# ZhentaoHuang/SealD-NeRF

Hardware: AMD Instinct MI355X
Metric: rendered rays/sec + sampled-points/sec, 800×800 D-NeRF jumpingjacks (higher is better)
Workload: dtype f16; 1 GPU; dnerf jumpingjacks-like 800x800 full-frame inference render, -O (fp16 field network, fp16 grid table), test sequence of 20 frames (camera orbit, one time stamp per frame, t = 0 .. 1: every frame selects its own occupancy slice, time encoding and the t == 0 canonical rule), T_thresh 1e-2, max_steps 1024, dt_gamma 0; rays=640000, field=fused, loop=device, frames_per_loop=4, rays_per_loop_on_this_gpu=2560000, frames_in_flight=4 loops of 4 frame(s) (the next starts when the newest is down to rays/2 alive), parallelism=single GPU

## Files before the change

### include/sdn_hip.h

```cpp
#ifndef SDN_HIP_H
#define SDN_HIP_H

#include <stdint.h>

#ifdef __cplusplus
extern "C" {
#endif

#define SDN_F32 0
#define SDN_F16 1

#define SDN_E_BADARG (-1)
#define SDN_E_UNSUPPORTED (-2)
#define SDN_E_TIMEOUT (-3)

const char *sdn_version(void);
int sdn_debug_shader_clock(unsigned long long *out4, uint32_t wall_ticks, void *stream);


int sdn_near_far_from_aabb(const float *rays_o, const float *rays_d, const float *aabb, uint32_t N,
                           float min_near, float *nears, float *fars, void *stream);

int sdn_sph_from_ray(const float *rays_o, const float *rays_d, float radius, uint32_t N, float *coords,
                     void *stream);

int sdn_get_rays(const float *pose, float fx, float fy, float cx, float cy, uint32_t H, uint32_t W, float *rays_o,
                 float *rays_d, void *stream);

int sdn_morton3D(const int32_t *coords, uint32_t N, int32_t *indices, void *stream);
int sdn_morton3D_invert(const int32_t *indices, uint32_t N, int32_t *coords, void *stream);

int sdn_packbits(const float *grid, uint32_t N, float density_thresh, uint8_t *bitfield, void *stream);

uint64_t sdn_march_rays_train_scratch_bytes(uint32_t N, uint32_t max_steps);
int sdn_march_rays_train(const float *rays_o, const float *rays_d, const uint8_t *grid, float bound,
                         float dt_gamma, uint32_t max_steps, uint32_t N, uint32_t C, uint32_t H, uint32_t M,
                         const float *nears, const float *fars, float *xyzs, float *dirs, float *deltas,
                         int32_t *rays, int32_t *counter, const float *noises, void *scratch, void *stream);

int sdn_composite_rays_train_forward(const float *sigmas, const float *rgbs, const float *deltas,
                                     const int32_t *rays, uint32_t M, uint32_t N, float T_thresh,
                                     float *weights_sum, float *depth, float *image, void *stream);

int sdn_composite_rays_train_backward(const float *grad_weights_sum, const float *grad_image,
                                      const float *sigmas, const float *rgbs, const float *deltas,
                                      const int32_t *rays, const float *weights_sum, const float *image,
                                      uint32_t M, uint32_t N, float T_thresh, float *grad_sigmas,
                                      float *grad_rgbs, void *stream);

int sdn_composite_whole_rays(const float *sigmas, const float *rgbs, const float *deltas, const int32_t *rays,
                             const float *nears, uint32_t M, uint32_t N, float T_thresh, float *weights_sum,
                             float *depth, float *image, void *stream);

int sdn_march_rays(uint32_t n_alive, uint32_t n_step, const int32_t *rays_alive, const float *rays_t,
                   const float *rays_o, const float *rays_d, float bound, float dt_gamma, uint32_t max_steps,
                   uint32_t C, uint32_t H, const uint8_t *grid, const float *nears, const float *fars,
                   float *xyzs, float *dirs, float *deltas, const float *noises, void *stream);

int sdn_march_rays_ex(uint32_t n_alive, uint32_t n_step, const int32_t *rays_alive, const float *rays_t,
                      const float *rays_o, const float *rays_d, float bound, float dt_gamma, uint32_t max_steps,
                      uint32_t C, uint32_t H, const uint8_t *grid, const float *fars, float *xyzs, float *dirs,
                      float *deltas, const float *noises, uint32_t M_pad, const uint8_t *cull_grid,
                      uint32_t *live_idx, uint32_t *live_count, void *stream);
uint32_t sdn_cull_grid_bytes(void);
int sdn_build_cull_grid(const uint8_t *bitfield, uint32_t H, uint8_t *cull_grid, void *stream);

int sdn_composite_rays(uint32_t n_alive, uint32_t n_step, float T_thresh, int32_t *rays_alive, float *rays_t,
                       const float *sigmas, const float *rgbs, const float *deltas, float *weights_sum,
                       float *depth, float *image, void *stream);

uint64_t sdn_compact_alive_scratch_bytes(uint32_t n);
int sdn_compact_alive(const int32_t *in, uint32_t n, int32_t *out, int32_t *n_out, void *scratch, void *stream);


int sdn_grid_encode_forward_quad_f16(const float *inputs, const void *quad_table, const int32_t *ref_offsets_host, void *outputs,
                                     uint32_t B, float S, uint32_t H, void *stream);
int sdn_grid_encode_forward(const float *inputs, const void *embeddings, const int32_t *offsets_host,
                            void *outputs, uint32_t B, uint32_t D, uint32_t C, uint32_t L, float S, uint32_t H,
                            void *dy_dx, uint32_t gridtype, int align_corners, uint32_t interp, int dtype,
                            void *stream);

int sdn_grid_encode_backward(const void *grad, const float *inputs, const int32_t *offsets_host,
                             void *grad_embeddings, uint32_t B, uint32_t D, uint32_t C, uint32_t L, float S,
                             uint32_t H, const void *dy_dx, void *grad_inputs, uint32_t gridtype,
                             int align_corners, uint32_t interp, int dtype, void *stream);
int sdn_grid_encode_backward_det(const void *grad, const float *inputs, const int32_t *offsets_host, void *grad_embeddings, uint32_t B,
                                 uint32_t D, uint32_t C, uint32_t L, float S, uint32_t H, const void *dy_dx, void *grad_inputs,
                                 uint32_t gridtype, int align_corners, uint32_t interp, int dtype, void *det_scratch, void *stream);

int sdn_sh_encode_forward(const float *inputs, float *outputs, uint32_t B, uint32_t D, uint32_t C,
                          float *dy_dx, void *stream);
int sdn_sh_encode_backward(const float *grad, const float *inputs, uint32_t B, uint32_t D, uint32_t C,
                           const float *dy_dx, float *grad_inputs, void *stream);

int sdn_freq_encode_forward(const float *inputs, uint32_t B, uint32_t D, uint32_t deg, uint32_t C,
                            float *outputs, void *stream);
int sdn_freq_encode_backward(const float *grad, const float *outputs, uint32_t B, uint32_t D, uint32_t deg,
                             uint32_t C, float *grad_inputs, void *stream);

uint32_t sdn_field_weight_blocks(void);

int sdn_field_forward_f16(const float *xyzs, const float *dirs, const uint32_t *live_idx, const uint32_t *live_count,
                          uint32_t M, const void *weights, const float *bias0, const void *table,
                          const int32_t *offsets_host, float S, uint32_t H, float bound, float density_scale,
                          int zero_deform, float *sigmas, float *rgbs, void *stream);

uint32_t sdn_field_weight_floats_f32(void);
int sdn_field_forward_f32(const float *xyzs, const float *dirs, const uint32_t *live_idx, const uint32_t *live_count,
                          uint32_t M, const float *weights, const float *bias0, const float *table,
                          const int32_t *offsets_host, float S, uint32_t H, float bound, float density_scale,
                          int zero_deform, float *sigmas, float *rgbs, float *deform, void *stream);

int sdn_field_forward_f32x3(const float *xyzs, const float *dirs, const uint32_t *live_idx, const uint32_t *live_count,
                            uint32_t M, const float *weights, const float *bias0, const float *table,
                            const int32_t *offsets_host, float S, uint32_t H, float bound, float density_scale,
                            int zero_deform, float *sigmas, float *rgbs, float *deform, void *stream);

void sdn_field_select_kernel(int persistent);
void sdn_field_persistent_workgroups(int n);

int sdn_field_build_quad_table(const void *embeddings, int dtype, const int32_t *ref_offsets_host, float S, uint32_t H, void *out,
                               void *stream);

int sdn_density_query_cells_f16(const int32_t *cells, const uint32_t *cell_count, uint32_t n, const float *noise, uint32_t seed,
                                uint32_t grid_size, float cas_bound, const void *weights, const float *bias0, const void *table,
                                const int32_t *offsets_host, float S, uint32_t H, float bound, float density_scale, int zero_deform,
                                float *tmp_slice, void *stream);
int sdn_density_query_cells_f32(const int32_t *cells, const uint32_t *cell_count, uint32_t n, const float *noise, uint32_t seed,
                                uint32_t grid_size, float cas_bound, const float *weights, const float *bias0, const float *table,
                                const int32_t *offsets_host, float S, uint32_t H, float bound, float density_scale, int zero_deform,
                                float *tmp_slice, void *stream);
int sdn_density_grid_ema(float *density_grid, const float *tmp_grid, uint64_t n, float decay, double *sum, void *stream);
int sdn_density_grid_pack(const float *density_grid, uint64_t n, const double *sum, float density_thresh, float *mean_out,
                          uint8_t *bitfield, void *stream);

uint64_t sdn_ffmlp_scratch_bytes(uint32_t B, uint32_t input_dim, uint32_t output_dim, uint32_t hidden_dim, uint32_t num_layers);

int sdn_ffmlp_forward(const void *inputs, const void *weights, uint32_t B, uint32_t input_dim, uint32_t output_dim,
                      uint32_t hidden_dim, uint32_t num_layers, uint32_t activation, uint32_t output_activation,
                      void *forward_buffer, void *outputs, void *scratch, void *stream);

int sdn_ffmlp_inference(const void *inputs, const void *weights, uint32_t B, uint32_t input_dim, uint32_t output_dim,
                        uint32_t hidden_dim, uint32_t num_layers, uint32_t activation, uint32_t output_activation,
                        void *outputs, void *scratch, void *stream);

int sdn_ffmlp_backward(const void *grad, const void *inputs, const void *weights, const void *forward_buffer, uint32_t B,
                       uint32_t input_dim, uint32_t output_dim, uint32_t hidden_dim, uint32_t num_layers,
                       uint32_t activation, uint32_t output_activation, int calc_grad_inputs, void *backward_buffer,
                       void *grad_inputs, void *grad_weights, void *scratch, void *stream);

typedef struct SdnSealBox {
    float bounds[24];
    uint32_t n_bounds, n_tris;
    const float *tris;
    float test_dir[3], tinv[12], rinv[9], scale[3], center[3];
    float hsv[3];
    int32_t modify_hsv;
    float rgb[3], rgb_light_offset;
    int32_t modify_rgb;
    int32_t has_map_source;
    float source_bound[6], map_source[3];
    uint32_t reserved_;
    void *scratch;
} SdnSealBox;

#define SDN_MAX_GROUP_FRAMES 16

typedef struct SdnFrameTime {
    const uint8_t *bitfield[SDN_MAX_GROUP_FRAMES];
    const float *field_bias0;
    uint32_t zero_deform;
    uint32_t reserved_;
    const void *cull_grid[SDN_MAX_GROUP_FRAMES];
} SdnFrameTime;

typedef struct SdnRenderCtx {
    const float *rays_o, *rays_d, *nears, *fars;
    const uint8_t *bitfield;
    void *cull_bits;
    int32_t *alive_a, *alive_b;
    float *rays_t, *weights_sum, *depth, *image;
    float *xyzs, *dirs, *deltas, *sigmas, *rgbs;
    uint32_t *live_idx;
    int32_t *live_counts, *state, *trace, *n_out;
    void *block_totals;
    const void *field_weights;
    const float *field_bias0;
    const void *grid_table;
    int32_t grid_offsets[17];
    float grid_S;
    uint32_t grid_H;
    uint32_t N, M_cap, n_counters, max_steps, C, H;
    float bound, dt_gamma, T_thresh, density_scale;
    int32_t zero_deform;
    const float *aabb;
    float min_near;
    int32_t reserved_;
    float *rays_tend;
    const struct SdnSealBox *seal;
    uint8_t *seal_mask;
    uint32_t n_group_frames, rays_per_frame;
    const uint8_t *frame_bitfield[SDN_MAX_GROUP_FRAMES];
    uint8_t *slot_frame;
    const void *frame_cull[SDN_MAX_GROUP_FRAMES];
    int32_t field_f32;
    int32_t reserved2_;
} SdnRenderCtx;

int sdn_render_begin(const SdnRenderCtx *ctx, void *stream);
int sdn_render_step_f16(const SdnRenderCtx *ctx, uint32_t bound_alive, void *stream);
int sdn_render_step_f16_ev(const SdnRenderCtx *ctx, uint32_t bound_alive, void *ev_field_begin, void *ev_field_end,
                           void *stream);
int sdn_render_time_kernel(int which);
int sdn_render_frame_f16(const SdnRenderCtx *ctx, float bg_color, float *image_out, float *depth_out, void *stream,
                         void *side_stream, void **ev_main, void **ev_copy, int32_t *host_snap, void **ev_field,
                         uint32_t max_field_events, uint32_t *iterations_out);
int sdn_render_frames_pipelined_f16(const SdnRenderCtx *const *ctxs, uint32_t n_ctx, uint32_t n_frames, const float *const *rays_o,
                                    const float *const *rays_d, float *const *image_outs, float *const *depth_outs, float bg_color,
                                    uint32_t overlap_div, void *const *streams, void *const *side_streams, void **ev_main,
                                    void **ev_copy, int32_t *host_snap, void *const *ev_field_frames, uint32_t max_field_events,
                                    const uint8_t *exclusive_frames, const SdnFrameTime *frame_times, void *const *done_events,
                                    uint32_t *iterations_out);
int sdn_seal_bbox_map(float *xyzs, float *dirs, uint32_t M, const float *bounds, uint32_t n_bounds, const float *tris,
                      uint32_t n_tris, const float *test_dir, const float *tinv, const float *rinv, const float *scale,
                      const float *center, uint8_t *mask, void *stream);
int sdn_seal_bbox_map_source(float *xyzs, float *dirs, uint32_t M, const float *bounds, uint32_t n_bounds, const float *tris,
                             uint32_t n_tris, const float *test_dir, const float *tinv, const float *rinv, const float *scale,
                             const float *center, const float *source_bound, const float *map_source, uint32_t *flag, uint8_t *mask,
                             const uint32_t *live_idx, const uint32_t *live_count, const int32_t *state, void *stream);
int sdn_seal_modify_hsv(float *rgbs, const uint8_t *mask, uint32_t M, float dh, float ds, float dv, void *stream);
int sdn_seal_modify_rgb(float *rgbs, const uint8_t *mask, uint32_t M, float r, float g, float b, float light_offset, void *scratch16,
                        const uint32_t *live_idx, const uint32_t *live_count, const int32_t *state, void *stream);

void *sdn_host_mailbox_alloc(uint32_t groups);
int sdn_host_mailbox_free(void *mailbox);
int sdn_render_finish(const SdnRenderCtx *ctx, float bg_color, float *image_out, float *depth_out, void *stream);

#define SDN_TRAIN_N_PARAMS 14

typedef struct SdnTrainParam {
    float *param;
    float *exp_avg, *exp_avg_sq;
    float *ema;
    uint64_t n;
} SdnTrainParam;

typedef struct SdnTrainStep {
    const float *rays_o, *rays_d;
    const float *target;
    const float *bg_color;
    float bg_value;
    uint32_t N, M;
    const uint8_t *bitfield;
    const void *cull_grid;
    const float *aabb;
    float bound, min_near, dt_gamma, density_scale, T_thresh;
    float time;
    uint32_t cascade, grid_size, max_steps;
    int32_t perturb;
    uint64_t noise_seed;
    const float *noises;
    int32_t *counter;
    int32_t grid_offsets[17];
    float grid_S;
    uint32_t grid_H;
    SdnTrainParam params[SDN_TRAIN_N_PARAMS];
    double lr_table, lr_net;
    double beta1, beta2, eps;
    float *adam_steps;
    float *loss_scale;
    int32_t *growth_tracker;
    float growth_factor, backoff_factor;
    uint32_t growth_interval;
    float ema_decay;
    float *loss_out;
    float *image_out;
    void *workspace;
    int32_t mode;
    int32_t keep_deform;
    float grad_divisor;
    int32_t deform_frozen;
    int32_t phase;
    int32_t sample_set;
    void *table_stream, *table_ready, *table_done;
    void *det_scratch;
} SdnTrainStep;

typedef struct SdnTrainLayout {
    uint64_t total_bytes;
    uint64_t w_table, w_deform, w_sigma0, w_sigma1, w_color;
    uint64_t g_table, g_deform, g_sigma0, g_sigma1, g_color;
    uint64_t xyzs, dirs, deltas, rays;
    uint64_t sample_set_stride;
    uint64_t sigmas;
    uint64_t weights_sum, depth, image;
    uint64_t found_inf;
} SdnTrainLayout;

int sdn_train_layout(uint32_t N, uint32_t M, uint32_t max_steps, const int32_t *grid_offsets, SdnTrainLayout *out);
int sdn_train_refresh(const SdnTrainStep *s, void *stream);
int sdn_train_step_f16(const SdnTrainStep *s, void *stream);
int sdn_train_flush(const SdnTrainStep *s, void *stream);

int sdn_train_layout_f32(uint32_t N, uint32_t M, uint32_t max_steps, const int32_t *grid_offsets, SdnTrainLayout *out);
int sdn_train_refresh_f32(const SdnTrainStep *s, void *stream);
int sdn_train_step_f32(const SdnTrainStep *s, void *stream);

#ifdef __cplusplus
}
#endif
#endif
```

### seald-nerf_amd/csrc/raymarching.hip

```cpp
#include <stdlib.h>

#include "sdn_common.h"
#include "sdn_internal.h"

namespace {
using sdn_int::FrameSel;

constexpr float kSqrt3 = 1.7320508075688772f;
constexpr float kRPi = 0.3183098861837907f;

__device__ __forceinline__ float signf_(float x) { return copysignf(1.0f, x); }
__device__ __forceinline__ float clampf_(float x, float lo, float hi) { return fminf(hi, fmaxf(lo, x)); }

__device__ __forceinline__ int mip_from_pos(float x, float y, float z, float max_cascade) {
    const float mx = fmaxf(fabsf(x), fmaxf(fabsf(y), fabsf(z)));
    int exponent;
    frexpf(mx, &exponent);
    return (int)fminf(max_cascade - 1, fmaxf(0.0f, (float)exponent));
}
__device__ __forceinline__ int mip_from_dt(float dt, float H, float max_cascade) {
    const float mx = (float)((double)(dt * H) * 0.5);
    int exponent;
    frexpf(mx, &exponent);
    return (int)fminf(max_cascade - 1, fmaxf(0.0f, (float)exponent));
// ... 702 lines not shown
    for (uint32_t k = lane; k < num_steps; k += 64u) {
        const float t = ts[k];
        const float dt = m.step_size(t);
        const float after = t + dt;
        float last = t0;
        if (k > 0) { const float tp = ts[k - 1]; last = tp + m.step_size(tp); }
        const size_t p = (size_t)point_index + k;
        xyzs[p * 3] = clampf_(m.ox + t * m.dx, -bound, bound);
        xyzs[p * 3 + 1] = clampf_(m.oy + t * m.dy, -bound, bound);
        xyzs[p * 3 + 2] = clampf_(m.oz + t * m.dz, -bound, bound);
        dirs[p * 3] = m.dx; dirs[p * 3 + 1] = m.dy; dirs[p * 3 + 2] = m.dz;
        deltas[p * 2] = dt;
        deltas[p * 2 + 1] = after - last;
    }
}

__global__ void __launch_bounds__(256) k_composite_train_fwd(const float *__restrict__ sigmas, const float *__restrict__ rgbs,
                                                             const float *__restrict__ deltas, const int32_t *__restrict__ rays,
                                                             uint32_t M, uint32_t N, float T_thresh, float *__restrict__ weights_sum,
                                                             float *__restrict__ depth, float *__restrict__ image) {
    const uint32_t n = threadIdx.x + blockIdx.x * blockDim.x;
    if (n >= N) return;
    const uint32_t index = (uint32_t)rays[n * 3], offset = (uint32_t)rays[n * 3 + 1], num_steps = (uint32_t)rays[n * 3 + 2];
    if (num_steps == 0 || offset + num_steps > M) {
        weights_sum[index] = 0; depth[index] = 0;
        image[(size_t)index * 3] = 0; image[(size_t)index * 3 + 1] = 0; image[(size_t)index * 3 + 2] = 0;
        return;
    }
    const float *s = sigmas + offset, *c = rgbs + (size_t)offset * 3, *dl = deltas + (size_t)offset * 2;
    uint32_t step = 0;
    float T = 1.0f, r = 0, g = 0, b = 0, ws = 0, t = 0, d = 0;
    while (step < num_steps) {
        const float alpha = 1.0f - sdn_exp_cr(-s[0] * dl[0]);
        const float weight = alpha * T;
        r += weight * c[0]; g += weight * c[1]; b += weight * c[2];
        t += dl[1];
        d += weight * t;
        ws += weight;
        T *= 1.0f - alpha;
        if (T < T_thresh) break;
        s++; c += 3; dl += 2; step++;
    }
    weights_sum[index] = ws; depth[index] = d;
    image[(size_t)index * 3] = r; image[(size_t)index * 3 + 1] = g; image[(size_t)index * 3 + 2] = b;
}

__global__ void __launch_bounds__(256) k_composite_whole_rays(const float *__restrict__ sigmas, const float *__restrict__ rgbs,
                                                              const float *__restrict__ deltas, const int32_t *__restrict__ rays,
                                                              const float *__restrict__ nears, uint32_t M, uint32_t N, float T_thresh,
                                                              float *__restrict__ weights_sum, float *__restrict__ depth, float *__restrict__ image) {
    const uint32_t n = threadIdx.x + blockIdx.x * blockDim.x;
    if (n >= N) return;
    const uint32_t index = (uint32_t)rays[n * 3], offset = (uint32_t)rays[n * 3 + 1], num_steps = (uint32_t)rays[n * 3 + 2];
    float weight_sum = 0, d = 0, r = 0, g = 0, b = 0;
    if (num_steps != 0 && offset + num_steps <= M) {
        const float *s = sigmas + offset, *c = rgbs + (size_t)offset * 3, *dl = deltas + (size_t)offset * 2;
        float t = nears[index];
        for (uint32_t step = 0; step < num_steps; step++) {
            if (dl[0] == 0) break;
            const float alpha = 1.0f - sdn_exp_cr(-s[0] * dl[0]);
            const float T = 1 - weight_sum;
            const float weight = alpha * T;
            weight_sum += weight;
            t += dl[1];
            d += weight * t;
            r += weight * c[0]; g += weight * c[1]; b += weight * c[2];
            if (T < T_thresh) break;
            s++; c += 3; dl += 2;
        }
    }
    weights_sum[index] = weight_sum; depth[index] = d;
    image[(size_t)index * 3] = r; image[(size_t)index * 3 + 1] = g; image[(size_t)index * 3 + 2] = b;
}

__global__ void __launch_bounds__(256) k_composite_train_bwd(const float *__restrict__ grad_weights_sum, const float *__restrict__ grad_image,
                                                             const float *__restrict__ sigmas, const float *__restrict__ rgbs,
                                                             const float *__restrict__ deltas, const int32_t *__restrict__ rays,
                                                             const float *__restrict__ weights_sum, const float *__restrict__ image,
                                                             uint32_t M, uint32_t N, float T_thresh, float *__restrict__ grad_sigmas,
                                                             float *__restrict__ grad_rgbs) {
    const uint32_t n = threadIdx.x + blockIdx.x * blockDim.x;
    if (n >= N) return;
    const uint32_t index = (uint32_t)rays[n * 3], offset = (uint32_t)rays[n * 3 + 1], num_steps = (uint32_t)rays[n * 3 + 2];
    if (num_steps == 0 || offset + num_steps > M) return;
    const float gws = grad_weights_sum[index];
    const float gi0 = grad_image[(size_t)index * 3], gi1 = grad_image[(size_t)index * 3 + 1], gi2 = grad_image[(size_t)index * 3 + 2];
    const float r_final = image[(size_t)index * 3], g_final = image[(size_t)index * 3 + 1], b_final = image[(size_t)index * 3 + 2];
    const float ws_final = weights_sum[index];
    const float *s = sigmas + offset, *c = rgbs + (size_t)offset * 3, *dl = deltas + (size_t)offset * 2;
    float *gs = grad_sigmas + offset, *gc = grad_rgbs + (size_t)offset * 3;
    uint32_t step = 0;
    float T = 1.0f, r = 0, g = 0, b = 0;
    while (step < num_steps) {
        const float alpha = 1.0f - sdn_exp_cr(-s[0] * dl[0]);
        const float weight = alpha * T;
        r += weight * c[0]; g += weight * c[1]; b += weight * c[2];
        T *= 1.0f - alpha;
        gc[0] = gi0 * weight; gc[1] = gi1 * weight; gc[2] = gi2 * weight;
        gs[0] = dl[0] * (gi0 * (T * c[0] - (r_final - r)) + gi1 * (T * c[1] - (g_final - g)) +
                         gi2 * (T * c[2] - (b_final - b)) + gws * (1 - ws_final));
        if (T < T_thresh) break;
        s++; c += 3; dl += 2; gs++; gc += 3; step++;
    }
}

constexpr float kTendUnset = -2.0f, kTendDead = -1.0f;
__device__ __forceinline__ float *state_tend(const int32_t *__restrict__ state) {
    return reinterpret_cast<float *>(((unsigned long long)(uint32_t)state[14] << 32) | (uint32_t)state[13]);
}
template <bool FAST>
__device__ __forceinline__ uint32_t march_ray(MarcherT<FAST> &m, const OccCache &oc, float t, float far, uint32_t n_step, float *px, float *pd,
                                              float *pl, float *tend = nullptr, uint8_t *psf = nullptr, uint32_t frame = 0,
                                              const float *t_begin = nullptr) {
    m.fine = oc.fine; m.fx0 = oc.fx0; m.fy0 = oc.fy0; m.fz0 = oc.fz0; m.fnx = oc.fnx; m.fny = oc.fny; m.fnz = oc.fnz;
    uint32_t step = 0;
    float last_t = t_begin ? *t_begin : t, x, y, z, dt;
    bool go = t < far;
    float t_end = far;
    if (FAST && oc.s_cull && go) {
        const float cached = tend ? *tend : kTendUnset;
        if (cached != kTendUnset) {
            t_end = cached;
            go = t < t_end;
        } else {
            go = ray_may_hit(oc.s_cull, m.ox, m.oy, m.oz, m.dx, m.dy, m.dz, t, far, t_end, oc.fx0, oc.fy0, oc.fz0, oc.fnx, oc.fny, oc.fnz);
            if (tend) *tend = go ? t_end : kTendDead;
        }
    }
    if (go) {
        while (t < far && t < t_end && step < n_step) {
            if (m.probe(t, x, y, z, dt, oc.s_cull)) {
                px[0] = x; px[1] = y; px[2] = z;
                pd[0] = m.dx; pd[1] = m.dy; pd[2] = m.dz;
                t += dt;
                pl[0] = dt;
                pl[1] = t - last_t;
                last_t = t;
                px += 3; pd += 3; pl += 2;
                if (psf) psf[step] = (uint8_t)frame;
                step++;
            }
        }
    }
    for (uint32_t k = step; k < n_step; k++) {
        px[0] = 0; px[1] = 0; px[2] = 0;
        pd[0] = 0; pd[1] = 0; pd[2] = 0;
        pl[0] = 0; pl[1] = 0;
        px += 3; pd += 3; pl += 2;
    }
    return step;
}

__device__ __forceinline__ uint32_t block_min_256(uint32_t v, uint32_t *lds4) {
    #pragma unroll
    for (int off = 32; off > 0; off >>= 1) v = min(v, (uint32_t)__shfl_xor((int)v, off, 64));
    __syncthreads();
    if ((threadIdx.x & 63u) == 0) lds4[threadIdx.x >> 6] = v;
    __syncthreads();
    return min(min(lds4[0], lds4[1]), min(lds4[2], lds4[3]));
}
constexpr uint32_t kNoFrame = 0xFFFFFFFFu;
__device__ __forceinline__ const uint8_t *frame_grid_uniform(const FrameSel &fs, uint32_t frame_uniform) {
    return fs.grid[__builtin_amdgcn_readfirstlane(frame_uniform)];
}

__device__ __forceinline__ void live_append(uint32_t step, uint32_t n, uint32_t n_step, uint32_t *__restrict__ live_idx,
                                            uint32_t *__restrict__ live_count) {
    const uint32_t lane = threadIdx.x & 63u;
    uint32_t incl = step;
    #pragma unroll
    for (int off = 1; off < 64; off <<= 1) {
        const uint32_t u = __shfl_up(incl, off, 64);
        if (lane >= (uint32_t)off) incl += u;
    }
    const uint32_t total = __shfl(incl, 63, 64);
    uint32_t base = 0;
    if (lane == 63 && total) base = atomicAdd(live_count, total);
    base = __shfl(base, 63, 64);
    const uint32_t dst = base + incl - step;
    for (uint32_t k = 0; k < step; k++) live_idx[dst + k] = n * n_step + k;
}

__device__ __forceinline__ bool composite_ray(int index, uint32_t n_step, float T_thresh, const float *s, const float *c, const float *dl,
                                              float *__restrict__ rays_t, float *__restrict__ weights_sum, float *__restrict__ depth,
                                              float *__restrict__ image, float *t_out = nullptr) {
    float t = rays_t[index];
    float weight_sum = weights_sum[index], d = depth[index];
    float r = image[(size_t)index * 3], g = image[(size_t)index * 3 + 1], b = image[(size_t)index * 3 + 2];
    uint32_t step = 0;
    if (n_step == 8) {
        float sv[8], cv[24], dv[16];
        #pragma unroll
        for (int q = 0; q < 2; q++) *reinterpret_cast<float4 *>(sv + 4 * q) = *reinterpret_cast<const float4 *>(s + 4 * q);
        #pragma unroll
        for (int q = 0; q < 6; q++) *reinterpret_cast<float4 *>(cv + 4 * q) = *reinterpret_cast<const float4 *>(c + 4 * q);
        #pragma unroll
        for (int q = 0; q < 4; q++) *reinterpret_cast<float4 *>(dv + 4 * q) = *reinterpret_cast<const float4 *>(dl + 4 * q);
        bool open = true;
        #pragma unroll
        for (int k = 0; k < 8; k++) {
            if (open && dv[2 * k] == 0) open = false;
            if (open) {
                const float alpha = 1.0f - sdn_exp_cr(-sv[k] * dv[2 * k]);
                const float T = 1 - weight_sum;
                const float weight = alpha * T;
                weight_sum += weight;
                t += dv[2 * k + 1];
                d += weight * t;
                r += weight * cv[3 * k]; g += weight * cv[3 * k + 1]; b += weight * cv[3 * k + 2];
                if (T < T_thresh) open = false; else step++;
            }
        }
    } else {
        while (step < n_step) {
            if (dl[0] == 0) break;
            const float alpha = 1.0f - sdn_exp_cr(-s[0] * dl[0]);
            const float T = 1 - weight_sum;
            const float weight = alpha * T;
            weight_sum += weight;
            t += dl[1];
            d += weight * t;
            r += weight * c[0]; g += weight * c[1]; b += weight * c[2];
            if (T < T_thresh) break;
            s++; c += 3; dl += 2; step++;
        }
    }
    const bool survives = !(step < n_step);
    if (survives) rays_t[index] = t;
    if (t_out) *t_out = t;
    weights_sum[index] = weight_sum; depth[index] = d;
    image[(size_t)index * 3] = r; image[(size_t)index * 3 + 1] = g; image[(size_t)index * 3 + 2] = b;
    return survives;
}

template <bool FAST>
__global__ void __launch_bounds__(256) k_march_rays(uint32_t n_alive, uint32_t n_step, const int32_t *__restrict__ rays_alive,
                                                    const float *__restrict__ rays_t, const float *__restrict__ rays_o,
                                                    const float *__restrict__ rays_d, float bound, float dt_gamma, uint32_t max_steps,
                                                    uint32_t C, uint32_t H, const uint8_t *__restrict__ grid,
                                                    const float *__restrict__ fars, float *__restrict__ xyzs, float *__restrict__ dirs,
                                                    float *__restrict__ deltas, const float *__restrict__ noises, uint32_t M_pad,
                                                    const uint32_t *__restrict__ cull, uint32_t *__restrict__ live_idx,
                                                    uint32_t *__restrict__ live_count, const int32_t *__restrict__ state,
                                                    const int32_t *__restrict__ rays_alive_b, FrameSel fs, const float *__restrict__ jump) {
    if (state) {
        n_alive = (uint32_t)state[0];
        n_step = (uint32_t)state[1];
        if (n_alive == 0) return;
        if (state[4]) rays_alive = rays_alive_b;
        live_count += state[3];
        const uint32_t m0 = n_alive * n_step;
        M_pad = m0 + (128u - m0 % 128u);
        if (!(state[15] && state[3] == 0)) jump = nullptr;
        if (blockIdx.x * 256u >= n_alive + 128u) return;
    }
    __shared__ uint4 s_cull4[FAST ? 256 : 1];
    __shared__ unsigned long long s_fine[FAST ? kFineCacheCells : 1];
    __shared__ uint32_t s_min4[4];
    const uint32_t n = threadIdx.x + blockIdx.x * blockDim.x;
    const int index = n < n_alive ? rays_alive[n] : -1;
    const bool grouped = fs.n_frames > 1;
    const uint32_t frame = (grouped && index >= 0) ? (uint32_t)index / fs.rays_per_frame : (grouped ? kNoFrame : 0u);
    uint32_t step = 0;
    float ro[3] = {0, 0, 0}, rdv[3] = {0, 0, 1}, t_ray = 0, far_ray = 0, t_jump = 0, noise = 0;
    if (index >= 0) {
        ro[0] = rays_o[(size_t)index * 3]; ro[1] = rays_o[(size_t)index * 3 + 1]; ro[2] = rays_o[(size_t)index * 3 + 2];
        rdv[0] = rays_d[(size_t)index * 3]; rdv[1] = rays_d[(size_t)index * 3 + 1]; rdv[2] = rays_d[(size_t)index * 3 + 2];
        t_ray = rays_t[index]; far_ray = fars[index];
        if (jump) t_jump = jump[index];
        if (noises) noise = noises[n];
    }
    uint32_t fcur = grouped ? block_min_256(frame, s_min4) : 0u;
    while (fcur != kNoFrame) {
        const uint8_t *grid_f = grouped ? frame_grid_uniform(fs, fcur) : grid;
        const uint32_t *cull_f = (grouped && cull) ? cull + (size_t)fcur * fs.cull_stride : cull;
        OccCache oc;
        occ_cache_load<FAST>(cull_f, grid_f, s_cull4, s_fine, oc);
        if (index >= 0 && frame == fcur) {
            MarcherT<FAST> m;
            m.init(ro, rdv, bound, dt_gamma, max_steps, C, H, grid_f);
            float t = t_ray;
            t += m.step_size(t) * noise;
            float *tend = state ? state_tend(state) : nullptr;
            if (tend) tend += index;
            const float t_walk = jump ? t_jump : t;
            step = march_ray<FAST>(m, oc, t_walk, far_ray, n_step, xyzs + (size_t)n * n_step * 3, dirs + (size_t)n * n_step * 3,
                                   deltas + (size_t)n * n_step * 2, tend, grouped ? fs.slot_frame + (size_t)n * n_step : nullptr, frame,
                                   jump ? &t : nullptr);
        }
        if (!grouped) break;
        fcur = block_min_256((frame != kNoFrame && frame > fcur) ? frame : kNoFrame, s_min4);
    }
    if (n >= n_alive) {
        const uint32_t slot = n_alive * n_step + (n - n_alive);
        if (slot < M_pad) {
            xyzs[(size_t)slot * 3] = 0; xyzs[(size_t)slot * 3 + 1] = 0; xyzs[(size_t)slot * 3 + 2] = 0;
            dirs[(size_t)slot * 3] = 0; dirs[(size_t)slot * 3 + 1] = 0; dirs[(size_t)slot * 3 + 2] = 0;
            deltas[(size_t)slot * 2] = 0; deltas[(size_t)slot * 2 + 1] = 0;
        }
    }
    if (live_idx) live_append(step, n, n_step, live_idx, live_count);
}

__device__ __forceinline__ uint32_t loop_list_len(const int32_t *__restrict__ state) {
    return state[8] ? (uint32_t)state[8] : (uint32_t)state[0];
}

__global__ void __launch_bounds__(256) k_composite_rays(uint32_t n_alive, uint32_t n_step, float T_thresh, int32_t *__restrict__ rays_alive,
                                                        float *__restrict__ rays_t, const float *__restrict__ sigmas,
                                                        const float *__restrict__ rgbs, const float *__restrict__ deltas,
                                                        float *__restrict__ weights_sum, float *__restrict__ depth, float *__restrict__ image,
                                                        const int32_t *__restrict__ state, int32_t *__restrict__ rays_alive_b,
                                                        uint32_t *__restrict__ block_totals) {
    if (state) {
        n_alive = loop_list_len(state);
        n_step = (uint32_t)state[1];
        if (state[4]) rays_alive = rays_alive_b;
    }
    const uint32_t n = threadIdx.x + blockIdx.x * blockDim.x;
    bool survives = false;
    if (n < n_alive) {
        const int index = rays_alive[n];
        if (index >= 0) {
            survives = composite_ray(index, n_step, T_thresh, sigmas + (size_t)n * n_step, rgbs + (size_t)n * n_step * 3,
                                     deltas + (size_t)n * n_step * 2, rays_t, weights_sum, depth, image);
            if (!survives) rays_alive[n] = -1;
        }
    }
    if (block_totals) {
        __shared__ uint32_t s_cnt[4];
        const unsigned long long m = __ballot(survives);
        if ((threadIdx.x & 63u) == 0) s_cnt[threadIdx.x >> 6] = (uint32_t)__popcll(m);
        __syncthreads();
        if (threadIdx.x == 0) block_totals[blockIdx.x] = s_cnt[0] + s_cnt[1] + s_cnt[2] + s_cnt[3];
    }
}

__global__ void __launch_bounds__(kScanBlock) k_compact_count(const int32_t *__restrict__ in, uint32_t n, uint32_t *__restrict__ block_totals,
                                                              const int32_t *__restrict__ state, const int32_t *__restrict__ in_b) {
    if (state) {
        n = loop_list_len(state);
        if (state[4]) in = in_b;
        if (blockIdx.x * kScanBlock >= n) return;
    }
    __shared__ uint32_t lds[16];
    const uint32_t i = blockIdx.x * kScanBlock + threadIdx.x;
    const bool keep = i < n && in[i] >= 0;
    const unsigned long long mask = __ballot(keep);
    if ((threadIdx.x & 63u) == 0) lds[threadIdx.x >> 6] = (uint32_t)__popcll(mask);
    __syncthreads();
    if (threadIdx.x == 0) {
        uint32_t t = 0;
        for (uint32_t w = 0; w < (kScanBlock >> 6); w++) t += lds[w];
        block_totals[blockIdx.x] = t;
    }
}

__global__ void __launch_bounds__(kScanBlock) k_compact_scatter(const int32_t *__restrict__ in, uint32_t n, const uint32_t *__restrict__ block_totals,
                                                                int32_t *__restrict__ out, int32_t *__restrict__ n_out,
                                                                const int32_t *__restrict__ state, const int32_t *__restrict__ in_b,
                                                                int32_t *__restrict__ out_b, uint32_t totals_per_block) {
    uint32_t last_block = gridDim.x - 1;
    if (state) {
        n = loop_list_len(state);
        if (state[4]) { in = in_b; out = out_b; }
        if (n == 0) {
            if (blockIdx.x == 0 && threadIdx.x == 0) n_out[0] = 0;
            return;
        }
        last_block = (n - 1) / kScanBlock;
        if (blockIdx.x > last_block) return;
    }
    __shared__ uint32_t lds[16];
    __shared__ uint32_t s_prev;
    uint32_t part = 0;
    for (uint32_t b = threadIdx.x; b < blockIdx.x * totals_per_block; b += kScanBlock) part += block_totals[b];
    uint32_t prev_total;
    block_inclusive_scan(part, lds, prev_total);
    if (threadIdx.x == 0) s_prev = prev_total;
    __syncthreads();
    const uint32_t i = blockIdx.x * kScanBlock + threadIdx.x;
    const int32_t v = i < n ? in[i] : -1;
    const bool keep = v >= 0;
    const unsigned long long mask = __ballot(keep);
    const uint32_t lane = threadIdx.x & 63u, wid = threadIdx.x >> 6;
    const uint32_t below = (uint32_t)__popcll(mask & ((1ull << lane) - 1ull));
    if (lane == 0) lds[wid] = (uint32_t)__popcll(mask);
    __syncthreads();
    uint32_t carry = 0, total = 0;
    for (uint32_t w = 0; w < (kScanBlock >> 6); w++) {
        const uint32_t c = lds[w];
        if (w < wid) carry += c;
        total += c;
    }
    if (keep) out[s_prev + carry + below] = v;
    if (blockIdx.x == last_block && threadIdx.x == 0) n_out[0] = (int32_t)(s_prev + total);
}


__global__ void __launch_bounds__(256) k_loop_init(uint32_t N, uint32_t max_steps, const float *__restrict__ nears, int32_t *__restrict__ alive_a,
                                                   float *__restrict__ rays_t, float *__restrict__ weights_sum, float *__restrict__ depth,
                                                   float *__restrict__ image, int32_t *__restrict__ state, int32_t *__restrict__ live_counts,
                                                   uint32_t n_counters, unsigned long long mailbox, uint32_t frame_tag,
                                                   float *__restrict__ rays_tend) {
    const uint32_t n = threadIdx.x + blockIdx.x * blockDim.x;
    if (n < N) {
        if (rays_tend) rays_tend[n] = kTendUnset;
        alive_a[n] = (int32_t)n;
        rays_t[n] = nears[n];
        weights_sum[n] = 0; depth[n] = 0;
        image[(size_t)n * 3] = 0; image[(size_t)n * 3 + 1] = 0; image[(size_t)n * 3 + 2] = 0;
    }
    if (n < n_counters) live_counts[n] = 0;
    if (n == 0) {
        state[0] = (int32_t)N; state[1] = 1; state[2] = 0; state[3] = 0; state[4] = 0;
        state[5] = (int32_t)N; state[6] = (int32_t)max_steps; state[7] = 0;
        for (int k = 8; k < 16; k++) state[k] = 0;
        state[10] = (int32_t)(uint32_t)mailbox;
        state[11] = (int32_t)(uint32_t)(mailbox >> 32);
        state[12] = (int32_t)frame_tag;
        const unsigned long long tp = (unsigned long long)(uintptr_t)rays_tend;
        state[13] = (int32_t)(uint32_t)tp;
        state[14] = (int32_t)(uint32_t)(tp >> 32);
    }
}


__device__ __forceinline__ void publish_snapshot(int32_t *__restrict__ state, int32_t *__restrict__ snap, int32_t call) {
    snap[(call & 3) * 2] = state[0];
    snap[(call & 3) * 2 + 1] = call + 1;
    const unsigned long long mb = ((unsigned long long)(uint32_t)state[11] << 32) | (uint32_t)state[10];
    if (mb) {
        const unsigned long long tag = ((uint32_t)state[12] << 16) | (uint32_t)(call + 1);
        __hip_atomic_store(reinterpret_cast<unsigned long long *>(mb) + (call & 3), (tag << 32) | (uint32_t)state[0], __ATOMIC_RELEASE,
                           __HIP_MEMORY_SCOPE_SYSTEM);
    }
}

__device__ __forceinline__ float lattice_floor(float t, float dt, float target) {
    for (int hop = 0; hop < 4; hop++) {
        const float first = t + dt;
        if (!(first <= target)) break;
        const float c = first - t;
        const float err = dt - c;
        const uint32_t eb = __float_as_uint(t) >> 23;
        const bool normal = t >= dt && dt > 0.0f && eb > 30u && eb < 254u;
        const float half_ulp = __uint_as_float((eb - 24u) << 23), c_cap = __uint_as_float((eb - 5u) << 23);
        if (!(normal && fabsf(err) != half_ulp && c < c_cap)) break;
        const float top = __uint_as_float(((eb + 1u) << 23) - 1u);
        const float lim = fminf(target, top);
        float k = floorf((lim - t) / c);
        while (t + (k + 1.0f) * c <= lim) k += 1.0f;
        while (k > 0.0f && t + k * c > lim) k -= 1.0f;
        t = t + k * c;
        if (lim == target) break;
        if (!(t + dt <= target)) break;
        t = t + dt;
    }
    return t;
}

__device__ __forceinline__ float certified_jump(const MarcherT<true> &m, float t, float t_safe) {
    const float dt = m.dt_const;
    if (!(t_safe > t + 64.0f * dt)) return t;
    const float L = lattice_floor(t, dt, t_safe - 18.0f * dt);
    if (!(L > t)) return t;
    const float c = (L + dt) - L, err = dt - c;
    const uint32_t eb = __float_as_uint(L) >> 23;
    if (!(L >= dt && dt > 0.0f && eb > 30u && eb < 254u)) return t;
    const float half_ulp = __uint_as_float((eb - 24u) << 23), c_cap = __uint_as_float((eb - 5u) << 23);
    if (!(fabsf(err) != half_ulp && c < c_cap && c > 0.0f)) return t;
    if ((__float_as_uint(L - 14.0f * c) >> 23) != eb || (__float_as_uint(L + 14.0f * c) >> 23) != eb) return t;
    float x, y, z;
    int vx, vy, vz, nx, ny, nz;
    m.locate(L, x, y, z, vx, vy, vz);
    float q = L;
    int k = 0;
    for (; k < 12; k++) {
        const float qm = q - c;
        if (!(qm > t) || (qm + dt) != q) return t;
        m.locate(qm, x, y, z, nx, ny, nz);
        if (nx != vx || ny != vy || nz != vz) break;
        q = qm;
    }
    if (k == 12) return t;
    float max_tt = -__FLT_MAX__;
    for (k = 0; k < 26; k++) {
        m.locate(q, x, y, z, nx, ny, nz);
        if (nx != vx || ny != vy || nz != vz) break;
        max_tt = fmaxf(max_tt, m.exit_t(q, x, y, z, nx, ny, nz));
        q = q + dt;
    }
    if (k == 26 || !(max_tt <= q) || !(q < t_safe - 4.0f * dt)) return t;
    return q;
}

__device__ __forceinline__ bool cull_start_ray(uint32_t n, const float *__restrict__ rays_o, const float *__restrict__ rays_d,
                                               const float *__restrict__ nears, const float *__restrict__ fars, const uint32_t *__restrict__ cull,
                                               const FrameSel &fs, int32_t *__restrict__ alive_a, float *__restrict__ rays_tend, float bound,
                                               float dt_gamma, uint32_t max_steps, uint32_t C, uint32_t H, float *__restrict__ jump) {
    const uint32_t frame = fs.n_frames > 1 ? n / fs.rays_per_frame : 0u;
    const uint32_t *__restrict__ cull_f = fs.n_frames > 1 ? cull + (size_t)frame * fs.cull_stride : cull;
    const int *meta = reinterpret_cast<const int *>(cull_f + kCullWords);
    const int fx0 = meta[0], fy0 = meta[1], fz0 = meta[2];
    const int fnx = meta[3] - fx0 + 1, fny = meta[4] - fy0 + 1, fnz = meta[5] - fz0 + 1;
    const float t = nears[n], far = fars[n];
    bool go = t < far;
    float t_end = far, start = t;
    if (go) {
        MarcherT<true> m;
        m.init(rays_o + (size_t)n * 3, rays_d + (size_t)n * 3, bound, dt_gamma, max_steps, C, H, nullptr);
        float t_safe;
        go = ray_may_hit(cull_f, m.ox, m.oy, m.oz, m.dx, m.dy, m.dz, t, far, t_end, fx0, fy0, fz0, fnx, fny, fnz, &t_safe);
        rays_tend[n] = go ? t_end : kTendDead;
        if (go && jump && m.dt_is_const) start = certified_jump(m, t, fminf(t_safe, fminf(far, t_end)));
    }
    alive_a[n] = go ? (int32_t)n : -1;
    if (jump) jump[n] = start;
    return go;
}

__global__ void __launch_bounds__(256) k_cull_start(uint32_t N, const float *__restrict__ rays_o, const float *__restrict__ rays_d,
                                                    const float *__restrict__ nears, const float *__restrict__ fars,
                                                    const uint32_t *__restrict__ cull, FrameSel fs, int32_t *__restrict__ alive_a,
                                                    float *__restrict__ rays_tend, float bound, float dt_gamma, uint32_t max_steps, uint32_t C,
                                                    uint32_t H, float *__restrict__ jump, uint32_t *__restrict__ block_totals) {
    const uint32_t n = threadIdx.x + blockIdx.x * blockDim.x;
    bool go = false;
    if (n < N) go = cull_start_ray(n, rays_o, rays_d, nears, fars, cull, fs, alive_a, rays_tend, bound, dt_gamma, max_steps, C, H, jump);
    __shared__ uint32_t s_cnt[4];
    const unsigned long long m = __ballot(go);
    if ((threadIdx.x & 63u) == 0) s_cnt[threadIdx.x >> 6] = (uint32_t)__popcll(m);
    __syncthreads();
    if (threadIdx.x == 0) block_totals[blockIdx.x] = s_cnt[0] + s_cnt[1] + s_cnt[2] + s_cnt[3];
}

__global__ void k_cull_advance(int32_t *__restrict__ state, const int32_t *__restrict__ n_out, int32_t *__restrict__ trace) {
    if (threadIdx.x != 0 || blockIdx.x != 0) return;
    const int32_t n0 = n_out[0];
    state[4] = 1;
    state[15] = 1;
    if (n0 > 0) {
        state[0] = n0;
    } else {
        trace[0] = state[5];
        trace[1] = state[1];
        state[2] += state[1];
        state[3] = 1;
        state[0] = 0;
    }
}

__global__ void k_loop_advance(int32_t *__restrict__ state, const int32_t *__restrict__ n_out, int32_t *__restrict__ trace,
                               int32_t *__restrict__ snap, int freeze) {
    if (threadIdx.x != 0 || blockIdx.x != 0) return;
    const int32_t it = state[3];
    const int32_t call = state[7];
    state[7] = call + 1;
    if (state[0] > 0) {
        trace[2 * it] = (it == 0 && state[15]) ? state[5] : state[0];
        trace[2 * it + 1] = state[1];
        state[2] += state[1];
        state[3] = it + 1;
        state[4] ^= 1;
        int32_t n_new = n_out[0];
        if (state[2] >= state[6]) n_new = 0;
        state[0] = n_new;
        if (n_new > 0) {
            int32_t ns = state[5] / n_new;
            state[1] = ns > 8 ? 8 : (ns < 1 ? 1 : ns);
        }
    }
    if (freeze) { state[8] = state[0]; state[9] = 0; }
    publish_snapshot(state, snap, call);
}

__device__ __forceinline__ uint32_t block_sum_256(uint32_t v, uint32_t *lds4) {
    #pragma unroll
    for (int off = 32; off > 0; off >>= 1) v += __shfl_down(v, off, 64);
    __syncthreads();
    if ((threadIdx.x & 63u) == 0) lds4[threadIdx.x >> 6] = v;
    __syncthreads();
    return lds4[0] + lds4[1] + lds4[2] + lds4[3];
}

__global__ void __launch_bounds__(256) k_scatter_advance(int32_t *__restrict__ alive_a, int32_t *__restrict__ alive_b,
                                                         const uint32_t *__restrict__ block_totals, int32_t *__restrict__ state,
                                                         int32_t *__restrict__ ticket, int32_t *__restrict__ trace, int32_t *__restrict__ snap,
                                                         int freeze) {
    __shared__ uint32_t lds4[4];
    __shared__ int s_last;
    const uint32_t n = loop_list_len(state);
    const int32_t *in = state[4] ? alive_b : alive_a;
    int32_t *out = state[4] ? alive_a : alive_b;
    const uint32_t nb = (n + 255u) / 256u;
    if (blockIdx.x < nb) {
        uint32_t part = 0;
        for (uint32_t b = threadIdx.x; b < blockIdx.x; b += 256) part += block_totals[b];
        const uint32_t prev = block_sum_256(part, lds4);
        const uint32_t i = blockIdx.x * 256u + threadIdx.x;
        const int32_t v = i < n ? in[i] : -1;
        const bool keep = v >= 0;
        const unsigned long long mask = __ballot(keep);
        const uint32_t lane = threadIdx.x & 63u, wid = threadIdx.x >> 6;
        const uint32_t below = (uint32_t)__popcll(mask & ((1ull << lane) - 1ull));
        __syncthreads();
        if (lane == 0) lds4[wid] = (uint32_t)__popcll(mask);
        __syncthreads();
        uint32_t carry = 0;
        for (uint32_t w = 0; w < wid; w++) carry += lds4[w];
        if (keep) out[prev + carry + below] = v;
    }
    __syncthreads();
    if (threadIdx.x == 0) {
        __threadfence();
        s_last = (atomicAdd(ticket, 1) == (int)gridDim.x - 1);
    }
    __syncthreads();
    if (!s_last) return;
    __threadfence();
    uint32_t part = 0;
    for (uint32_t b = threadIdx.x; b < nb; b += 256) part += block_totals[b];
    const uint32_t total = block_sum_256(part, lds4);
    if (threadIdx.x == 0) {
        *ticket = 0;
        const int32_t it = state[3];
        const int32_t call = state[7];
        state[7] = call + 1;
        if (state[0] > 0) {
            trace[2 * it] = (it == 0 && state[15]) ? state[5] : state[0];
            trace[2 * it + 1] = state[1];
            state[2] += state[1];
            state[3] = it + 1;
            state[4] ^= 1;
            int32_t n_new = (int32_t)total;
            if (state[2] >= state[6]) n_new = 0;
            state[0] = n_new;
            if (n_new > 0) {
                const int32_t ns = state[5] / n_new;
                state[1] = ns > 8 ? 8 : (ns < 1 ? 1 : ns);
            }
        }
        if (freeze) { state[8] = state[0]; state[9] = 0; }
        publish_snapshot(state, snap, call);
    }
}


__global__ void k_steady_begin(int32_t *__restrict__ state) {
    if (threadIdx.x == 0 && blockIdx.x == 0) { state[8] = state[0]; state[9] = 0; }
}

template <bool FAST>
__global__ void __launch_bounds__(256) k_composite_march(float T_thresh, int32_t *__restrict__ alive_a, int32_t *__restrict__ alive_b,
                                                         float *__restrict__ rays_t, const float *__restrict__ rays_o,
                                                         const float *__restrict__ rays_d, float bound, float dt_gamma, uint32_t max_steps,
                                                         uint32_t C, uint32_t H, const uint8_t *__restrict__ grid, const float *__restrict__ fars,
                                                         const float *__restrict__ sigmas, const float *__restrict__ rgbs,
                                                         float *__restrict__ xyzs, float *__restrict__ dirs, float *__restrict__ deltas,
                                                         float *__restrict__ weights_sum, float *__restrict__ depth, float *__restrict__ image,
                                                         const uint32_t *__restrict__ cull, uint32_t *__restrict__ live_idx,
                                                         uint32_t *__restrict__ live_counts, int32_t *__restrict__ state,
                                                         int32_t *__restrict__ ticket, int32_t *__restrict__ trace, int32_t *__restrict__ snap,
                                                         FrameSel fs) {
    __shared__ uint4 s_cull4[FAST ? 256 : 1];
    __shared__ unsigned long long s_fine[FAST ? kFineCacheCells : 1];
    __shared__ uint32_t s_cnt[4], s_min4[4];
    __shared__ int s_last;
    const uint32_t n_alive = (uint32_t)state[0], n_step = (uint32_t)state[1], list_len = (uint32_t)state[8];
    const int32_t it = state[3];
    int32_t *__restrict__ alive = state[4] ? alive_b : alive_a;
    const bool march_next = (uint32_t)state[2] + n_step < (uint32_t)state[6];
    const uint32_t n = threadIdx.x + blockIdx.x * blockDim.x;
    bool survives = false;
    uint32_t emitted = 0;
    if (n_alive > 0 && blockIdx.x * 256u < list_len) {
        const int index = n < list_len ? alive[n] : -1;
        float ro[3] = {0, 0, 0}, rdv[3] = {0, 0, 1}, far_ray = 0, t_new = 0;
        if (index >= 0) {
            if (march_next) {
                ro[0] = rays_o[(size_t)index * 3]; ro[1] = rays_o[(size_t)index * 3 + 1]; ro[2] = rays_o[(size_t)index * 3 + 2];
                rdv[0] = rays_d[(size_t)index * 3]; rdv[1] = rays_d[(size_t)index * 3 + 1]; rdv[2] = rays_d[(size_t)index * 3 + 2];
                far_ray = fars[index];
            }
            survives = composite_ray(index, n_step, T_thresh, sigmas + (size_t)n * n_step, rgbs + (size_t)n * n_step * 3,
                                     deltas + (size_t)n * n_step * 2, rays_t, weights_sum, depth, image, &t_new);
            if (!survives) alive[n] = -1;
        }
        const bool marches = survives && march_next;
        const bool grouped = fs.n_frames > 1;
        const uint32_t frame = (grouped && marches) ? (uint32_t)index / fs.rays_per_frame : (grouped ? kNoFrame : 0u);
        uint32_t fcur = grouped ? block_min_256(frame, s_min4) : 0u;
        while (fcur != kNoFrame) {
            const uint8_t *grid_f = grouped ? frame_grid_uniform(fs, fcur) : grid;
            const uint32_t *cull_f = (grouped && cull) ? cull + (size_t)fcur * fs.cull_stride : cull;
            OccCache oc;
            occ_cache_load<FAST>(cull_f, grid_f, s_cull4, s_fine, oc);
            if (marches && frame == fcur) {
                float *px = xyzs + (size_t)n * n_step * 3, *pd = dirs + (size_t)n * n_step * 3, *pl = deltas + (size_t)n * n_step * 2;
                MarcherT<FAST> m;
                m.init(ro, rdv, bound, dt_gamma, max_steps, C, H, grid_f);
                float *tend = state_tend(state);
                if (tend) tend += index;
                emitted = march_ray<FAST>(m, oc, t_new, far_ray, n_step, px, pd, pl, tend,
                                          grouped ? fs.slot_frame + (size_t)n * n_step : nullptr, frame);
            }
            if (!grouped) break;
            fcur = block_min_256((frame != kNoFrame && frame > fcur) ? frame : kNoFrame, s_min4);
        }
        live_append(emitted, n, n_step, live_idx, live_counts + it + 1);
    }
    const unsigned long long mask = __ballot(survives);
    if ((threadIdx.x & 63u) == 0) s_cnt[threadIdx.x >> 6] = (uint32_t)__popcll(mask);
    __syncthreads();
    if (threadIdx.x == 0) {
        const uint32_t c = s_cnt[0] + s_cnt[1] + s_cnt[2] + s_cnt[3];
        if (c) atomicAdd(state + 9, (int32_t)c);
        __threadfence();
        s_last = (atomicAdd(ticket, 1) == (int)gridDim.x - 1);
    }
    __syncthreads();
    if (!s_last || threadIdx.x != 0) return;
    __threadfence();
    *ticket = 0;
    const int32_t call = state[7];
    state[7] = call + 1;
    if (state[0] > 0) {
        trace[2 * it] = state[0];
        trace[2 * it + 1] = state[1];
        state[2] += state[1];
        state[3] = it + 1;
        int32_t n_new = atomicAdd(state + 9, 0);
        state[9] = 0;
        if (state[2] >= state[6]) n_new = 0;
        state[0] = n_new;
    }
    publish_snapshot(state, snap, call);
}

__global__ void __launch_bounds__(256) k_loop_finish(uint32_t N, const float *__restrict__ nears, const float *__restrict__ fars,
                                                     const float *__restrict__ weights_sum, const float *__restrict__ depth,
                                                     const float *__restrict__ image, float bg, float *__restrict__ image_out,
                                                     float *__restrict__ depth_out) {
    const uint32_t n = threadIdx.x + blockIdx.x * blockDim.x;
    if (n >= N) return;
    const float w = (1 - weights_sum[n]) * bg;
    image_out[(size_t)n * 3] = image[(size_t)n * 3] + w;
    image_out[(size_t)n * 3 + 1] = image[(size_t)n * 3 + 1] + w;
    image_out[(size_t)n * 3 + 2] = image[(size_t)n * 3 + 2] + w;
    depth_out[n] = fmaxf(depth[n] - nears[n], 0.0f) / (fars[n] - nears[n]);
}

}

namespace sdn_int {

int loop_begin(uint32_t N, uint32_t max_steps, const float *nears, int32_t *alive_a, float *rays_t, float *weights_sum, float *depth,
               float *image, int32_t *state, int32_t *live_counts, uint32_t n_counters, void *mailbox, uint32_t frame_tag, float *rays_tend,
               hipStream_t st) {
    const uint32_t threads = N > n_counters ? N : n_counters;
    hipLaunchKernelGGL(k_loop_init, dim3(sdn_div_up(threads, 256u)), dim3(256), 0, st, N, max_steps, nears, alive_a, rays_t, weights_sum, depth,
                       image, state, live_counts, n_counters, (unsigned long long)(uintptr_t)mailbox, frame_tag, rays_tend);
    return sdn_launch_status();
}

int loop_cull_start(uint32_t N, const float *rays_o, const float *rays_d, const float *nears, const float *fars, float bound, float dt_gamma,
                    uint32_t C, uint32_t H, const uint32_t *cull, const FrameSel &fs, int32_t *alive_a, int32_t *alive_b, float *rays_tend,
                    int32_t *state, uint32_t *block_totals, int32_t *n_out, int32_t *trace, uint32_t max_steps, float *jump, hipStream_t st) {
    if (!cull || !rays_tend || H != 128 || !fast_config(bound, C, H)) return 0;
    hipLaunchKernelGGL(k_cull_start, dim3(sdn_div_up(N, 256u)), dim3(256), 0, st, N, rays_o, rays_d, nears, fars, cull, fs, alive_a, rays_tend, bound,
                       dt_gamma, max_steps, C, H, jump, block_totals);
    const uint32_t nb = sdn_div_up(N, kScanBlock);
    hipLaunchKernelGGL(k_compact_scatter, dim3(nb), dim3(kScanBlock), 0, st, (const int32_t *)alive_a, N, (const uint32_t *)block_totals, alive_b, n_out,
                       (const int32_t *)nullptr, (const int32_t *)nullptr, (int32_t *)nullptr, 4u);
    hipLaunchKernelGGL(k_cull_advance, dim3(1), dim3(64), 0, st, state, (const int32_t *)n_out, trace);
    return sdn_launch_status();
}

int loop_march(uint32_t bound_alive, const int32_t *alive_a, const int32_t *alive_b, const float *rays_t, const float *rays_o,
               const float *rays_d, float bound, float dt_gamma, uint32_t max_steps, uint32_t C, uint32_t H, const uint8_t *grid,
               const float *fars, float *xyzs, float *dirs, float *deltas, const uint32_t *cull, uint32_t *live_idx,
               uint32_t *live_counts, const int32_t *state, const FrameSel &fs, hipStream_t st, const float *jump) {
    const dim3 g(sdn_div_up(bound_alive + 128u, 256u)), b(256);
    if (fast_config(bound, C, H)) {
        if (cull && H != 128) cull = nullptr;
        hipLaunchKernelGGL(k_march_rays<true>, g, b, 0, st, 0u, 0u, alive_a, rays_t, rays_o, rays_d, bound, dt_gamma, max_steps, C, H, grid, fars,
                           xyzs, dirs, deltas, (const float *)nullptr, 0u, cull, live_idx, live_counts, state, alive_b, fs, cull ? jump : (const float *)nullptr);
    } else {
        hipLaunchKernelGGL(k_march_rays<false>, g, b, 0, st, 0u, 0u, alive_a, rays_t, rays_o, rays_d, bound, dt_gamma, max_steps, C, H, grid, fars,
                           xyzs, dirs, deltas, (const float *)nullptr, 0u, (const uint32_t *)nullptr, live_idx, live_counts, state, alive_b, fs,
                           (const float *)nullptr);
    }
    return sdn_launch_status();
}

int loop_composite_compact(uint32_t bound_alive, float T_thresh, int32_t *alive_a, int32_t *alive_b, float *rays_t, const float *sigmas,
                           const float *rgbs, const float *deltas, float *weights_sum, float *depth, float *image, int32_t *state,
                           uint32_t *block_totals, int32_t *n_out, int32_t *trace, int32_t *snap, hipStream_t st, bool freeze) {
    const dim3 g(sdn_div_up(bound_alive, 256u)), b(256);
    if (bound_alive > 65536u) {
        static_assert(kScanBlock == 1024, "the compositing kernel's 256-ray survivor counts are summed four to a scatter block");
        hipLaunchKernelGGL(k_composite_rays, g, b, 0, st, 0u, 0u, T_thresh, alive_a, rays_t, sigmas, rgbs, deltas, weights_sum, depth, image,
                           (const int32_t *)state, alive_b, block_totals);
        const uint32_t nb = sdn_div_up(bound_alive, kScanBlock);
        hipLaunchKernelGGL(k_compact_scatter, dim3(nb), dim3(kScanBlock), 0, st, (const int32_t *)alive_a, 0u, (const uint32_t *)block_totals,
                           alive_b, snap + 8, (const int32_t *)state, (const int32_t *)alive_b, alive_a, 4u);
        hipLaunchKernelGGL(k_loop_advance, dim3(1), dim3(64), 0, st, state, (const int32_t *)(snap + 8), trace, snap, freeze ? 1 : 0);
        return sdn_launch_status();
    }
    hipLaunchKernelGGL(k_composite_rays, g, b, 0, st, 0u, 0u, T_thresh, alive_a, rays_t, sigmas, rgbs, deltas, weights_sum, depth, image,
                       (const int32_t *)state, alive_b, block_totals);
    hipLaunchKernelGGL(k_scatter_advance, g, b, 0, st, alive_a, alive_b, (const uint32_t *)block_totals, state, n_out, trace, snap, freeze ? 1 : 0);
    return sdn_launch_status();
}


int loop_steady_begin(uint32_t bound_alive, const int32_t *alive_a, const int32_t *alive_b, const float *rays_t, const float *rays_o,
                      const float *rays_d, float bound, float dt_gamma, uint32_t max_steps, uint32_t C, uint32_t H, const uint8_t *grid,
                      const float *fars, float *xyzs, float *dirs, float *deltas, const uint32_t *cull, uint32_t *live_idx,
                      uint32_t *live_counts, int32_t *state, const FrameSel &fs, hipStream_t st, bool frozen_already) {
    if (!frozen_already) hipLaunchKernelGGL(k_steady_begin, dim3(1), dim3(64), 0, st, state);
    return loop_march(bound_alive, alive_a, alive_b, rays_t, rays_o, rays_d, bound, dt_gamma, max_steps, C, H, grid, fars, xyzs, dirs, deltas,
                      cull, live_idx, live_counts, state, fs, st, nullptr);
}

int loop_composite_march(uint32_t bound_list, float T_thresh, int32_t *alive_a, int32_t *alive_b, float *rays_t, const float *rays_o,
                         const float *rays_d, float bound, float dt_gamma, uint32_t max_steps, uint32_t C, uint32_t H, const uint8_t *grid,
                         const float *fars, const float *sigmas, const float *rgbs, float *xyzs, float *dirs, float *deltas,
                         float *weights_sum, float *depth, float *image, const uint32_t *cull, uint32_t *live_idx, uint32_t *live_counts,
                         int32_t *state, int32_t *ticket, int32_t *trace, int32_t *snap, const FrameSel &fs, hipStream_t st) {
    const dim3 g(sdn_div_up(bound_list, 256u)), b(256);
    if (fast_config(bound, C, H)) {
        if (cull && H != 128) cull = nullptr;
        hipLaunchKernelGGL(k_composite_march<true>, g, b, 0, st, T_thresh, alive_a, alive_b, rays_t, rays_o, rays_d, bound, dt_gamma, max_steps, C, H,
                           grid, fars, sigmas, rgbs, xyzs, dirs, deltas, weights_sum, depth, image, cull, live_idx, live_counts, state, ticket,
                           trace, snap, fs);
    } else {
        hipLaunchKernelGGL(k_composite_march<false>, g, b, 0, st, T_thresh, alive_a, alive_b, rays_t, rays_o, rays_d, bound, dt_gamma, max_steps, C,
                           H, grid, fars, sigmas, rgbs, xyzs, dirs, deltas, weights_sum, depth, image, (const uint32_t *)nullptr, live_idx,
                           live_counts, state, ticket, trace, snap, fs);
    }
    return sdn_launch_status();
}

int loop_finish(uint32_t N, const float *nears, const float *fars, const float *weights_sum, const float *depth, const float *image, float bg,
                float *image_out, float *depth_out, hipStream_t st) {
    hipLaunchKernelGGL(k_loop_finish, dim3(sdn_div_up(N, 256u)), dim3(256), 0, st, N, nears, fars, weights_sum, depth, image, bg, image_out,
                       depth_out);
    return sdn_launch_status();
}

int build_cull(const uint8_t *bitfield, uint32_t *cull_bits, hipStream_t st, bool with_image) {
    hipLaunchKernelGGL(k_cull_meta_init, dim3(1), dim3(64), 0, st, cull_bits, 1u, 0u);
    hipLaunchKernelGGL(k_build_cull_grid, dim3(kCullRes * kCullRes * kCullRes / 256), dim3(256), 0, st, bitfield, cull_bits, FrameSel());
    if (with_image) hipLaunchKernelGGL(k_build_fine_image, dim3(kFineCacheCells / 256), dim3(256), 0, st, bitfield, cull_bits, FrameSel());
    return sdn_launch_status();
}

struct CullCopy { const uint32_t *src[SDN_MAX_GROUP_FRAMES]; };
__global__ void __launch_bounds__(256) k_copy_cull_grids(CullCopy srcs, uint32_t *__restrict__ dst, uint32_t words, uint32_t stride) {
    const uint32_t i = blockIdx.x * blockDim.x + threadIdx.x;
    if (i < words) dst[(size_t)blockIdx.y * stride + i] = srcs.src[blockIdx.y][i];
}

int copy_cull(const void *const *prebuilt, uint32_t n_frames, uint32_t *cull_bits, hipStream_t st) {
    CullCopy c{};
    for (uint32_t f = 0; f < n_frames && f < (uint32_t)SDN_MAX_GROUP_FRAMES; f++) c.src[f] = (const uint32_t *)prebuilt[f];
    const uint32_t words = sdn_cull_grid_bytes() / 4u;
    hipLaunchKernelGGL(k_copy_cull_grids, dim3(sdn_div_up(words, 256u), n_frames), dim3(256), 0, st, c, cull_bits, words, n_frames > 1 ? words : 0u);
    return sdn_launch_status();
}

int build_cull_group(const FrameSel &fs, uint32_t *cull_bits, hipStream_t st) {
    hipLaunchKernelGGL(k_cull_meta_init, dim3(1), dim3(64), 0, st, cull_bits, fs.n_frames, fs.cull_stride);
    hipLaunchKernelGGL(k_build_cull_grid, dim3(kCullRes * kCullRes * kCullRes / 256, fs.n_frames), dim3(256), 0, st, (const uint8_t *)nullptr,
                       cull_bits, fs);
    hipLaunchKernelGGL(k_build_fine_image, dim3(kFineCacheCells / 256, fs.n_frames), dim3(256), 0, st, (const uint8_t *)nullptr, cull_bits, fs);
    return sdn_launch_status();
}

FrameSel frame_sel(const SdnRenderCtx *c) {
    FrameSel fs;
    if (c->n_group_frames > 1) {
        fs.n_frames = c->n_group_frames;
        fs.rays_per_frame = c->rays_per_frame;
        fs.cull_stride = sdn_cull_grid_bytes() / 4u;
        for (uint32_t f = 0; f < c->n_group_frames && f < SDN_MAX_GROUP_FRAMES; f++) fs.grid[f] = c->frame_bitfield[f];
        fs.slot_frame = c->slot_frame;
    }
    return fs;
}

}

extern "C" {

int sdn_near_far_from_aabb(const float *rays_o, const float *rays_d, const float *aabb, uint32_t N, float min_near,
                           float *nears, float *fars, void *stream) {
    if (N == 0) return 0;
    if (!rays_o || !rays_d || !aabb || !nears || !fars) return SDN_E_BADARG;
    hipLaunchKernelGGL(k_near_far_from_aabb, dim3(sdn_div_up(N, 256u)), dim3(256), 0, (hipStream_t)stream, rays_o, rays_d, aabb, N,
                       min_near, nears, fars);
    return sdn_launch_status();
}

int sdn_sph_from_ray(const float *rays_o, const float *rays_d, float radius, uint32_t N, float *coords, void *stream) {
    if (N == 0) return 0;
    if (!rays_o || !rays_d || !coords) return SDN_E_BADARG;
    hipLaunchKernelGGL(k_sph_from_ray, dim3(sdn_div_up(N, 256u)), dim3(256), 0, (hipStream_t)stream, rays_o, rays_d, radius, N, coords);
    return sdn_launch_status();
}

int sdn_morton3D(const int32_t *coords, uint32_t N, int32_t *indices, void *stream) {
    if (N == 0) return 0;
    if (!coords || !indices) return SDN_E_BADARG;
    hipLaunchKernelGGL(k_morton3D, dim3(sdn_div_up(N, 256u)), dim3(256), 0, (hipStream_t)stream, coords, N, indices);
    return sdn_launch_status();
}

int sdn_morton3D_invert(const int32_t *indices, uint32_t N, int32_t *coords, void *stream) {
    if (N == 0) return 0;
    if (!coords || !indices) return SDN_E_BADARG;
    hipLaunchKernelGGL(k_morton3D_invert, dim3(sdn_div_up(N, 256u)), dim3(256), 0, (hipStream_t)stream, indices, N, coords);
    return sdn_launch_status();
}

int sdn_packbits(const float *grid, uint32_t N, float density_thresh, uint8_t *bitfield, void *stream) {
    if (N == 0) return 0;
    if (!grid || !bitfield) return SDN_E_BADARG;
    if (((uintptr_t)grid & 15u) != 0) return SDN_E_BADARG;
    hipLaunchKernelGGL(k_packbits, dim3(sdn_div_up(N, 256u)), dim3(256), 0, (hipStream_t)stream, (const float4 *)grid, N, density_thresh,
                       bitfield);
    return sdn_launch_status();
}

static uint64_t train_scratch_words(uint32_t N) { return (uint64_t)N + sdn_div_up(N, kScanBlock) + 4u; }

uint64_t sdn_march_rays_train_scratch_bytes(uint32_t N, uint32_t max_steps) {
    const uint64_t head = (train_scratch_words(N) * sizeof(uint32_t) + 15u) & ~(uint64_t)15u;
    const uint64_t cull = ((uint64_t)(kCullWords + 8u) * sizeof(uint32_t) + 15u) & ~(uint64_t)15u;
    return head + cull + (uint64_t)N * max_steps * sizeof(float);
}

int sdn_march_rays_train(const float *rays_o, const float *rays_d, const uint8_t *grid, float bound, float dt_gamma,
                         uint32_t max_steps, uint32_t N, uint32_t C, uint32_t H, uint32_t M, const float *nears,
                         const float *fars, float *xyzs, float *dirs, float *deltas, int32_t *rays, int32_t *counter,
                         const float *noises, void *scratch, void *stream) {
    return sdn_int::march_rays_train(rays_o, rays_d, grid, bound, dt_gamma, max_steps, N, C, H, M, nears, fars, xyzs, dirs, deltas, rays, counter, noises,
                                     scratch, nullptr, (hipStream_t)stream);
}

}

int sdn_int::march_rays_train(const float *rays_o, const float *rays_d, const uint8_t *grid, float bound, float dt_gamma, uint32_t max_steps, uint32_t N,
                              uint32_t C, uint32_t H, uint32_t M, const float *nears, const float *fars, float *xyzs, float *dirs, float *deltas,
                              int32_t *rays, int32_t *counter, const float *noises, void *scratch, const void *prebuilt_cull, hipStream_t st) {
    if (N == 0) return 0;
    if (!rays_o || !rays_d || !grid || !nears || !fars || !xyzs || !dirs || !deltas || !rays || !counter || !noises || !scratch)
        return SDN_E_BADARG;
    if (C == 0 || C > 16 || H == 0 || max_steps == 0 || ((uintptr_t)scratch & 15u) || ((uintptr_t)prebuilt_cull & 15u)) return SDN_E_BADARG;
    uint32_t *num_steps = (uint32_t *)scratch;
    const uint32_t nb = sdn_div_up(N, kScanBlock);
    uint32_t *block_totals = num_steps + N;
    uint32_t *base_out = block_totals + nb;
    const uint64_t head = (train_scratch_words(N) * sizeof(uint32_t) + 15u) & ~(uint64_t)15u;
    const uint64_t cull_bytes = ((uint64_t)(kCullWords + 8u) * sizeof(uint32_t) + 15u) & ~(uint64_t)15u;
    const uint32_t *cull = (const uint32_t *)((unsigned char *)scratch + head);
    float *sample_t = (float *)((unsigned char *)scratch + head + cull_bytes);
    const bool fast = fast_config(bound, C, H);
    const bool use_cull = fast && H == 128;
    if (use_cull && prebuilt_cull) {
        cull = (const uint32_t *)prebuilt_cull;
    } else if (use_cull) {
        int rc = sdn_int::build_cull(grid, (uint32_t *)((unsigned char *)scratch + head), st, false);
        if (rc) return rc;
    }
    if (fast && dt_gamma == 0.0f && H <= 256u)
        hipLaunchKernelGGL(k_march_train_count_wave, dim3(sdn_div_up(N, 4u)), dim3(256), 0, st, rays_o, rays_d, grid, bound, max_steps, N, H, nears,
                           fars, noises, num_steps, use_cull ? cull : nullptr, sample_t);
    else if (fast) hipLaunchKernelGGL(k_march_train_count<true>, dim3(sdn_div_up(N, 256u)), dim3(256), 0, st, rays_o, rays_d, grid, bound, dt_gamma,
                                 max_steps, N, C, H, nears, fars, noises, num_steps, use_cull ? cull : nullptr, sample_t);
    else hipLaunchKernelGGL(k_march_train_count<false>, dim3(sdn_div_up(N, 256u)), dim3(256), 0, st, rays_o, rays_d, grid, bound, dt_gamma,
                            max_steps, N, C, H, nears, fars, noises, num_steps, (const uint32_t *)nullptr, sample_t);
    const bool small = N <= 16u * kScanBlock;
    if (small) {
        hipLaunchKernelGGL(k_march_train_offsets_small, dim3(1), dim3(kScanBlock), 0, st, num_steps, N, rays, counter, base_out);
    } else {
        hipLaunchKernelGGL(k_scan_block_totals, dim3(nb), dim3(kScanBlock), 0, st, num_steps, N, block_totals);
        hipLaunchKernelGGL(k_march_train_offsets, dim3(nb), dim3(kScanBlock), 0, st, num_steps, N, block_totals, rays, counter, base_out);
    }
    if (fast) hipLaunchKernelGGL(k_march_train_emit<true>, dim3(sdn_div_up(N, 4u)), dim3(256), 0, st, rays_o, rays_d, bound, dt_gamma, max_steps, N, C, H, M,
                                 nears, noises, rays, base_out, sample_t, xyzs, dirs, deltas);
    else hipLaunchKernelGGL(k_march_train_emit<false>, dim3(sdn_div_up(N, 4u)), dim3(256), 0, st, rays_o, rays_d, bound, dt_gamma, max_steps, N, C, H, M,
                            nears, noises, rays, base_out, sample_t, xyzs, dirs, deltas);
    if (!small) hipLaunchKernelGGL(k_march_train_finish, dim3(1), dim3(64), 0, st, counter, base_out, N);
    return sdn_launch_status();
}

extern "C" {

int sdn_composite_rays_train_forward(const float *sigmas, const float *rgbs, const float *deltas, const int32_t *rays, uint32_t M,
                                     uint32_t N, float T_thresh, float *weights_sum, float *depth, float *image, void *stream) {
    if (N == 0) return 0;
    if ((M != 0 && (!sigmas || !rgbs || !deltas)) || !rays || !weights_sum || !depth || !image) return SDN_E_BADARG;
    hipLaunchKernelGGL(k_composite_train_fwd, dim3(sdn_div_up(N, 256u)), dim3(256), 0, (hipStream_t)stream, sigmas, rgbs, deltas, rays, M, N,
                       T_thresh, weights_sum, depth, image);
    return sdn_launch_status();
}

int sdn_composite_whole_rays(const float *sigmas, const float *rgbs, const float *deltas, const int32_t *rays, const float *nears, uint32_t M,
                             uint32_t N, float T_thresh, float *weights_sum, float *depth, float *image, void *stream) {
    if (N == 0) return 0;
    if (!sigmas || !rgbs || !deltas || !rays || !nears || !weights_sum || !depth || !image) return SDN_E_BADARG;
    hipLaunchKernelGGL(k_composite_whole_rays, dim3(sdn_div_up(N, 256u)), dim3(256), 0, (hipStream_t)stream, sigmas, rgbs, deltas, rays, nears, M, N,
                       T_thresh, weights_sum, depth, image);
    return sdn_launch_status();
}

int sdn_composite_rays_train_backward(const float *grad_weights_sum, const float *grad_image, const float *sigmas, const float *rgbs,
                                      const float *deltas, const int32_t *rays, const float *weights_sum, const float *image,
                                      uint32_t M, uint32_t N, float T_thresh, float *grad_sigmas, float *grad_rgbs, void *stream) {
    if (N == 0) return 0;
    if (M == 0) return 0;
    if (!grad_weights_sum || !grad_image || !sigmas || !rgbs || !deltas || !rays || !weights_sum || !image || !grad_sigmas || !grad_rgbs)
        return SDN_E_BADARG;
    hipLaunchKernelGGL(k_composite_train_bwd, dim3(sdn_div_up(N, 256u)), dim3(256), 0, (hipStream_t)stream, grad_weights_sum, grad_image,
                       sigmas, rgbs, deltas, rays, weights_sum, image, M, N, T_thresh, grad_sigmas, grad_rgbs);
    return sdn_launch_status();
}

static int launch_march_rays(uint32_t n_alive, uint32_t n_step, const int32_t *rays_alive, const float *rays_t, const float *rays_o,
                             const float *rays_d, float bound, float dt_gamma, uint32_t max_steps, uint32_t C, uint32_t H,
                             const uint8_t *grid, const float *fars, float *xyzs, float *dirs, float *deltas, const float *noises,
                             uint32_t M_pad, const uint32_t *cull, uint32_t *live_idx, uint32_t *live_count, hipStream_t st) {
    if (n_alive == 0 || n_step == 0) {
        if (M_pad && xyzs && dirs && deltas) {
            if (hipMemsetAsync(xyzs, 0, (size_t)M_pad * 12, st) != hipSuccess || hipMemsetAsync(dirs, 0, (size_t)M_pad * 12, st) != hipSuccess ||
                hipMemsetAsync(deltas, 0, (size_t)M_pad * 8, st) != hipSuccess)
                return sdn_launch_status();
        }
        return 0;
    }
    if (!rays_alive || !rays_t || !rays_o || !rays_d || !grid || !fars || !xyzs || !dirs || !deltas) return SDN_E_BADARG;
    if (C == 0 || C > 16 || H == 0 || max_steps == 0) return SDN_E_BADARG;
    if ((live_idx == nullptr) != (live_count == nullptr)) return SDN_E_BADARG;
    const uint32_t base = n_alive * n_step;
    if (M_pad < base) M_pad = base;
    const uint32_t threads = n_alive + (M_pad - base);
    const dim3 g(sdn_div_up(threads, 256u)), b(256);
    if (fast_config(bound, C, H)) {
        if (cull && H != 128) cull = nullptr;
        hipLaunchKernelGGL(k_march_rays<true>, g, b, 0, st, n_alive, n_step, rays_alive, rays_t, rays_o, rays_d, bound, dt_gamma, max_steps, C, H,
                           grid, fars, xyzs, dirs, deltas, noises, M_pad, cull, live_idx, live_count, (const int32_t *)nullptr,
                           (const int32_t *)nullptr, FrameSel(), (const float *)nullptr);
    } else {
        hipLaunchKernelGGL(k_march_rays<false>, g, b, 0, st, n_alive, n_step, rays_alive, rays_t, rays_o, rays_d, bound, dt_gamma, max_steps, C, H,
                           grid, fars, xyzs, dirs, deltas, noises, M_pad, (const uint32_t *)nullptr, live_idx, live_count,
                           (const int32_t *)nullptr, (const int32_t *)nullptr, FrameSel(), (const float *)nullptr);
    }
    return sdn_launch_status();
}

int sdn_march_rays(uint32_t n_alive, uint32_t n_step, const int32_t *rays_alive, const float *rays_t, const float *rays_o,
                   const float *rays_d, float bound, float dt_gamma, uint32_t max_steps, uint32_t C, uint32_t H,
                   const uint8_t *grid, const float *nears, const float *fars, float *xyzs, float *dirs, float *deltas,
                   const float *noises, void *stream) {
    (void)nears;
    return launch_march_rays(n_alive, n_step, rays_alive, rays_t, rays_o, rays_d, bound, dt_gamma, max_steps, C, H, grid, fars, xyzs, dirs,
                             deltas, noises, 0, nullptr, nullptr, nullptr, (hipStream_t)stream);
}

int sdn_march_rays_ex(uint32_t n_alive, uint32_t n_step, const int32_t *rays_alive, const float *rays_t, const float *rays_o,
                      const float *rays_d, float bound, float dt_gamma, uint32_t max_steps, uint32_t C, uint32_t H,
                      const uint8_t *grid, const float *fars, float *xyzs, float *dirs, float *deltas, const float *noises,
                      uint32_t M_pad, const uint8_t *cull_grid, uint32_t *live_idx, uint32_t *live_count, void *stream) {
    return launch_march_rays(n_alive, n_step, rays_alive, rays_t, rays_o, rays_d, bound, dt_gamma, max_steps, C, H, grid, fars, xyzs, dirs,
                             deltas, noises, M_pad, (const uint32_t *)cull_grid, live_idx, live_count, (hipStream_t)stream);
}

uint32_t sdn_cull_grid_bytes(void) { return kCullImageWord * 4 + kFineCacheCells * 8; }

int sdn_build_cull_grid(const uint8_t *bitfield, uint32_t H, uint8_t *cull_grid, void *stream) {
    if (!bitfield || !cull_grid) return SDN_E_BADARG;
    if (H != 128) return SDN_E_UNSUPPORTED;
    if (((uintptr_t)bitfield & 7u) != 0 || ((uintptr_t)cull_grid & 15u) != 0) return SDN_E_BADARG;
    hipLaunchKernelGGL(k_cull_meta_init, dim3(1), dim3(64), 0, (hipStream_t)stream, (uint32_t *)cull_grid, 1u, 0u);
    hipLaunchKernelGGL(k_build_cull_grid, dim3(kCullRes * kCullRes * kCullRes / 256), dim3(256), 0, (hipStream_t)stream, bitfield,
                       (uint32_t *)cull_grid, FrameSel());
    hipLaunchKernelGGL(k_build_fine_image, dim3(kFineCacheCells / 256), dim3(256), 0, (hipStream_t)stream, bitfield, (uint32_t *)cull_grid, FrameSel());
    return sdn_launch_status();
}

int sdn_composite_rays(uint32_t n_alive, uint32_t n_step, float T_thresh, int32_t *rays_alive, float *rays_t, const float *sigmas,
                       const float *rgbs, const float *deltas, float *weights_sum, float *depth, float *image, void *stream) {
    if (n_alive == 0 || n_step == 0) return 0;
    if (!rays_alive || !rays_t || !sigmas || !rgbs || !deltas || !weights_sum || !depth || !image) return SDN_E_BADARG;
    hipLaunchKernelGGL(k_composite_rays, dim3(sdn_div_up(n_alive, 256u)), dim3(256), 0, (hipStream_t)stream, n_alive, n_step, T_thresh,
                       rays_alive, rays_t, sigmas, rgbs, deltas, weights_sum, depth, image, (const int32_t *)nullptr, (int32_t *)nullptr,
                       (uint32_t *)nullptr);
    return sdn_launch_status();
}

uint64_t sdn_compact_alive_scratch_bytes(uint32_t n) { return (uint64_t)sdn_div_up(n, kScanBlock) * sizeof(uint32_t); }

int sdn_compact_alive(const int32_t *in, uint32_t n, int32_t *out, int32_t *n_out, void *scratch, void *stream) {
    if (!n_out) return SDN_E_BADARG;
    hipStream_t st = (hipStream_t)stream;
    if (n == 0) return (int)hipMemsetAsync(n_out, 0, sizeof(int32_t), st);
    if (!in || !out || !scratch) return SDN_E_BADARG;
    const uint32_t nb = sdn_div_up(n, kScanBlock);
    hipLaunchKernelGGL(k_compact_count, dim3(nb), dim3(kScanBlock), 0, st, in, n, (uint32_t *)scratch, (const int32_t *)nullptr,
                       (const int32_t *)nullptr);
    hipLaunchKernelGGL(k_compact_scatter, dim3(nb), dim3(kScanBlock), 0, st, in, n, (const uint32_t *)scratch, out, n_out,
                       (const int32_t *)nullptr, (const int32_t *)nullptr, (int32_t *)nullptr, 1u);
    return sdn_launch_status();
}

}
```

### seald-nerf_amd/csrc/render.hip

```cpp
#include <atomic>
#include <chrono>
#include <stdio.h>
#include <stdlib.h>
#include <string.h>

#include "sdn_common.h"
#include "sdn_internal.h"

namespace sdn_int {
int render_begin(const SdnRenderCtx *c, void *mailbox, uint32_t frame_tag, hipStream_t st) {
    if (c->aabb) {
        int rc0 = sdn_near_far_from_aabb(c->rays_o, c->rays_d, c->aabb, c->N, c->min_near, (float *)c->nears, (float *)c->fars, st);
        if (rc0) return rc0;
    }
    int rc = loop_begin(c->N, c->max_steps, c->nears, c->alive_a, c->rays_t, c->weights_sum, c->depth, c->image, c->state, c->live_counts,
                        c->n_counters, mailbox, frame_tag, c->rays_tend, st);
    if (rc) return rc;
    if (c->H == 128 && c->C == 1) {
        const uint32_t nf = c->n_group_frames > 1 ? c->n_group_frames : 1u;
        bool kept = true;
        for (uint32_t f = 0; f < nf; f++) kept = kept && c->frame_cull[f] != nullptr;
        if (kept) rc = copy_cull(c->frame_cull, nf, (uint32_t *)c->cull_bits, st);
        else rc = c->n_group_frames > 1 ? build_cull_group(frame_sel(c), (uint32_t *)c->cull_bits, st) : build_cull(c->bitfield, (uint32_t *)c->cull_bits, st);
        if (!rc && c->rays_tend)
            rc = loop_cull_start(c->N, c->rays_o, c->rays_d, c->nears, c->fars, c->bound, c->dt_gamma, c->C, c->H, (const uint32_t *)c->cull_bits, frame_sel(c),
                                 c->alive_a, c->alive_b, (float *)c->rays_tend, c->state, (uint32_t *)c->block_totals, c->trace + 2 * (size_t)c->n_counters + 8,
                                 c->trace, c->max_steps, c->sigmas, st);
    }
    return rc;
}
}

namespace {
std::atomic<int> g_timed_kernel{0};
}

extern "C" {

int sdn_render_time_kernel(int which) {
    if (which < 0 || which > 1) return SDN_E_BADARG;
    g_timed_kernel.store(which);
    return 0;
}

int sdn_render_finish(const SdnRenderCtx *c, float bg_color, float *image_out, float *depth_out, void *stream);
int sdn_render_step_f16_ev(const SdnRenderCtx *c, uint32_t bound_alive, void *ev_field_begin, void *ev_field_end, void *stream);

static int seal_map(const SdnRenderCtx *c, uint32_t m_slots, hipStream_t st) {
    const SdnSealBox *s = c->seal;
    if (!s) return 0;
    if (!c->seal_mask) return SDN_E_BADARG;
    if (s->has_map_source) {
        if (!s->scratch) return SDN_E_BADARG;
        return sdn_seal_bbox_map_source(c->xyzs, c->dirs, m_slots, s->bounds, s->n_bounds, s->tris, s->n_tris, s->test_dir, s->tinv, s->rinv,
                                        s->scale, s->center, s->source_bound, s->map_source, (uint32_t *)((char *)s->scratch + 16), c->seal_mask,
                                        c->live_idx, (const uint32_t *)c->live_counts, c->state, st);
    }
    return sdn_seal_bbox_map(c->xyzs, c->dirs, m_slots, s->bounds, s->n_bounds, s->tris, s->n_tris, s->test_dir, s->tinv, s->rinv, s->scale,
                             s->center, c->seal_mask, st);
}
static int seal_color(const SdnRenderCtx *c, uint32_t m_slots, hipStream_t st) {
    const SdnSealBox *s = c->seal;
    if (!s) return 0;
    int rc = 0;
    if (s->modify_hsv) rc = sdn_seal_modify_hsv(c->rgbs, c->seal_mask, m_slots, s->hsv[0], s->hsv[1], s->hsv[2], st);
    if (!rc && s->modify_rgb) {
        if (!s->scratch) return SDN_E_BADARG;
        rc = sdn_seal_modify_rgb(c->rgbs, c->seal_mask, m_slots, s->rgb[0], s->rgb[1], s->rgb[2], s->rgb_light_offset, s->scratch, c->live_idx,
                                 (const uint32_t *)c->live_counts, c->state, st);
    }
    return rc;
}

static int launch_field(const SdnRenderCtx *c, uint32_t m_bound, uint32_t expect_points, hipStream_t st) {
    if (c->field_f32 == 2)
        return sdn_int::field_forward_f32x3(c->xyzs, c->dirs, c->live_idx, (const uint32_t *)c->live_counts, c->state, m_bound,
                                            (const float *)c->field_weights, c->field_bias0, (const float *)c->grid_table, c->grid_offsets, c->grid_S,
                                            c->grid_H, c->bound, c->density_scale, c->zero_deform, c->sigmas, c->rgbs, nullptr,
                                            c->n_group_frames > 1 ? c->slot_frame : nullptr, c->n_group_frames > 1 ? c->n_group_frames : 1u, st);
    if (c->field_f32)
        return sdn_int::field_forward_f32(c->xyzs, c->dirs, c->live_idx, (const uint32_t *)c->live_counts, c->state, m_bound,
                                          (const float *)c->field_weights, c->field_bias0, (const float *)c->grid_table, c->grid_offsets, c->grid_S,
                                          c->grid_H, c->bound, c->density_scale, c->zero_deform, c->sigmas, c->rgbs, nullptr,
                                          c->n_group_frames > 1 ? c->slot_frame : nullptr, c->n_group_frames > 1 ? c->n_group_frames : 1u, st);
    return sdn_int::field_forward_f16(c->xyzs, c->dirs, c->live_idx, (const uint32_t *)c->live_counts, c->state, m_bound, c->field_weights,
                                      c->field_bias0, c->grid_table, c->grid_offsets, c->grid_S, c->grid_H, c->bound, c->density_scale,
                                      c->zero_deform, c->sigmas, c->rgbs, expect_points, c->n_group_frames > 1 ? c->slot_frame : nullptr,
                                      c->n_group_frames > 1 ? c->n_group_frames : 1u, st);
}

static bool ctx_ok(const SdnRenderCtx *c) {
    if (!(c && c->rays_o && c->rays_d && c->nears && c->fars && c->alive_a && c->alive_b && c->rays_t && c->weights_sum &&
          c->depth && c->image && c->state && c->live_counts && c->cull_bits))
        return false;
    if (c->n_group_frames > 1) {
        if (c->n_group_frames > SDN_MAX_GROUP_FRAMES || !c->slot_frame || c->rays_per_frame == 0 ||
            (uint64_t)c->n_group_frames * c->rays_per_frame != c->N)
            return false;
        for (uint32_t f = 0; f < c->n_group_frames; f++)
            if (!c->frame_bitfield[f]) return false;
        return true;
    }
    return c->bitfield != nullptr;
}

int sdn_render_begin(const SdnRenderCtx *c, void *stream) {
    if (!ctx_ok(c)) return SDN_E_BADARG;
    return sdn_int::render_begin(c, nullptr, 0, (hipStream_t)stream);
}

int sdn_render_step_f16(const SdnRenderCtx *c, uint32_t bound_alive, void *stream) {
    return sdn_render_step_f16_ev(c, bound_alive, nullptr, nullptr, stream);
}

int sdn_render_step_f16_ev(const SdnRenderCtx *c, uint32_t bound_alive, void *ev_field_begin, void *ev_field_end, void *stream) {
    if (!c || bound_alive == 0) return SDN_E_BADARG;
    if (bound_alive > c->N) bound_alive = c->N;
    hipStream_t st = (hipStream_t)stream;
    const uint32_t *cull = (c->H == 128 && c->C == 1) ? (const uint32_t *)c->cull_bits : nullptr;
    const bool time_march = g_timed_kernel.load() == 1;
    if (time_march && ev_field_begin) (void)hipEventRecord((hipEvent_t)ev_field_begin, st);
    int rc = sdn_int::loop_march(bound_alive, c->alive_a, c->alive_b, c->rays_t, c->rays_o, c->rays_d, c->bound, c->dt_gamma, c->max_steps,
                                 c->C, c->H, c->bitfield, c->fars, c->xyzs, c->dirs, c->deltas, cull, c->live_idx,
                                 (uint32_t *)c->live_counts, c->state, sdn_int::frame_sel(c), st, c->rays_tend ? c->sigmas : nullptr);
    if (time_march && ev_field_end) (void)hipEventRecord((hipEvent_t)ev_field_end, st);
    if (time_march) ev_field_begin = ev_field_end = nullptr;
    if (rc) return rc;
    uint64_t m_bound = (uint64_t)bound_alive * 8u;
    if (m_bound > c->N) m_bound = c->N;
    rc = seal_map(c, (uint32_t)m_bound, st);
    if (rc) return rc;
    if (ev_field_begin) (void)hipEventRecord((hipEvent_t)ev_field_begin, st);
    rc = launch_field(c, (uint32_t)m_bound, 0u, st);
    if (ev_field_end) (void)hipEventRecord((hipEvent_t)ev_field_end, st);
    if (rc) return rc;
    rc = seal_color(c, (uint32_t)m_bound, st);
    if (rc) return rc;
    return sdn_int::loop_composite_compact(bound_alive, c->T_thresh, c->alive_a, c->alive_b, c->rays_t, c->sigmas, c->rgbs, c->deltas,
                                           c->weights_sum, c->depth, c->image, c->state, (uint32_t *)c->block_totals, c->n_out, c->trace,
                                           c->trace + 2 * (size_t)c->n_counters, st);
}

}

namespace {

constexpr uint32_t kRecompactMin = 8192;
uint32_t recompact_pct(uint32_t list_len) { return list_len > 81920u ? 95u : 50u; }
constexpr int kDriverTimeoutSeconds = 20;

struct FrameRun {
    const SdnRenderCtx *c;
    hipStream_t st, side;
    void **ev_main, **ev_copy, **ev_field;
    int32_t *host_snap;
    uint32_t max_field_events;
    uint32_t bound, it;
    bool steady, done;
    bool recompact = false;
    uint32_t list_bound = 0;
    void *mail_dev = nullptr;
    uint32_t tag = 0;
    uint32_t last_alive = 0;

    int begin() {
        if (!ctx_ok(c)) return SDN_E_BADARG;
        bound = c->N; it = 0; steady = false; done = false; last_alive = c->N; recompact = false; list_bound = 0;
        mail_dev = nullptr;
        unsigned int flags = 0;
        void *dptr = nullptr;
        if (hipHostGetFlags(&flags, host_snap) == hipSuccess && (flags & hipHostMallocCoherent) &&
            hipHostGetDevicePointer(&dptr, host_snap, 0) == hipSuccess && dptr) {
            static std::atomic<uint32_t> frame_seq{0};
            tag = (frame_seq.fetch_add(1) % 0x7FFFu) + 1u;
            mail_dev = dptr;
        } else {
            (void)hipGetLastError();
        }
        return sdn_int::render_begin(c, mail_dev, tag, st);
    }
    const uint32_t *cull() const { return (c->H == 128 && c->C == 1) ? (const uint32_t *)c->cull_bits : nullptr; }

    int enqueue() {
        int32_t *snap_dev = c->trace + 2 * (size_t)c->n_counters;
        void *e0 = (ev_field && it < max_field_events) ? ev_field[2 * it] : nullptr;
        void *e1 = (ev_field && it < max_field_events) ? ev_field[2 * it + 1] : nullptr;
        int rc;
        if (!steady) {
            rc = sdn_render_step_f16_ev(c, bound, e0, e1, st);
        } else {
            uint64_t m_bound = (uint64_t)bound * 8u;
            if (m_bound > c->N) m_bound = c->N;
            rc = seal_map(c, (uint32_t)m_bound, st);
            if (rc) return rc;
            const bool time_march = g_timed_kernel.load() == 1;
            void *m0 = time_march ? e0 : nullptr, *m1 = time_march ? e1 : nullptr;
            if (time_march) e0 = e1 = nullptr;
            if (e0) (void)hipEventRecord((hipEvent_t)e0, st);
            rc = launch_field(c, (uint32_t)m_bound, last_alive * 8u, st);
            if (e1) (void)hipEventRecord((hipEvent_t)e1, st);
            if (!rc) rc = seal_color(c, (uint32_t)m_bound, st);
            if (!rc && m0) (void)hipEventRecord((hipEvent_t)m0, st);
            if (!rc && recompact) {
                rc = sdn_int::loop_composite_compact(bound, c->T_thresh, c->alive_a, c->alive_b, c->rays_t, c->sigmas, c->rgbs, c->deltas, c->weights_sum,
                                                     c->depth, c->image, c->state, (uint32_t *)c->block_totals, c->n_out, c->trace, snap_dev, st, true);
                const uint32_t nb = last_alive < bound ? last_alive : bound;
                if (!rc)
                    rc = sdn_int::loop_steady_begin(nb, c->alive_a, c->alive_b, c->rays_t, c->rays_o, c->rays_d, c->bound, c->dt_gamma, c->max_steps, c->C,
                                                    c->H, c->bitfield, c->fars, c->xyzs, c->dirs, c->deltas, cull(), c->live_idx, (uint32_t *)c->live_counts,
                                                    c->state, sdn_int::frame_sel(c), st, true);
                bound = list_bound = nb;
                recompact = false;
            } else if (!rc)
                rc = sdn_int::loop_composite_march(bound, c->T_thresh, c->alive_a, c->alive_b, c->rays_t, c->rays_o, c->rays_d, c->bound,
                                                   c->dt_gamma, c->max_steps, c->C, c->H, c->bitfield, c->fars, c->sigmas, c->rgbs, c->xyzs,
                                                   c->dirs, c->deltas, c->weights_sum, c->depth, c->image, cull(), c->live_idx,
                                                   (uint32_t *)c->live_counts, c->state, c->n_out, c->trace, snap_dev, sdn_int::frame_sel(c), st);
            if (!rc && m1) (void)hipEventRecord((hipEvent_t)m1, st);
        }
        if (rc) return rc;
        if (mail_dev) return 0;
        const uint32_t slot = it & 3u;
        hipError_t e = hipEventRecord((hipEvent_t)ev_main[slot], st);
        if (e == hipSuccess) e = hipStreamWaitEvent(side, (hipEvent_t)ev_main[slot], 0);
        if (e == hipSuccess) e = hipMemcpyAsync(host_snap + 2 * slot, snap_dev + 2 * slot, 2 * sizeof(int32_t), hipMemcpyDeviceToHost, side);
        if (e == hipSuccess) e = hipEventRecord((hipEvent_t)ev_copy[slot], side);
        return (int)e;
    }

    bool ready() const {
        if (it == 0) return true;
        const uint32_t prev = (it - 1) & 3u;
        if (mail_dev) {
            const uint64_t want = ((uint64_t)tag << 16) | it;
            return (__atomic_load_n(reinterpret_cast<const uint64_t *>(host_snap) + prev, __ATOMIC_ACQUIRE) >> 32) == want;
        }
        return hipEventQuery((hipEvent_t)ev_copy[prev]) == hipSuccess;
    }

    int settle() {
        if (it >= 1) {
            const uint32_t prev = (it - 1) & 3u;
            int32_t n_prev;
            if (mail_dev) {
                const uint64_t want = ((uint64_t)tag << 16) | it;
                const uint64_t *word = reinterpret_cast<const uint64_t *>(host_snap) + prev;
                uint64_t v;
                uint32_t spins = 0;
                auto t0 = std::chrono::steady_clock::now();
                auto t_query = t0;
                while (((v = __atomic_load_n(word, __ATOMIC_ACQUIRE)) >> 32) != want) {
                    if ((++spins & 0x3FFFu) == 0) {
                        const auto now = std::chrono::steady_clock::now();
                        if (now - t0 > std::chrono::seconds(kDriverTimeoutSeconds)) return SDN_E_TIMEOUT;
                        if (now - t_query > std::chrono::milliseconds(5)) {
                            t_query = now;
                            hipError_t q = hipStreamQuery(st);
                            if (q != hipSuccess && q != hipErrorNotReady) return (int)q;
                        }
                    }
                }
                n_prev = (int32_t)(uint32_t)v;
            } else {
                hipError_t e = hipEventSynchronize((hipEvent_t)ev_copy[prev]);
                if (e != hipSuccess) return (int)e;
                n_prev = host_snap[2 * prev];
            }
            if (n_prev <= 0) { done = true; return 0; }
            last_alive = (uint32_t)n_prev;
            if (!steady) {
                bound = (uint32_t)n_prev;
                if ((uint64_t)n_prev * 8u <= c->N) {
                    int rc = sdn_int::loop_steady_begin(bound, c->alive_a, c->alive_b, c->rays_t, c->rays_o, c->rays_d, c->bound, c->dt_gamma,
                                                        c->max_steps, c->C, c->H, c->bitfield, c->fars, c->xyzs, c->dirs, c->deltas, cull(),
                                                        c->live_idx, (uint32_t *)c->live_counts, c->state, sdn_int::frame_sel(c), st);
                    if (rc) return rc;
                    steady = true;
                    list_bound = bound;
                }
            } else if ((uint64_t)n_prev * 100u <= (uint64_t)list_bound * recompact_pct(list_bound) && (uint32_t)n_prev >= kRecompactMin) {
                recompact = true;
            }
        }
        it++;
        if (it > c->max_steps + 1) done = true;
        return 0;
    }
};

}

extern "C" {

int sdn_render_frame_f16(const SdnRenderCtx *c, float bg_color, float *image_out, float *depth_out, void *stream, void *side_stream,
                         void **ev_main, void **ev_copy, int32_t *host_snap, void **ev_field, uint32_t max_field_events,
                         uint32_t *iterations_out) {
    if (!c || !image_out || !depth_out || !side_stream || !ev_main || !ev_copy || !host_snap) return SDN_E_BADARG;
    FrameRun r{c, (hipStream_t)stream, (hipStream_t)side_stream, ev_main, ev_copy, ev_field, host_snap, max_field_events, 0, 0, false, false};
    int rc = r.begin();
    while (!rc && !r.done) {
        rc = r.enqueue();
        if (!rc) rc = r.settle();
    }
    if (rc) return rc;
    if (iterations_out) *iterations_out = r.it + 1;
    return sdn_render_finish(c, bg_color, image_out, depth_out, stream);
}

int sdn_render_frames_pipelined_f16(const SdnRenderCtx *const *ctxs, uint32_t n_ctx, uint32_t n_frames, const float *const *rays_o,
                                    const float *const *rays_d, float *const *image_outs, float *const *depth_outs, float bg_color,
                                    uint32_t overlap_div, void *const *streams, void *const *side_streams, void **ev_main, void **ev_copy,
                                    int32_t *host_snap, void *const *ev_field_frames, uint32_t max_field_events, const uint8_t *exclusive_frames,
                                    const SdnFrameTime *frame_times, void *const *done_events, uint32_t *iterations_out) {
    constexpr uint32_t kMaxCtx = 8;
    if (!ctxs || n_ctx == 0 || n_ctx > kMaxCtx || !rays_o || !rays_d || !image_outs || !depth_outs || !streams || !side_streams ||
        !ev_main || !ev_copy || !host_snap)
        return SDN_E_BADARG;
    for (uint32_t s = 0; s < n_ctx; s++)
        if (!ctxs[s] || !ctxs[s]->aabb || !side_streams[s]) return SDN_E_BADARG;
    if (n_frames == 0) return 0;
    if (overlap_div == 0) overlap_div = 1;
    SdnRenderCtx local[kMaxCtx];
    FrameRun runs[kMaxCtx];
    int frame_of[kMaxCtx];
    for (uint32_t s = 0; s < n_ctx; s++) { local[s] = *ctxs[s]; frame_of[s] = -1; }
    uint32_t next = 0, finished = 0;
    auto start = [&](uint32_t slot) -> int {
        if (!rays_o[next] || !rays_d[next] || !image_outs[next] || !depth_outs[next]) return SDN_E_BADARG;
        local[slot].rays_o = rays_o[next];
        local[slot].rays_d = rays_d[next];
        if (frame_times) {
            const SdnFrameTime &ft = frame_times[next];
            if (!ft.field_bias0 || !ft.bitfield[0]) return SDN_E_BADARG;
            local[slot].bitfield = ft.bitfield[0];
            for (uint32_t f = 0; f < SDN_MAX_GROUP_FRAMES; f++) local[slot].frame_bitfield[f] = ft.bitfield[f];
            for (uint32_t f = 0; f < SDN_MAX_GROUP_FRAMES; f++) local[slot].frame_cull[f] = ft.cull_grid[f];
            local[slot].field_bias0 = ft.field_bias0;
            local[slot].zero_deform = (int32_t)ft.zero_deform;
        }
        void **evf = ev_field_frames ? (void **)ev_field_frames[next] : nullptr;
        runs[slot] = FrameRun{&local[slot], (hipStream_t)streams[slot], (hipStream_t)side_streams[slot], ev_main + 4 * slot, ev_copy + 4 * slot,
                              evf, host_snap + 8 * slot, evf ? max_field_events : 0u, 0, 0, false, false};
        frame_of[slot] = (int)next++;
        return runs[slot].begin();
    };
    const bool stats = getenv("SDN_DRIVER_STATS") != nullptr;
    double t_work = 0, t_idle = 0;
    uint32_t n_loops = 0;
    auto now = [] { return std::chrono::duration<double, std::micro>(std::chrono::steady_clock::now().time_since_epoch()).count(); };
    auto launch_next = [&]() -> int {
        if (next >= n_frames) return 0;
        const uint32_t slot = next % n_ctx;
        if (frame_of[slot] >= 0) return 0;
        int newest = -1;
        bool any_active = false, excl_in_flight = false;
        for (uint32_t c = 0; c < n_ctx; c++) {
            if (frame_of[c] < 0) continue;
            any_active = true;
            if (newest < 0 || frame_of[c] > frame_of[newest]) newest = (int)c;
            if (exclusive_frames && exclusive_frames[frame_of[c]]) excl_in_flight = true;
        }
        bool ok = !any_active || (uint64_t)runs[newest].last_alive * overlap_div <= local[slot].N;
        if (exclusive_frames && any_active && (exclusive_frames[next] || excl_in_flight)) ok = false;
        if (!ok) return 0;
        int r = start(slot);
        if (!r) r = runs[slot].enqueue();
        return r;
    };
    auto fail = [&](int code) -> int {
        for (uint32_t c = 0; c < n_ctx; c++) { (void)hipStreamSynchronize((hipStream_t)streams[c]); (void)hipStreamSynchronize((hipStream_t)side_streams[c]); }
        (void)hipGetLastError();
        return code;
    };
    int rc = launch_next();
    if (rc) return fail(rc);
    auto t_last = stats ? now() : 0.0;
    uint32_t idle_spins = 0;
    auto t_progress = std::chrono::steady_clock::now();
    auto t_query = t_progress;
    while (finished < n_frames) {
        n_loops++;
        bool progress = false;
        uint32_t order[kMaxCtx], n_act = 0;
        for (uint32_t s2 = 0; s2 < n_ctx; s2++)
            if (frame_of[s2] >= 0) order[n_act++] = s2;
        for (uint32_t a = 1; a < n_act; a++)
            for (uint32_t b = a; b > 0 && frame_of[order[b]] < frame_of[order[b - 1]]; b--) { const uint32_t t = order[b]; order[b] = order[b - 1]; order[b - 1] = t; }
        for (uint32_t a = 0; a < n_act; a++) {
            const uint32_t s2 = order[a];
            if (!runs[s2].ready()) continue;
            progress = true;
            rc = runs[s2].settle();
            if (rc) return fail(rc);
            if (runs[s2].done) {
                const int f = frame_of[s2];
                rc = sdn_render_finish(&local[s2], bg_color, image_outs[f], depth_outs[f], streams[s2]);
                if (rc) return fail(rc);
                if (done_events && done_events[f]) {
                    hipError_t e = hipEventRecord((hipEvent_t)done_events[f], (hipStream_t)streams[s2]);
                    if (e != hipSuccess) return fail((int)e);
                }
                if (iterations_out) __atomic_store_n(&iterations_out[f], runs[s2].it + 1, __ATOMIC_RELEASE);
                frame_of[s2] = -1;
                finished++;
            } else {
                rc = runs[s2].enqueue();
                if (rc) return fail(rc);
            }
            rc = launch_next();
            if (rc) return fail(rc);
        }
        if (!progress) {
            rc = launch_next();
            if (rc) return fail(rc);
            if ((++idle_spins & 0x3FFFu) == 0) {
                const auto now_c = std::chrono::steady_clock::now();
                if (now_c - t_progress > std::chrono::milliseconds(5) && now_c - t_query > std::chrono::milliseconds(5)) {
                    t_query = now_c;
                    for (uint32_t c = 0; c < n_ctx; c++)
                        if (frame_of[c] >= 0) { hipError_t q = hipStreamQuery((hipStream_t)streams[c]); if (q != hipSuccess && q != hipErrorNotReady) return fail((int)q); }
                }
                if (now_c - t_progress > std::chrono::seconds(kDriverTimeoutSeconds)) return SDN_E_TIMEOUT;
            }
        } else {
            idle_spins = 0;
            t_progress = std::chrono::steady_clock::now();
        }
        if (stats) { const double t = now(); (progress ? t_work : t_idle) += t - t_last; t_last = t; }
    }
    if (stats)
        fprintf(stderr, "[sdn driver] frames %u contexts %u loops %u  host busy %.0f us  idle-polling %.0f us  mailbox %d\n", n_frames, n_ctx, n_loops, t_work,
                t_idle, runs[0].mail_dev != nullptr);
    return 0;
}

void *sdn_host_mailbox_alloc(uint32_t groups) {
    void *p = nullptr;
    if (groups == 0 || hipHostMalloc(&p, 32u * groups, hipHostMallocCoherent | hipHostMallocMapped) != hipSuccess) {
        (void)hipGetLastError();
        return nullptr;
    }
    memset(p, 0, 32u * groups);
    return p;
}

int sdn_host_mailbox_free(void *p) { return p ? (int)hipHostFree(p) : 0; }

int sdn_render_finish(const SdnRenderCtx *c, float bg_color, float *image_out, float *depth_out, void *stream) {
    if (!c || !image_out || !depth_out) return SDN_E_BADARG;
    return sdn_int::loop_finish(c->N, c->nears, c->fars, c->weights_sum, c->depth, c->image, bg_color, image_out, depth_out,
                                (hipStream_t)stream);
}

}
```

### seald-nerf_amd/csrc/sdn_internal.h

```cpp
#pragma once
#include "sdn_common.h"

namespace sdn_int {

struct FrameSel {
    uint32_t n_frames = 0;
    uint32_t rays_per_frame = 0;
    uint32_t cull_stride = 0;
    uint32_t pad_ = 0;
    const uint8_t *grid[SDN_MAX_GROUP_FRAMES] = {};
    uint8_t *slot_frame = nullptr;
};
FrameSel frame_sel(const SdnRenderCtx *c);

int loop_begin(uint32_t N, uint32_t max_steps, const float *nears, int32_t *alive_a, float *rays_t, float *weights_sum, float *depth,
               float *image, int32_t *state, int32_t *live_counts, uint32_t n_counters, void *mailbox, uint32_t frame_tag, float *rays_tend,
               hipStream_t st);
int loop_cull_start(uint32_t N, const float *rays_o, const float *rays_d, const float *nears, const float *fars, float bound, float dt_gamma,
                    uint32_t C, uint32_t H, const uint32_t *cull, const FrameSel &fs, int32_t *alive_a, int32_t *alive_b, float *rays_tend,
                    int32_t *state, uint32_t *block_totals, int32_t *n_out, int32_t *trace, uint32_t max_steps, float *jump, hipStream_t st);
int loop_march(uint32_t bound_alive, const int32_t *alive_a, const int32_t *alive_b, const float *rays_t, const float *rays_o,
               const float *rays_d, float bound, float dt_gamma, uint32_t max_steps, uint32_t C, uint32_t H, const uint8_t *grid,
               const float *fars, float *xyzs, float *dirs, float *deltas, const uint32_t *cull, uint32_t *live_idx,
               uint32_t *live_counts, const int32_t *state, const FrameSel &fs, hipStream_t st, const float *jump = nullptr);
int loop_composite_compact(uint32_t bound_alive, float T_thresh, int32_t *alive_a, int32_t *alive_b, float *rays_t, const float *sigmas,
                           const float *rgbs, const float *deltas, float *weights_sum, float *depth, float *image, int32_t *state,
                           uint32_t *block_totals, int32_t *n_out, int32_t *trace, int32_t *snap, hipStream_t st, bool freeze = false);
int loop_steady_begin(uint32_t bound_alive, const int32_t *alive_a, const int32_t *alive_b, const float *rays_t, const float *rays_o,
                      const float *rays_d, float bound, float dt_gamma, uint32_t max_steps, uint32_t C, uint32_t H, const uint8_t *grid,
                      const float *fars, float *xyzs, float *dirs, float *deltas, const uint32_t *cull, uint32_t *live_idx,
                      uint32_t *live_counts, int32_t *state, const FrameSel &fs, hipStream_t st, bool frozen_already = false);
int loop_composite_march(uint32_t bound_list, float T_thresh, int32_t *alive_a, int32_t *alive_b, float *rays_t, const float *rays_o,
                         const float *rays_d, float bound, float dt_gamma, uint32_t max_steps, uint32_t C, uint32_t H, const uint8_t *grid,
                         const float *fars, const float *sigmas, const float *rgbs, float *xyzs, float *dirs, float *deltas,
                         float *weights_sum, float *depth, float *image, const uint32_t *cull, uint32_t *live_idx, uint32_t *live_counts,
                         int32_t *state, int32_t *ticket, int32_t *trace, int32_t *snap, const FrameSel &fs, hipStream_t st);
int loop_finish(uint32_t N, const float *nears, const float *fars, const float *weights_sum, const float *depth, const float *image, float bg,
                float *image_out, float *depth_out, hipStream_t st);
int render_begin(const SdnRenderCtx *c, void *mailbox, uint32_t frame_tag, hipStream_t st);
int build_cull(const uint8_t *bitfield, uint32_t *cull_bits, hipStream_t st, bool with_image = true);
int march_rays_train(const float *rays_o, const float *rays_d, const uint8_t *grid, float bound, float dt_gamma, uint32_t max_steps, uint32_t N, uint32_t C,
                     uint32_t H, uint32_t M, const float *nears, const float *fars, float *xyzs, float *dirs, float *deltas, int32_t *rays, int32_t *counter,
                     const float *noises, void *scratch, const void *prebuilt_cull, hipStream_t st);
int build_cull_group(const FrameSel &fs, uint32_t *cull_bits, hipStream_t st);
int copy_cull(const void *const *prebuilt, uint32_t n_frames, uint32_t *cull_bits, hipStream_t st);
int field_forward_f16(const float *xyzs, const float *dirs, const uint32_t *live_idx, const uint32_t *live_count, const int32_t *state,
                      uint32_t M, const void *weights, const float *bias0, const void *table, const int32_t *offsets_host, float S,
                      uint32_t H, float bound, float density_scale, int zero_deform, float *sigmas, float *rgbs, uint32_t expect_points,
                      const uint8_t *slot_frame, uint32_t n_frames, hipStream_t st);

int field_forward_f32(const float *xyzs, const float *dirs, const uint32_t *live_idx, const uint32_t *live_count, const int32_t *state,
                      uint32_t M, const float *weights, const float *bias0, const float *table, const int32_t *offsets_host, float S,
                      uint32_t H, float bound, float density_scale, int zero_deform, float *sigmas, float *rgbs, float *deform,
                      const uint8_t *slot_frame, uint32_t n_frames, hipStream_t st);

int field_forward_f32x3(const float *xyzs, const float *dirs, const uint32_t *live_idx, const uint32_t *live_count, const int32_t *state,
                        uint32_t M, const float *weights, const float *bias0, const float *table, const int32_t *offsets_host, float S,
                        uint32_t H, float bound, float density_scale, int zero_deform, float *sigmas, float *rgbs, float *deform,
                        const uint8_t *slot_frame, uint32_t n_frames, hipStream_t st);

int field_cells_f16(const int32_t *cells, const uint32_t *cell_count, uint32_t n, const float *noise, uint32_t seed, uint32_t grid_size,
                    float cas_bound, const void *weights, const float *bias0, const void *table, const int32_t *offsets_host, float S,
                    uint32_t H, float bound, float density_scale, int zero_deform, float *tmp_slice, hipStream_t st);

}

namespace sdn_ffh {
struct PackJob { const void *weights; void *packed; uint32_t in_dim, W, L; int backward, with_last; };
struct DwJob { const void *G; uint32_t ldg, M; const void *X; uint32_t ldx, N; void *out; };
uint32_t total_frags(uint32_t in_dim, uint32_t W, uint32_t L, int backward, int with_last);
int pack_many(const PackJob *jobs, uint32_t n, hipStream_t st);
int forward_packed(const void *inputs, const void *packed, uint32_t B, uint32_t in_dim, uint32_t W, uint32_t L, uint32_t act,
                   void *forward_buffer, void *outputs, hipStream_t st);
int backward_packed(const void *grad, const void *packed, const void *forward_buffer, uint32_t B, uint32_t in_dim, uint32_t W, uint32_t L,
                    uint32_t act, int want_dx, void *backward_buffer, void *grad_inputs, hipStream_t st);
uint64_t dw_jobs_bytes(const DwJob *jobs, uint32_t n, uint32_t B);
int dw_jobs(const DwJob *jobs, uint32_t n, uint32_t B, void *partial, hipStream_t st);
}
```

### seald-nerf_amd/dnerf_amd/renderer.py

```python
import math

import numpy as np
import torch
import torch.nn as nn

import raymarching


def _meshgrid(*args):
    return torch.meshgrid(*args, indexing="ij")


def sample_pdf(bins, weights, n_samples, det=False):
    weights = weights + 1e-5
    pdf = weights / torch.sum(weights, -1, keepdim=True)
    cdf = torch.cumsum(pdf, -1)
    cdf = torch.cat([torch.zeros_like(cdf[..., :1]), cdf], -1)
    if det:
        u = torch.linspace(0.0 + 0.5 / n_samples, 1.0 - 0.5 / n_samples, steps=n_samples, device=weights.device)
        u = u.expand(list(cdf.shape[:-1]) + [n_samples])
    else:
        u = torch.rand(list(cdf.shape[:-1]) + [n_samples], device=weights.device)
    u = u.contiguous()
    inds = torch.searchsorted(cdf, u, right=True)
# ... 94 lines not shown
            counter = self.step_counter[self.local_step % 16]
            counter.zero_()
            self.local_step += 1
            bitfield = self.density_bitfield.index_select(0, t.reshape(1))[0]
            xyzs, dirs, deltas, rays = raymarching.march_rays_train(rays_o, rays_d, self.bound, bitfield, self.cascade,
                                                                    self.grid_size, nears, fars, counter, self.mean_count, perturb, 128,
                                                                    force_all_rays, dt_gamma, max_steps)
            sigmas, rgbs, deform = self(xyzs, dirs, time)
            sigmas = self.density_scale * sigmas
            args = (sigmas, rgbs, deltas, rays) if T_thresh is None else (sigmas, rgbs, deltas, rays, T_thresh)
            weights_sum, depth, image = raymarching.composite_rays_train(*args)
            image = image + (1 - weights_sum).unsqueeze(-1) * bg_color
            depth = torch.clamp(depth - nears, min=0) / (fars - nears)
            results["deform"] = deform
        else:
            weights_sum = torch.zeros(N, dtype=torch.float32, device=device)
            depth = torch.zeros(N, dtype=torch.float32, device=device)
            image = torch.zeros(N, 3, dtype=torch.float32, device=device)
            rays_alive = torch.arange(N, dtype=torch.int32, device=device)
            rays_t = nears.clone()
            bitfield = self.density_bitfield[t]
            step = 0
            while step < max_steps:
                n_alive = rays_alive.shape[0]
                if n_alive <= 0:
                    break
                n_step = max(min(N // n_alive, 8), 1)
                xyzs, dirs, deltas = raymarching.march_rays(n_alive, n_step, rays_alive, rays_t, rays_o, rays_d, self.bound, bitfield,
                                                            self.cascade, self.grid_size, nears, fars, 128, perturb if step == 0 else False,
                                                            dt_gamma, max_steps)
                sigmas, rgbs, _ = self(xyzs, dirs, time)
                sigmas = self.density_scale * sigmas
                cargs = (n_alive, n_step, rays_alive, rays_t, sigmas, rgbs, deltas, weights_sum, depth, image)
                raymarching.composite_rays(*(cargs if T_thresh is None else cargs + (T_thresh,)))
                rays_alive = rays_alive[rays_alive >= 0]
                step += n_step
            image = image + (1 - weights_sum).unsqueeze(-1) * bg_color
            depth = torch.clamp(depth - nears, min=0) / (fars - nears)
        results["depth"] = depth.view(*prefix)
        results["image"] = image.view(*prefix, 3)
        return results

    def run(self, rays_o, rays_d, time, num_steps=128, upsample_steps=128, bg_color=None, perturb=False, **kwargs):
        prefix = rays_o.shape[:-1]
        rays_o = rays_o.contiguous().view(-1, 3)
        rays_d = rays_d.contiguous().view(-1, 3)
        N = rays_o.shape[0]
        device = rays_o.device
        aabb = self.aabb_train if self.training else self.aabb_infer
        nears, fars = raymarching.near_far_from_aabb(rays_o, rays_d, aabb, self.min_near)
        nears, fars = nears.unsqueeze(-1), fars.unsqueeze(-1)
        z_vals = torch.linspace(0.0, 1.0, num_steps, device=device).unsqueeze(0).expand((N, num_steps))
        z_vals = nears + (fars - nears) * z_vals
        sample_dist = (fars - nears) / num_steps
        if perturb:
            z_vals = z_vals + (torch.rand(z_vals.shape, device=device) - 0.5) * sample_dist

        def points(z):
            p = rays_o.unsqueeze(-2) + rays_d.unsqueeze(-2) * z.unsqueeze(-1)
            return torch.min(torch.max(p, aabb[:3]), aabb[3:])

        def weights_of(z, sigma):
            deltas = torch.cat([z[..., 1:] - z[..., :-1], sample_dist * torch.ones_like(z[..., :1])], dim=-1)
            alphas = 1 - torch.exp(-deltas * self.density_scale * sigma)
            shifted = torch.cat([torch.ones_like(alphas[..., :1]), 1 - alphas + 1e-15], dim=-1)
            return deltas, alphas * torch.cumprod(shifted, dim=-1)[..., :-1]

        xyzs = points(z_vals)
        dens = {k: v.view(N, num_steps, -1) for k, v in self.density(xyzs.reshape(-1, 3), time).items()}
        if upsample_steps > 0:
            with torch.no_grad():
                deltas, weights = weights_of(z_vals, dens["sigma"].squeeze(-1))
                z_mid = z_vals[..., :-1] + 0.5 * deltas[..., :-1]
                new_z = sample_pdf(z_mid, weights[:, 1:-1], upsample_steps, det=not self.training).detach()
                new_xyzs = points(new_z)
            new_dens = {k: v.view(N, upsample_steps, -1) for k, v in self.density(new_xyzs.reshape(-1, 3), time).items()}
            z_vals, z_index = torch.sort(torch.cat([z_vals, new_z], dim=1), dim=1)
            xyzs = torch.cat([xyzs, new_xyzs], dim=1)
            xyzs = torch.gather(xyzs, dim=1, index=z_index.unsqueeze(-1).expand_as(xyzs))
            for k in dens:
                tmp = torch.cat([dens[k], new_dens[k]], dim=1)
                dens[k] = torch.gather(tmp, dim=1, index=z_index.unsqueeze(-1).expand_as(tmp))
        _, weights = weights_of(z_vals, dens["sigma"].squeeze(-1))
        dirs = rays_d.view(-1, 1, 3).expand_as(xyzs)
        dens = {k: v.view(-1, v.shape[-1]) for k, v in dens.items()}
        mask = weights > 1e-4
        rgbs = self.color(xyzs.reshape(-1, 3), dirs.reshape(-1, 3), mask=mask.reshape(-1), **dens).view(N, -1, 3)
        weights_sum = weights.sum(dim=-1)
        ori_z = ((z_vals - nears) / (fars - nears)).clamp(0, 1)
        depth = torch.sum(weights * ori_z, dim=-1)
        image = torch.sum(weights.unsqueeze(-1) * rgbs, dim=-2)
        bg_color = self._bg(rays_o, rays_d, bg_color)
        image = image + (1 - weights_sum).unsqueeze(-1) * bg_color
        return {"depth": depth.view(*prefix), "image": image.view(*prefix, 3), "deform": dens["deform"]}

    @torch.no_grad()
    def update_extra_state(self, decay=0.95, S=128):
        if not self.cuda_ray:
            return
        if getattr(self, "_density_updater", None) is not None:
            self._density_updater.refresh()
            self._mean_density_dev = self._density_updater.update(decay)
            self._update_step_counter()
            return
        dev = self.density_bitfield.device
        tmp_grid = -torch.ones_like(self.density_grid)
        half_time = 0.5 / self.time_size

        def query(coords, indices, t_idx, time, cas):
            xyzs = 2 * coords.float() / (self.grid_size - 1) - 1
            bound = min(2 ** cas, self.bound)
            half_grid = bound / self.grid_size
            cas_xyzs = xyzs * (bound - half_grid)
            cas_xyzs += (torch.rand_like(cas_xyzs) * 2 - 1) * half_grid
            time_perturb = time + (torch.rand_like(time) * 2 - 1) * half_time
            sigmas = self.density(cas_xyzs, time_perturb)["sigma"].reshape(-1).detach().float()
            tmp_grid[t_idx, cas, indices] = sigmas * self.density_scale

        if self.iter_density < 16:
            axes = [torch.arange(self.grid_size, dtype=torch.int32, device=dev).split(S) for _ in range(3)]
            for t_idx, time in enumerate(self.times):
                for xs in axes[0]:
                    for ys in axes[1]:
                        for zs in axes[2]:
                            xx, yy, zz = _meshgrid(xs, ys, zs)
                            coords = torch.cat([xx.reshape(-1, 1), yy.reshape(-1, 1), zz.reshape(-1, 1)], dim=-1)
                            indices = raymarching.morton3D(coords).long()
                            for cas in range(self.cascade):
                                query(coords, indices, t_idx, time, cas)
        elif self.iter_density < 100:
            N = self.grid_size ** 3 // 4
            for t_idx, time in enumerate(self.times):
                for cas in range(self.cascade):
                    coords = torch.randint(0, self.grid_size, (N, 3), device=dev)
                    indices = raymarching.morton3D(coords).long()
                    occ = torch.nonzero(self.density_grid[t_idx, cas] > 0).squeeze(-1)
                    if occ.shape[0] > 0:
                        occ = occ[torch.randint(0, occ.shape[0], [N], dtype=torch.long, device=dev)]
                        indices = torch.cat([indices, occ], dim=0)
                        coords = torch.cat([coords, raymarching.morton3D_invert(occ)], dim=0)
                    query(coords, indices, t_idx, time, cas)
        valid = (self.density_grid >= 0) & (tmp_grid >= 0)
        self.density_grid[valid] = torch.maximum(self.density_grid[valid] * decay, tmp_grid[valid])
        self.mean_density = torch.mean(self.density_grid.clamp(min=0)).item()
        self.iter_density += 1
        density_thresh = min(self.mean_density, self.density_thresh)
        for t_idx in range(self.time_size):
            raymarching.packbits(self.density_grid[t_idx], density_thresh, self.density_bitfield[t_idx])
        self._update_step_counter()

    def _update_step_counter(self):
        total_step = min(16, self.local_step)
        if total_step > 0:
            self.mean_count = int(self.step_counter[:total_step, 0].sum().item() / total_step)
        self.local_step = 0

    def render(self, rays_o, rays_d, time, staged=False, max_ray_batch=4096, **kwargs):
        _run = self.run_cuda if self.cuda_ray else self.run
        B, N = rays_o.shape[:2]
        device = rays_o.device
        if staged and not self.cuda_ray:
            depth = torch.empty((B, N), device=device)
            image = torch.empty((B, N, 3), device=device)
            for b in range(B):
                for head in range(0, N, max_ray_batch):
                    tail = min(head + max_ray_batch, N)
                    r = _run(rays_o[b:b + 1, head:tail], rays_d[b:b + 1, head:tail], time[b:b + 1], **kwargs)
                    depth[b:b + 1, head:tail] = r["depth"]
                    image[b:b + 1, head:tail] = r["image"]
            return {"depth": depth, "image": image}
        return _run(rays_o, rays_d, time, **kwargs)


class FrameWorkspace:

    def __init__(self, N, device):
        self.N = N
        f32, i32 = torch.float32, torch.int32
        M = N + 128 + 8 * 128
        self.xyzs = torch.empty(M, 3, dtype=f32, device=device)
        self.dirs = torch.empty(M, 3, dtype=f32, device=device)
        self.deltas = torch.empty(M, 2, dtype=f32, device=device)
        self.alive = [torch.empty(N, dtype=i32, device=device), torch.empty(N, dtype=i32, device=device)]
        self.rays_t = torch.empty(N, dtype=f32, device=device)
        self.weights_sum = torch.empty(N, dtype=f32, device=device)
        self.depth = torch.empty(N, dtype=f32, device=device)
        self.image = torch.empty(N, 3, dtype=f32, device=device)
        self.count = torch.zeros(1, dtype=i32, device=device)
        self.count_host = torch.zeros(1, dtype=i32).pin_memory()
        from sdn_backend import lib
        self.scratch = torch.empty(max(int(lib.sdn_compact_alive_scratch_bytes(N)), 4), dtype=torch.uint8, device=device)
        self.cull = torch.empty(int(lib.sdn_cull_grid_bytes()), dtype=torch.uint8, device=device)
        self.live_idx = torch.empty(M, dtype=i32, device=device)
        self.live_counts = torch.zeros(1024 + 8, dtype=i32, device=device)


@torch.no_grad()
def render_frame(model, rays_o, rays_d, time, fp16=False, dt_gamma=0.0, max_steps=1024, T_thresh=1e-2, bg_color=1.0,
                 workspace=None, field=None, count_samples=True, use_cull=True, mapper=None):
    from sdn_backend import lib, check, ptr, stream
    device = rays_o.device
    rays_o = rays_o.contiguous().view(-1, 3)
    rays_d = rays_d.contiguous().view(-1, 3)
    N = rays_o.shape[0]
    ws = workspace if workspace is not None and workspace.N == N else FrameWorkspace(N, device)
    nears, fars = raymarching.near_far_from_aabb(rays_o, rays_d, model.aabb_infer, model.min_near)
    bitfield = model.density_bitfield[model.time_slice(time)]
    ws.weights_sum.zero_(); ws.depth.zero_(); ws.image.zero_()
    ws.rays_t.copy_(nears)
    torch.arange(N, dtype=torch.int32, device=device, out=ws.alive[0])
    cur = 0
    n_alive = N
    step = 0
    trace = []
    use_list = field is not None
    n_samples = torch.zeros((), dtype=torch.int64, device=device) if (count_samples and not use_list) else None
    st = stream()
    evaluate = field if field is not None else _field_eval(model, time, fp16)
    cull = None
    if use_cull and model.grid_size == 128 and model.cascade == 1:
        check(lib.sdn_build_cull_grid(ptr(bitfield), 128, ptr(ws.cull), st), "build_cull_grid")
        cull = ptr(ws.cull)
    if use_list:
        ws.live_counts.zero_()
    it = 0
    while step < max_steps and n_alive > 0:
        n_step = max(min(N // n_alive, 8), 1)
        M0 = n_alive * n_step
        M = M0 + (128 - M0 % 128)
        xyzs, dirs, deltas = ws.xyzs[:M], ws.dirs[:M], ws.deltas[:M]
        alive = ws.alive[cur]
        live_count = ws.live_counts[it:it + 1] if use_list else None
        check(lib.sdn_march_rays_ex(n_alive, n_step, ptr(alive), ptr(ws.rays_t), ptr(rays_o), ptr(rays_d), float(model.bound),
                                    float(dt_gamma), int(max_steps), int(model.cascade), int(model.grid_size), ptr(bitfield), ptr(fars),
                                    ptr(xyzs), ptr(dirs), ptr(deltas), None, M, cull, ptr(ws.live_idx) if use_list else None,
                                    ptr(live_count), st), "march_rays_ex")
        if n_samples is not None:
            n_samples += (deltas[:M0, 0] > 0).sum()
        q_xyzs, q_dirs, mapped = xyzs, dirs, None
        native_map = mapper is not None and hasattr(mapper, "map_to_origin_") and mapper._native_ok(xyzs, dirs)
        if native_map:
            mapper.map_data_conversion(xyzs)
            mapped = mapper.map_to_origin_(xyzs, dirs)
        elif mapper is not None:
            q_xyzs, q_dirs, mapped = mapper.map_to_origin(xyzs, dirs)
            q_xyzs, q_dirs = q_xyzs.contiguous(), q_dirs.contiguous()
        if use_list:
            sigmas, rgbs = evaluate(q_xyzs, q_dirs, ws.live_idx, live_count)
        else:
            sigmas, rgbs = evaluate(q_xyzs, q_dirs)
        if native_map:
            mapper.map_color_(rgbs, mapped)
        elif mapped is not None and bool(mapped.any()):
            rgbs[mapped] = mapper.map_color(q_xyzs[mapped], q_dirs[mapped], rgbs[mapped]).to(rgbs.dtype)
        check(lib.sdn_composite_rays(n_alive, n_step, float(T_thresh), ptr(alive), ptr(ws.rays_t), ptr(sigmas), ptr(rgbs), ptr(deltas),
                                     ptr(ws.weights_sum), ptr(ws.depth), ptr(ws.image), st), "composite_rays")
        check(lib.sdn_compact_alive(ptr(alive), n_alive, ptr(ws.alive[1 - cur]), ptr(ws.count), ptr(ws.scratch), st), "compact_alive")
        ws.count_host.copy_(ws.count, non_blocking=True)
        torch.cuda.current_stream().synchronize()
        trace.append((n_alive, n_step, M))
        n_alive = int(ws.count_host[0])
        cur = 1 - cur
        step += n_step
        it += 1
    if getattr(model, "bg_radius", -1) > 0:
        bg_color = model._bg(rays_o, rays_d, None).float()
    image = ws.image + (1 - ws.weights_sum).unsqueeze(-1) * bg_color
    depth = torch.clamp(ws.depth - nears, min=0) / (fars - nears)
    if count_samples:
        total = int(ws.live_counts[:it].sum().item()) if use_list else int(n_samples.item())
    else:
        total = None
    return {"image": image, "depth": depth, "weights_sum": ws.weights_sum.clone(), "trace": trace, "nears": nears, "fars": fars,
            "n_samples": total}


def _field_eval(model, time, fp16):
    def run(xyzs, dirs):
        keep = model.__dict__.get("fused_inference")
        model.fused_inference = False
        try:
            if fp16:
                with torch.autocast("cuda", dtype=torch.float16):
                    sigmas, rgbs, _ = model(xyzs, dirs, time)
            else:
                sigmas, rgbs, _ = model(xyzs, dirs, time)
        finally:
            if keep is None:
                del model.fused_inference
            else:
                model.fused_inference = keep
        return (model.density_scale * sigmas).float().contiguous(), rgbs.float().contiguous()
    return run


class DeviceLoop:

    RING = 4
    MAX_TIMED = 24

    def __init__(self, model, field, N, device, max_steps=1024, T_thresh=1e-2, dt_gamma=0.0, mailbox=True, mapper=None, frames=1,
                 keep_cull_grids=False):
        import ctypes
        from sdn_backend import lib, SdnRenderCtx, MAX_GROUP_FRAMES
        f32, i32 = torch.float32, torch.int32
        self.model, self.field, self.N = model, field, N
        self.frames = int(frames)
        self.keep_cull_grids = bool(keep_cull_grids)
        if not 1 <= self.frames <= MAX_GROUP_FRAMES or N % self.frames:
            raise ValueError(f"a frame group holds 1..{MAX_GROUP_FRAMES} frames of equal ray count (N = {N}, frames = {frames})")
        M = N + 128 + 8 * 128
        n_counters = max_steps + 8
        z = lambda *shape, dt=f32: torch.empty(*shape, dtype=dt, device=device)
        self.buf = dict(alive_a=z(N, dt=i32), alive_b=z(N, dt=i32), rays_t=z(N), weights_sum=z(N), depth=z(N), image=z(N, 3),
                        xyzs=z(M, 3), dirs=z(M, 3), deltas=z(M, 2), sigmas=z(M), rgbs=z(M, 3), live_idx=z(M, dt=i32),
                        live_counts=torch.zeros(n_counters, dtype=i32, device=device), state=torch.zeros(16, dtype=i32, device=device),
                        trace=torch.zeros(2 * n_counters + 16, dtype=i32, device=device), n_out=torch.zeros(1, dtype=i32, device=device),
                        block_totals=z((N + 255) // 256 + 1, dt=i32), nears=z(N), fars=z(N), rays_tend=z(N),
                        cull_bits=torch.empty(self.frames * int(lib.sdn_cull_grid_bytes()), dtype=torch.uint8, device=device))
        if self.frames > 1:
            self.buf["slot_frame"] = torch.zeros(M, dtype=torch.uint8, device=device)
        self.image_out, self.depth_out = z(N, 3), z(N)
        self.snap = self.buf["trace"][2 * n_counters: 2 * n_counters + 8].view(4, 2)
        from sdn_backend import HostMailbox
        self.host_state = HostMailbox(1) if mailbox else torch.zeros(self.RING, 2, dtype=i32).pin_memory()
        self.events = [torch.cuda.Event() for _ in range(self.RING)]
        self.copy_events = [torch.cuda.Event() for _ in range(self.RING)]
        self.side = torch.cuda.Stream(device=device)
        self._handles = None
        self._timing_queue = []
        c = SdnRenderCtx()
        for k, v in self.buf.items():
            setattr(c, k, v.data_ptr())
        c.field_weights, c.field_bias0, c.grid_table = field.weights.data_ptr(), field.bias0.data_ptr(), field.table.data_ptr()
        c.grid_offsets = (ctypes.c_int32 * 17)(*[int(v) for v in field.offsets_host])
        c.grid_S, c.grid_H = field.S, field.H
        c.N, c.M_cap, c.n_counters, c.max_steps, c.C, c.H = N, M, n_counters, int(max_steps), int(model.cascade), int(model.grid_size)
        c.bound, c.dt_gamma, c.T_thresh, c.density_scale = float(model.bound), float(dt_gamma), float(T_thresh), float(model.density_scale)
        c.n_group_frames, c.rays_per_frame = (self.frames, N // self.frames) if self.frames > 1 else (0, 0)
        c.field_f32 = field.ctx_kind
        self.ctx = c
        self.max_steps = int(max_steps)
        self.set_mapper(mapper)

    def set_mapper(self, mapper):
        import ctypes
        from sdn_backend import SdnSealBox
        c = self.ctx
        self.mapper = mapper
        if mapper is None:
            c.seal, c.seal_mask, self._seal = None, None, None
            return
        dev = self.buf["xyzs"].device
        mapper.map_data_conversion(self.buf["xyzs"])
        a = mapper._native_args(dev)
        if self.frames > 1 and ("map_source" in mapper.map_data or "rgb" in mapper.map_data):
            raise NotImplementedError("mapSource / rgb tint depend on the set of samples of an iteration: render such edits one frame per loop")
        box = SdnSealBox()
        for k in range(6 * a["n_bounds"]):
            box.bounds[k] = a["bounds"][k]
        box.n_bounds, box.n_tris, box.tris = a["n_bounds"], a["n_tris"], a["tris"].data_ptr()
        for name, n in (("test_dir", 3), ("tinv", 12), ("rinv", 9), ("scale", 3), ("center", 3)):
            for k in range(n):
                getattr(box, name)[k] = a[name][k]
        if "hsv" in mapper.map_data:
            h = [float(v) for v in mapper.map_data["hsv"].reshape(-1).tolist()]
            box.hsv[0], box.hsv[1], box.hsv[2], box.modify_hsv = h[0], h[1], h[2], 1
        if "rgb" in a:
            box.rgb[0], box.rgb[1], box.rgb[2], box.rgb_light_offset, box.modify_rgb = a["rgb"][0], a["rgb"][1], a["rgb"][2], a["rgb_light_offset"], 1
        if "map_source" in a:
            for k in range(6):
                box.source_bound[k] = a["source_bound"][k]
            for k in range(3):
                box.map_source[k] = a["map_source"][k]
            box.has_map_source = 1
        scratch = torch.zeros(32, dtype=torch.uint8, device=dev)
        box.scratch = scratch.data_ptr()
        mask = torch.empty(self.buf["sigmas"].shape[0], dtype=torch.uint8, device=dev)
        self._seal = (box, mask, a, scratch)
        c.seal, c.seal_mask = ctypes.addressof(box), mask.data_ptr()

    def prepare_timing(self, frames):
        import ctypes
        cur = torch.cuda.current_stream()
        self._timing_queue = []
        for _ in range(frames):
            recs = []
            for _ in range(self.MAX_TIMED):
                s_, e_ = torch.cuda.Event(enable_timing=True), torch.cuda.Event(enable_timing=True)
                s_.record(cur); e_.record(cur)
                recs.append((s_, e_, 0))
            arr = (ctypes.c_void_p * (2 * self.MAX_TIMED))(*[h for r in recs for h in (r[0].cuda_event, r[1].cuda_event)])
            self._timing_queue.append((arr, recs))
        torch.cuda.synchronize()

    def frame_time(self, time):
        from sdn_backend import SdnFrameTime
        model = self.model
        times = list(time) if isinstance(time, (list, tuple)) else [time]
        if len(times) == 1 and self.frames > 1:
            times = times * self.frames
        if len(times) != self.frames:
            raise ValueError(f"{self.frames} frame(s) in this loop, {len(times)} time stamp(s) given")
        bias, mask, slices = self.field.group_constants(times)
        ft = SdnFrameTime()
        bits = [model.density_bitfield[s_] for s_ in slices]
        for f, b_ in enumerate(bits):
            ft.bitfield[f] = b_.data_ptr()
        ft.field_bias0, ft.zero_deform = bias.data_ptr(), mask
        culls = None
        if self.keep_cull_grids and int(model.grid_size) == 128 and int(model.cascade) == 1:
            culls = [self._cull_grid(s_) for s_ in slices]
            for f, g_ in enumerate(culls):
                ft.cull_grid[f] = g_.data_ptr()
        return ft, (bias, bits, culls)

    def _cull_grid(self, t_idx):
        import sdn_backend as B
        cache = self.model.__dict__.get("_sdn_cull_cache")
        if cache is None:
            cache = {"epoch": None, "grids": {}}
            self.model.__dict__["_sdn_cull_cache"] = cache
        bf = self.model.density_bitfield
        epoch = (self.model.iter_density, bf.data_ptr(), bf._version)
        if cache["epoch"] != epoch:
            cache["epoch"], cache["grids"] = epoch, {}
        hit = cache["grids"].get(t_idx)
        if hit is None:
            hit = torch.empty(int(B.lib.sdn_cull_grid_bytes()), dtype=torch.uint8, device=self.model.density_bitfield.device)
            B.check(B.lib.sdn_build_cull_grid(self.model.density_bitfield[t_idx].data_ptr(), 128, hit.data_ptr(), B.stream()), "build_cull_grid")
            cache["grids"][t_idx] = hit
        return hit

    @staticmethod
    def invalidate_cull_grids(model=None):
        if model is not None:
            model.__dict__.pop("_sdn_cull_cache", None)

    def bind(self, rays_o, rays_d, time):
        import ctypes
        from sdn_backend import ptr
        c, model = self.ctx, self.model
        rays_o = rays_o.contiguous().view(-1, 3)
        rays_d = rays_d.contiguous().view(-1, 3)
        assert rays_o.shape[0] == self.N
        nears, fars = self.buf["nears"], self.buf["fars"]
        c.aabb, c.min_near = ptr(model.aabb_infer, torch.float32, "aabb_infer"), float(model.min_near)
        ft, refs = self.frame_time(time)
        c.rays_o, c.rays_d = ptr(rays_o, torch.float32, "rays_o"), ptr(rays_d, torch.float32, "rays_d")
        c.bitfield, c.field_bias0, c.zero_deform = ft.bitfield[0], ft.field_bias0, int(ft.zero_deform)
        for f in range(self.frames):
            c.frame_bitfield[f] = ft.bitfield[f]
            c.frame_cull[f] = ft.cull_grid[f]
        self._frame_refs = (rays_o, rays_d, nears, fars, refs)
        cur = torch.cuda.current_stream()
        if self._handles is None:
            for e in self.events + self.copy_events:
                e.record(cur)
            self._ev_main = (ctypes.c_void_p * self.RING)(*[e.cuda_event for e in self.events])
            self._ev_copy = (ctypes.c_void_p * self.RING)(*[e.cuda_event for e in self.copy_events])
            self._iters = ctypes.c_uint32(0)
            self._handles = True
        return nears, fars

    def collect(self, nears, fars, want_stats):
        out = {"image": self.image_out, "depth": self.depth_out, "weights_sum": self.buf["weights_sum"], "nears": nears, "fars": fars}
        if want_stats:
            iters = int(self.buf["state"][3].item())
            tr = self.buf["trace"][: 2 * iters].cpu().view(-1, 2).tolist()
            out["trace"] = [(a, s, a * s + (128 - (a * s) % 128)) for a, s in tr]
            out["n_samples"] = int(self.buf["live_counts"][:iters].sum().item())
        return out

    @torch.no_grad()
    def render(self, rays_o, rays_d, time, bg_color=1.0, want_stats=True):
        import ctypes
        from sdn_backend import lib, check, ptr, stream
        import sdn_backend
        nears, fars = self.bind(rays_o, rays_d, time)
        bg_model = getattr(self.model, "bg_radius", -1) > 0
        if bg_model:
            bg_color = 0.0
        cur = torch.cuda.current_stream()
        ev_field, n_ev, recs = None, 0, None
        if sdn_backend.timers is not None and self._timing_queue:
            ev_field, recs = self._timing_queue.pop()
            n_ev = self.MAX_TIMED
        self.side.wait_stream(cur)
        check(lib.sdn_render_frame_f16(ctypes.byref(self.ctx), float(bg_color), ptr(self.image_out), ptr(self.depth_out), stream(),
                                       self.side.cuda_stream, self._ev_main, self._ev_copy, self.host_state.data_ptr(), ev_field, n_ev,
                                       ctypes.byref(self._iters)), "render_frame_f16")
        if recs is not None:
            sdn_backend.timers.records.setdefault("field_forward_f16", []).extend(recs[: min(n_ev, int(self._iters.value))])
        if bg_model:
            ro, rd = self._frame_refs[0], self._frame_refs[1]
            self.image_out += (1 - self.buf["weights_sum"]).unsqueeze(-1) * self.model._bg(ro, rd, None).float()
        return self.collect(nears, fars, want_stats)


def _context_streams(k, device):
    import os
    if os.environ.get("SDN_CTX_STREAMS", "") == "torch":
        return [torch.cuda.Stream(device=device) for _ in range(k)]
    import ctypes
    spec = os.environ.get("SDN_CTX_PRIORITIES", "").strip() or "0"
    try:
        prios = [int(x) for x in spec.split(",")]
    except ValueError:
        raise ValueError(f"SDN_CTX_PRIORITIES={spec!r}: expected comma-separated integers (HIP stream priorities, e.g. '-1,0,0,0')") from None
    if any(p < -1 or p > 1 for p in prios):
        raise ValueError(f"SDN_CTX_PRIORITIES={spec!r}: HIP stream priorities are -1 (high), 0, 1 (low)")
    key = (str(torch.device(device)), int(k), tuple(prios))
    if key in _CONTEXT_STREAMS:
        return _CONTEXT_STREAMS[key]
    try:
        hip = ctypes.CDLL("libamdhip64.so")
    except OSError:
        return [torch.cuda.Stream(device=device) for _ in range(k)]
    out = []
    with torch.cuda.device(device):
        for i in range(k):
            h = ctypes.c_void_p()
            rc = hip.hipStreamCreateWithPriority(ctypes.byref(h), ctypes.c_uint(1), ctypes.c_int(prios[i % len(prios)]))
            if rc != 0:
                raise RuntimeError(f"hipStreamCreateWithPriority failed ({rc})")
            out.append(torch.cuda.ExternalStream(h.value, device=device))
    _CONTEXT_STREAMS[key] = out
    return out


_CONTEXT_STREAMS = {}


class PipelinedDeviceLoop:

    def __init__(self, model, field, N, device, overlap_div=1, contexts=2, mailbox=True, **kw):
        import ctypes
        from sdn_backend import SdnRenderCtx, HostMailbox
        self.N, self.device, self.overlap_div, self.K = N, device, int(overlap_div), int(contexts)
        self.loops = [DeviceLoop(model, field, N, device, mailbox=mailbox, **kw) for _ in range(self.K)]
        self.streams = _context_streams(self.K, device)
        if self.K > 1:
            import sdn_backend as B
            B.lib.sdn_field_persistent_workgroups(int(torch.cuda.get_device_properties(device).multi_processor_count) * 7 // 8)
        self.host_state = HostMailbox(self.K) if mailbox else torch.zeros(self.K, 8, dtype=torch.int32).pin_memory()
        self._ctxs = (ctypes.POINTER(SdnRenderCtx) * self.K)(*[ctypes.pointer(lp.ctx) for lp in self.loops])
        self._fixed = None

    def _drive(self, lib, n, a_ro, a_rd, a_img, a_dep, bg_color, fx, a_ev, n_ev, exclusive, a_ft, a_done, iters):
        import ctypes
        from sdn_backend import check
        check(lib.sdn_render_frames_pipelined_f16(self._ctxs, self.K, n, a_ro, a_rd, a_img, a_dep, float(bg_color), self.overlap_div, fx["streams"],
                                                  fx["sides"], fx["ev_main"], fx["ev_copy"], self.host_state.data_ptr(), a_ev, n_ev,
                                                  (ctypes.c_uint8 * n)(*[1 if e else 0 for e in exclusive]) if exclusive is not None else None,
                                                  a_ft, a_done, iters),
              "render_frames_pipelined_f16")

    @torch.no_grad()
    def render_frames(self, rays_o, rays_d, time, bg_color=1.0, outputs=None, timing=None, exclusive=None, on_done=None):
        import ctypes
        import time as _t
        _tin = _t.perf_counter()
        from sdn_backend import lib, check, ptr
        n = len(rays_o)
        assert n == len(rays_d) and n >= 1
        cur = torch.cuda.current_stream()
        ro = [r.contiguous().view(-1, 3) for r in rays_o]
        rd = [r.contiguous().view(-1, 3) for r in rays_d]
        from sdn_backend import SdnFrameTime
        times = list(time) if isinstance(time, (list, tuple)) else [time] * n
        if len(times) != n:
            raise ValueError(f"{n} frames, {len(times)} time entries")
        a_ft = (SdnFrameTime * n)()
        ft_refs = []
        for f in range(n):
            rec, refs = self.loops[0].frame_time(times[f])
            a_ft[f] = rec
            ft_refs.append(refs)
        for s, lp in enumerate(self.loops):
            self.streams[s].wait_stream(cur)
            with torch.cuda.stream(self.streams[s]):
                lp.bind(ro[min(s, n - 1)], rd[min(s, n - 1)], times[min(s, n - 1)])
                lp.side.wait_stream(self.streams[s])
        if outputs is None:
            outputs = [(self.loops[f % self.K].image_out, self.loops[f % self.K].depth_out) for f in range(n)]
        vp = ctypes.c_void_p
        if self._fixed is None:
            K = self.K
            self._fixed = dict(streams=(vp * K)(*[s.cuda_stream for s in self.streams]),
                               sides=(vp * K)(*[lp.side.cuda_stream for lp in self.loops]),
                               ev_main=(vp * (4 * K))(*[e.cuda_event for lp in self.loops for e in lp.events]),
                               ev_copy=(vp * (4 * K))(*[e.cuda_event for lp in self.loops for e in lp.copy_events]))
        fx = self._fixed
        a_ro = (vp * n)(*[ptr(t, torch.float32, "rays_o") for t in ro])
        a_rd = (vp * n)(*[ptr(t, torch.float32, "rays_d") for t in rd])
        a_img = (vp * n)(*[ptr(o[0], torch.float32, "image_out") for o in outputs])
        a_dep = (vp * n)(*[ptr(o[1], torch.float32, "depth_out") for o in outputs])
        iters = (ctypes.c_uint32 * n)()
        a_ev, n_ev = None, 0
        if timing is not None:
            a_ev = (vp * n)(*[ctypes.cast(t, vp).value if t is not None else None for t in timing])
            n_ev = DeviceLoop.MAX_TIMED
        import os, time as _t
        _dbg = os.environ.get("SDN_DRIVER_STATS")
        a_done, worker = None, None
        if on_done is not None:
            from .dist import InOrderHandOn
            done = [torch.cuda.Event(enable_timing=True) for _ in range(n)]
            for e in done:
                e.record(cur)
            a_done = (vp * n)(*[e.cuda_event for e in done])
            dev_index = self.streams[0].device_index
            self._done_stream = getattr(self, "_done_stream", None) or torch.cuda.Stream()
            side = self._done_stream

            def in_side_stream():
                torch.cuda.set_device(dev_index)
                return torch.cuda.stream(side)
            worker = InOrderHandOn(n, lambda f: iters[f] != 0, on_done, outputs, before=lambda f: side.wait_event(done[f]),
                                   context=in_side_stream).start()
            self.last_done_events, self.last_hand_on = done, worker
# ... 84 lines not shown
```

### seald-nerf_amd/sdn_backend.py

```python
import ctypes
import os
import weakref

import torch

_HERE = os.path.dirname(os.path.abspath(__file__))
LIB_PATH = os.environ.get("SDN_LIB_PATH") or os.path.join(_HERE, "lib", "libsdn_hip.so")

SDN_F32 = 0
SDN_F16 = 1

_c = ctypes
_vp, _u32, _f32, _i32, _u64 = _c.c_void_p, _c.c_uint32, _c.c_float, _c.c_int, _c.c_uint64

PROTOTYPES = {
    "sdn_near_far_from_aabb": [_vp, _vp, _vp, _u32, _f32, _vp, _vp, _vp],
    "sdn_sph_from_ray": [_vp, _vp, _f32, _u32, _vp, _vp],
    "sdn_get_rays": [_vp, _f32, _f32, _f32, _f32, _u32, _u32, _vp, _vp, _vp],
    "sdn_morton3D": [_vp, _u32, _vp, _vp],
    "sdn_morton3D_invert": [_vp, _u32, _vp, _vp],
    "sdn_packbits": [_vp, _u32, _f32, _vp, _vp],
    "sdn_march_rays_train": [_vp, _vp, _vp, _f32, _f32, _u32, _u32, _u32, _u32, _u32, _vp, _vp, _vp, _vp, _vp, _vp, _vp, _vp, _vp, _vp],
    "sdn_composite_rays_train_forward": [_vp, _vp, _vp, _vp, _u32, _u32, _f32, _vp, _vp, _vp, _vp],
    "sdn_composite_whole_rays": [_vp, _vp, _vp, _vp, _vp, _u32, _u32, _f32, _vp, _vp, _vp, _vp],
    "sdn_composite_rays_train_backward": [_vp, _vp, _vp, _vp, _vp, _vp, _vp, _vp, _u32, _u32, _f32, _vp, _vp, _vp],
    "sdn_march_rays": [_u32, _u32, _vp, _vp, _vp, _vp, _f32, _f32, _u32, _u32, _u32, _vp, _vp, _vp, _vp, _vp, _vp, _vp, _vp],
    "sdn_march_rays_ex": [_u32, _u32, _vp, _vp, _vp, _vp, _f32, _f32, _u32, _u32, _u32, _vp, _vp, _vp, _vp, _vp, _vp, _u32, _vp, _vp, _vp, _vp],
    "sdn_build_cull_grid": [_vp, _u32, _vp, _vp],
    "sdn_composite_rays": [_u32, _u32, _f32, _vp, _vp, _vp, _vp, _vp, _vp, _vp, _vp, _vp],
    "sdn_compact_alive": [_vp, _u32, _vp, _vp, _vp, _vp],
    "sdn_grid_encode_forward": [_vp, _vp, _vp, _vp, _u32, _u32, _u32, _u32, _f32, _u32, _vp, _u32, _i32, _u32, _i32, _vp],
    "sdn_grid_encode_backward": [_vp, _vp, _vp, _vp, _u32, _u32, _u32, _u32, _f32, _u32, _vp, _vp, _u32, _i32, _u32, _i32, _vp],
    "sdn_grid_encode_backward_det": [_vp, _vp, _vp, _vp, _u32, _u32, _u32, _u32, _f32, _u32, _vp, _vp, _u32, _i32, _u32, _i32, _vp, _vp],
    "sdn_sh_encode_forward": [_vp, _vp, _u32, _u32, _u32, _vp, _vp],
    "sdn_sh_encode_backward": [_vp, _vp, _u32, _u32, _u32, _vp, _vp, _vp],
    "sdn_freq_encode_forward": [_vp, _u32, _u32, _u32, _u32, _vp, _vp],
    "sdn_freq_encode_backward": [_vp, _vp, _u32, _u32, _u32, _u32, _vp, _vp],
    "sdn_render_begin": [_vp, _vp],
    "sdn_render_step_f16": [_vp, _u32, _vp],
    "sdn_render_step_f16_ev": [_vp, _u32, _vp, _vp, _vp],
    "sdn_render_finish": [_vp, _f32, _vp, _vp, _vp],
    "sdn_render_time_kernel": [_i32],
    "sdn_render_frame_f16": [_vp, _f32, _vp, _vp, _vp, _vp, _vp, _vp, _vp, _vp, _u32, _vp],
    "sdn_render_frames_pipelined_f16": [_vp, _u32, _u32, _vp, _vp, _vp, _vp, _f32, _u32, _vp, _vp, _vp, _vp, _vp, _vp, _u32, _vp, _vp, _vp, _vp],
    "sdn_host_mailbox_free": [_vp],
    "sdn_seal_bbox_map": [_vp, _vp, _u32, _vp, _u32, _vp, _u32, _vp, _vp, _vp, _vp, _vp, _vp, _vp],
    "sdn_seal_modify_hsv": [_vp, _vp, _u32, _f32, _f32, _f32, _vp],
    "sdn_seal_bbox_map_source": [_vp, _vp, _u32, _vp, _u32, _vp, _u32, _vp, _vp, _vp, _vp, _vp, _vp, _vp, _vp, _vp, _vp, _vp, _vp, _vp],
    "sdn_seal_modify_rgb": [_vp, _vp, _u32, _f32, _f32, _f32, _f32, _vp, _vp, _vp, _vp, _vp],
    "sdn_field_forward_f16": [_vp, _vp, _vp, _vp, _u32, _vp, _vp, _vp, _vp, _f32, _u32, _f32, _f32, _i32, _vp, _vp, _vp],
    "sdn_field_forward_f32": [_vp, _vp, _vp, _vp, _u32, _vp, _vp, _vp, _vp, _f32, _u32, _f32, _f32, _i32, _vp, _vp, _vp, _vp],
    "sdn_field_forward_f32x3": [_vp, _vp, _vp, _vp, _u32, _vp, _vp, _vp, _vp, _f32, _u32, _f32, _f32, _i32, _vp, _vp, _vp, _vp],
    "sdn_field_build_quad_table": [_vp, _i32, _vp, _f32, _u32, _vp, _vp],
    "sdn_grid_encode_forward_quad_f16": [_vp, _vp, _vp, _vp, _u32, _f32, _u32, _vp],
    "sdn_density_query_cells_f16": [_vp, _vp, _u32, _vp, _u32, _u32, _f32, _vp, _vp, _vp, _vp, _f32, _u32, _f32, _f32, _i32, _vp, _vp],
    "sdn_debug_shader_clock": [_vp, _u32, _vp],
    "sdn_density_query_cells_f32": [_vp, _vp, _u32, _vp, _u32, _u32, _f32, _vp, _vp, _vp, _vp, _f32, _u32, _f32, _f32, _i32, _vp, _vp],
    "sdn_density_grid_ema": [_vp, _vp, ctypes.c_uint64, _f32, _vp, _vp],
    "sdn_density_grid_pack": [_vp, ctypes.c_uint64, _vp, _f32, _vp, _vp, _vp],
    "sdn_ffmlp_forward": [_vp, _vp, _u32, _u32, _u32, _u32, _u32, _u32, _u32, _vp, _vp, _vp, _vp],
    "sdn_ffmlp_inference": [_vp, _vp, _u32, _u32, _u32, _u32, _u32, _u32, _u32, _vp, _vp, _vp],
    "sdn_ffmlp_backward": [_vp, _vp, _vp, _vp, _u32, _u32, _u32, _u32, _u32, _u32, _u32, _i32, _vp, _vp, _vp, _vp, _vp],
}
MAX_GROUP_FRAMES = 16


class SdnFrameTime(ctypes.Structure):
    _fields_ = [("bitfield", _vp * MAX_GROUP_FRAMES), ("field_bias0", _vp), ("zero_deform", _u32), ("reserved_", _u32),
                ("cull_grid", _vp * MAX_GROUP_FRAMES)]


class SdnRenderCtx(ctypes.Structure):
    _fields_ = ([(n, _vp) for n in ("rays_o", "rays_d", "nears", "fars", "bitfield", "cull_bits", "alive_a", "alive_b", "rays_t",
                                   "weights_sum", "depth", "image", "xyzs", "dirs", "deltas", "sigmas", "rgbs", "live_idx",
                                   "live_counts", "state", "trace", "n_out", "block_totals", "field_weights", "field_bias0",
                                   "grid_table")]
                + [("grid_offsets", ctypes.c_int32 * 17), ("grid_S", _f32), ("grid_H", _u32)]
                + [(n, _u32) for n in ("N", "M_cap", "n_counters", "max_steps", "C", "H")]
                + [(n, _f32) for n in ("bound", "dt_gamma", "T_thresh", "density_scale")]
                + [("zero_deform", ctypes.c_int32), ("aabb", _vp), ("min_near", _f32), ("reserved_", ctypes.c_int32), ("rays_tend", _vp), ("seal", _vp), ("seal_mask", _vp),
                   ("n_group_frames", _u32), ("rays_per_frame", _u32), ("frame_bitfield", _vp * MAX_GROUP_FRAMES), ("slot_frame", _vp),
                   ("frame_cull", _vp * MAX_GROUP_FRAMES), ("field_f32", _i32), ("reserved2_", _i32)])


class SdnSealBox(ctypes.Structure):
    _fields_ = [("bounds", _f32 * 24), ("n_bounds", _u32), ("n_tris", _u32), ("tris", _vp), ("test_dir", _f32 * 3), ("tinv", _f32 * 12),
                ("rinv", _f32 * 9), ("scale", _f32 * 3), ("center", _f32 * 3), ("hsv", _f32 * 3), ("modify_hsv", ctypes.c_int32),
                ("rgb", _f32 * 3), ("rgb_light_offset", _f32), ("modify_rgb", ctypes.c_int32), ("has_map_source", ctypes.c_int32),
                ("source_bound", _f32 * 6), ("map_source", _f32 * 3), ("reserved_", _u32), ("scratch", _vp)]


TRAIN_N_PARAMS = 14


class SdnTrainParam(ctypes.Structure):
    _fields_ = [("param", _vp), ("exp_avg", _vp), ("exp_avg_sq", _vp), ("ema", _vp), ("n", ctypes.c_uint64)]


class SdnTrainStep(ctypes.Structure):
    _fields_ = ([(n, _vp) for n in ("rays_o", "rays_d", "target", "bg_color")]
                + [("bg_value", _f32), ("N", _u32), ("M", _u32), ("bitfield", _vp), ("cull_grid", _vp), ("aabb", _vp)]
                + [(n, _f32) for n in ("bound", "min_near", "dt_gamma", "density_scale", "T_thresh", "time")]
                + [(n, _u32) for n in ("cascade", "grid_size", "max_steps")]
                + [("perturb", ctypes.c_int32), ("noise_seed", ctypes.c_uint64), ("noises", _vp), ("counter", _vp),
                   ("grid_offsets", ctypes.c_int32 * 17), ("grid_S", _f32), ("grid_H", _u32),
                   ("params", SdnTrainParam * TRAIN_N_PARAMS)]
                + [(n, ctypes.c_double) for n in ("lr_table", "lr_net", "beta1", "beta2", "eps")]
                + [("adam_steps", _vp), ("loss_scale", _vp), ("growth_tracker", _vp), ("growth_factor", _f32), ("backoff_factor", _f32),
                   ("growth_interval", _u32), ("ema_decay", _f32), ("loss_out", _vp), ("image_out", _vp), ("workspace", _vp),
                   ("mode", ctypes.c_int32), ("keep_deform", ctypes.c_int32), ("grad_divisor", _f32), ("deform_frozen", ctypes.c_int32), ("phase", ctypes.c_int32), ("sample_set", ctypes.c_int32),
                   ("table_stream", _vp), ("table_ready", _vp), ("table_done", _vp), ("det_scratch", _vp)])


class SdnTrainLayout(ctypes.Structure):
    _fields_ = [(n, ctypes.c_uint64) for n in ("total_bytes", "w_table", "w_deform", "w_sigma0", "w_sigma1", "w_color", "g_table", "g_deform",
                                                "g_sigma0", "g_sigma1", "g_color", "xyzs", "dirs", "deltas", "rays", "sample_set_stride", "sigmas",
                                                "weights_sum", "depth", "image", "found_inf")]


PROTOTYPES.update({
    "sdn_train_layout": [_u32, _u32, _u32, ctypes.POINTER(ctypes.c_int32), ctypes.POINTER(SdnTrainLayout)],
    "sdn_train_refresh": [ctypes.POINTER(SdnTrainStep), _vp],
    "sdn_train_step_f16": [ctypes.POINTER(SdnTrainStep), _vp],
    "sdn_train_flush": [ctypes.POINTER(SdnTrainStep), _vp],
    "sdn_train_layout_f32": [_u32, _u32, _u32, ctypes.POINTER(ctypes.c_int32), ctypes.POINTER(SdnTrainLayout)],
    "sdn_train_refresh_f32": [ctypes.POINTER(SdnTrainStep), _vp],
    "sdn_train_step_f32": [ctypes.POINTER(SdnTrainStep), _vp],
})

PROTOTYPES_U32 = {
    "sdn_field_weight_blocks": [],
    "sdn_field_weight_floats_f32": [],
    "sdn_cull_grid_bytes": [],
}
PROTOTYPES_U64 = {
    "sdn_march_rays_train_scratch_bytes": [_u32, _u32],
    "sdn_compact_alive_scratch_bytes": [_u32],
    "sdn_ffmlp_scratch_bytes": [_u32, _u32, _u32, _u32, _u32],
}

if not os.path.exists(LIB_PATH):
    raise ImportError(
        f"{LIB_PATH} is missing: build it with `make -C seald-nerf_amd/csrc` (or __graft_entry__.build()). "
        "There is no CPU fallback for the SealD-NeRF operators.")

lib = ctypes.CDLL(LIB_PATH)
lib.sdn_version.restype = ctypes.c_char_p
lib.sdn_host_mailbox_alloc.restype = ctypes.c_void_p
lib.sdn_host_mailbox_alloc.argtypes = [ctypes.c_uint32]
lib.sdn_field_select_kernel.restype = None
lib.sdn_field_select_kernel.argtypes = [ctypes.c_int]
lib.sdn_field_persistent_workgroups.restype = None
lib.sdn_field_persistent_workgroups.argtypes = [ctypes.c_int]
for _name, _args in PROTOTYPES.items():
    _fn = getattr(lib, _name)
    _fn.argtypes = _args
    _fn.restype = ctypes.c_int
for _name, _args in PROTOTYPES_U32.items():
    _fn = getattr(lib, _name)
    _fn.argtypes = _args
    _fn.restype = ctypes.c_uint32
for _name, _args in PROTOTYPES_U64.items():
    _fn = getattr(lib, _name)
    _fn.argtypes = _args
    _fn.restype = ctypes.c_uint64


class SdnError(RuntimeError):
    pass


def check(rc, what):
    if rc != 0:
        kind = {-1: "bad argument", -2: "unsupported configuration", -3: "timed out waiting for the device"}.get(rc, f"hipError_t {rc}")
        raise SdnError(f"{what} failed: {kind}")


class HostMailbox:

    def __init__(self, groups=1):
        self.ptr = lib.sdn_host_mailbox_alloc(int(groups))
        if not self.ptr:
            raise SdnError("sdn_host_mailbox_alloc failed")

    def data_ptr(self):
        return self.ptr

    def __del__(self):
        try:
            if getattr(self, "ptr", None):
                lib.sdn_host_mailbox_free(self.ptr)
                self.ptr = None
        except Exception:
            pass


_device_seen = False


def require_device():
    global _device_seen
    if _device_seen:
        return
    if not torch.cuda.is_available():
        raise SdnError("SealD-NeRF HIP operators need a ROCm device (torch.cuda.is_available() is False); "
                       "there is no CPU fallback")
    _device_seen = True


def to_device(t):
    require_device()
    return t if t.is_cuda else t.cuda()


def ptr(t, dtype=None, name="tensor"):
    if t is None:
        return None
    if not t.is_cuda:
        raise SdnError(f"{name} must be a device tensor")
    if not t.is_contiguous():
        raise SdnError(f"{name} must be contiguous")
    if dtype is not None and t.dtype != dtype:
        raise SdnError(f"{name} must be {dtype}, got {t.dtype}")
    return t.data_ptr()


_raw_stream = getattr(torch._C, "_cuda_getCurrentRawStream", None)


def stream():
    if _raw_stream is not None:
        return _raw_stream(torch.cuda.current_device())
    return torch.cuda.current_stream().cuda_stream


_PENDING_WRITES = {}


def set_pending_write(t, writer):
    _PENDING_WRITES[id(t)] = (weakref.ref(t), weakref.ref(writer))


def await_pending_write(t):
    if not _PENDING_WRITES:
        return
    hit = _PENDING_WRITES.get(id(t))
    if hit is None or hit[0]() is not t:
        return
    writer = hit[1]()
    if writer is None or not writer.pending():
        del _PENDING_WRITES[id(t)]
        return
    writer.flush()


def dtype_id(dt):
    if dt == torch.float32:
        return SDN_F32
    if dt == torch.float16:
        return SDN_F16
    raise SdnError(f"unsupported table dtype {dt} (the reference dispatches float/half; double is not built)")


class KernelTimers:

    def __init__(self):
        self.records = {}

    def record(self, name, units):
        s = torch.cuda.Event(enable_timing=True)
        e = torch.cuda.Event(enable_timing=True)
        self.records.setdefault(name, []).append((s, e, units))
        return s, e

    def raw_pair(self, name, units):
        s, e = self.record(name, units)
        cur = torch.cuda.current_stream()
        s.record(cur); e.record(cur)
        return s.cuda_event, e.cuda_event

    def summary(self):
        torch.cuda.synchronize()
        out = {}
        for name, recs in self.records.items():
            ms = [s.elapsed_time(e) for s, e, _ in recs]
            units = [u for _, _, u in recs]
            out[name] = {"launches": len(recs), "total_ms": float(sum(ms)), "avg_ms": float(sum(ms) / len(ms)),
                         "units": int(sum(units)), "avg_units": float(sum(units) / len(units))}
        return out


timers = None


_launch_log = None


class launch_log:

    def __init__(self, out):
        self.out = out

    def __enter__(self):
        global _launch_log
        self.prev, _launch_log = _launch_log, self.out
        return self.out

    def __exit__(self, *exc):
        global _launch_log
        _launch_log = self.prev
        return False


class timed:

    def __init__(self, name, units):
        if _launch_log is not None:
            _launch_log.append((name, units))
        self.ev = timers.record(name, units) if timers is not None else None

    def __enter__(self):
        if self.ev:
            self.ev[0].record()

    def __exit__(self, *exc):
        if self.ev:
            self.ev[1].record()
        return False
```

Baseline: 3.288 billion sampled-points/s.

## Compact alive list inside fused composite-march kernel via per-block prefix offsets

Replaces the frozen alive list with survivors marked -1 by a ping-pong list that the fused composite+march kernel compacts as it goes. Each block writes its entries at an offset taken from a per-block prefix table, and its samples go to the compacted slot. The last block rebuilds the prefix table for the next step. Deltas are double-buffered so compositing reads the old layout while marching writes the new one. This drops the periodic recompaction path and keeps slot indices dense as rays die. In exchange it adds a block-level scan in the final block and two extra syncs per block.

```diff
diff --git a/include/sdn_hip.h b/include/sdn_hip.h
--- a/include/sdn_hip.h
+++ b/include/sdn_hip.h
@@ -205,12 +205,17 @@
     const void *frame_cull[SDN_MAX_GROUP_FRAMES];
     int32_t field_f32;
     int32_t reserved2_;
+    float *deltas_b;
+    uint32_t *steady_blocks;
 } SdnRenderCtx;
+#define SDN_STEADY_BLOCKS(N) ((N) / 2048u + 2u)
 
 int sdn_render_begin(const SdnRenderCtx *ctx, void *stream);
 int sdn_render_step_f16(const SdnRenderCtx *ctx, uint32_t bound_alive, void *stream);
 int sdn_render_step_f16_ev(const SdnRenderCtx *ctx, uint32_t bound_alive, void *ev_field_begin, void *ev_field_end,
                            void *stream);
+int sdn_render_steady_begin(const SdnRenderCtx *ctx, uint32_t bound_alive, void *stream);
+int sdn_render_steady_step_f16(const SdnRenderCtx *ctx, uint32_t bound_list, void *stream);
 int sdn_render_time_kernel(int which);
 int sdn_render_frame_f16(const SdnRenderCtx *ctx, float bg_color, float *image_out, float *depth_out, void *stream,
                          void *side_stream, void **ev_main, void **ev_copy, int32_t *host_snap, void **ev_field,
diff --git a/seald-nerf_amd/csrc/raymarching.hip b/seald-nerf_amd/csrc/raymarching.hip
--- a/seald-nerf_amd/csrc/raymarching.hip
+++ b/seald-nerf_amd/csrc/raymarching.hip
@@ -1028,10 +1028,6 @@
     if (live_idx) live_append(step, n, n_step, live_idx, live_count);
 }
 
-__device__ __forceinline__ uint32_t loop_list_len(const int32_t *__restrict__ state) {
-    return state[8] ? (uint32_t)state[8] : (uint32_t)state[0];
-}
-
 __global__ void __launch_bounds__(256) k_composite_rays(uint32_t n_alive, uint32_t n_step, float T_thresh, int32_t *__restrict__ rays_alive,
                                                         float *__restrict__ rays_t, const float *__restrict__ sigmas,
                                                         const float *__restrict__ rgbs, const float *__restrict__ deltas,
@@ -1039,7 +1035,7 @@
                                                         const int32_t *__restrict__ state, int32_t *__restrict__ rays_alive_b,
                                                         uint32_t *__restrict__ block_totals) {
     if (state) {
-        n_alive = loop_list_len(state);
+        n_alive = (uint32_t)state[0];
         n_step = (uint32_t)state[1];
         if (state[4]) rays_alive = rays_alive_b;
     }
@@ -1065,7 +1061,7 @@
 __global__ void __launch_bounds__(kScanBlock) k_compact_count(const int32_t *__restrict__ in, uint32_t n, uint32_t *__restrict__ block_totals,
                                                               const int32_t *__restrict__ state, const int32_t *__restrict__ in_b) {
     if (state) {
-        n = loop_list_len(state);
+        n = (uint32_t)state[0];
         if (state[4]) in = in_b;
         if (blockIdx.x * kScanBlock >= n) return;
     }
@@ -1088,7 +1084,7 @@
                                                                 int32_t *__restrict__ out_b, uint32_t totals_per_block) {
     uint32_t last_block = gridDim.x - 1;
     if (state) {
-        n = loop_list_len(state);
+        n = (uint32_t)state[0];
         if (state[4]) { in = in_b; out = out_b; }
         if (n == 0) {
             if (blockIdx.x == 0 && threadIdx.x == 0) n_out[0] = 0;
@@ -1278,7 +1274,7 @@
 }
 
 __global__ void k_loop_advance(int32_t *__restrict__ state, const int32_t *__restrict__ n_out, int32_t *__restrict__ trace,
-                               int32_t *__restrict__ snap, int freeze) {
+                               int32_t *__restrict__ snap) {
     if (threadIdx.x != 0 || blockIdx.x != 0) return;
     const int32_t it = state[3];
     const int32_t call = state[7];
@@ -1297,7 +1293,6 @@
             state[1] = ns > 8 ? 8 : (ns < 1 ? 1 : ns);
         }
     }
-    if (freeze) { state[8] = state[0]; state[9] = 0; }
     publish_snapshot(state, snap, call);
 }
 
@@ -1312,11 +1307,10 @@
 
 __global__ void __launch_bounds__(256) k_scatter_advance(int32_t *__restrict__ alive_a, int32_t *__restrict__ alive_b,
                                                          const uint32_t *__restrict__ block_totals, int32_t *__restrict__ state,
-                                                         int32_t *__restrict__ ticket, int32_t *__restrict__ trace, int32_t *__restrict__ snap,
-                                                         int freeze) {
+                                                         int32_t *__restrict__ ticket, int32_t *__restrict__ trace, int32_t *__restrict__ snap) {
     __shared__ uint32_t lds4[4];
     __shared__ int s_last;
-    const uint32_t n = loop_list_len(state);
+    const uint32_t n = (uint32_t)state[0];
     const int32_t *in = state[4] ? alive_b : alive_a;
     int32_t *out = state[4] ? alive_a : alive_b;
     const uint32_t nb = (n + 255u) / 256u;
@@ -1367,14 +1361,15 @@
                 state[1] = ns > 8 ? 8 : (ns < 1 ? 1 : ns);
             }
         }
-        if (freeze) { state[8] = state[0]; state[9] = 0; }
         publish_snapshot(state, snap, call);
     }
 }
 
 
-__global__ void k_steady_begin(int32_t *__restrict__ state) {
-    if (threadIdx.x == 0 && blockIdx.x == 0) { state[8] = state[0]; state[9] = 0; }
+__global__ void __launch_bounds__(256) k_steady_begin(int32_t *__restrict__ state, uint32_t *__restrict__ blocks, uint32_t S) {
+    const uint32_t i = threadIdx.x + blockIdx.x * blockDim.x;
+    if (i < S) { blocks[i] = 0; blocks[S + i] = 256u * i; }
+    if (i == 0) { state[8] = state[0]; state[9] = 0; }
 }
 
 template <bool FAST>
@@ -1383,25 +1378,33 @@
                                                          const float *__restrict__ rays_d, float bound, float dt_gamma, uint32_t max_steps,
                                                          uint32_t C, uint32_t H, const uint8_t *__restrict__ grid, const float *__restrict__ fars,
                                                          const float *__restrict__ sigmas, const float *__restrict__ rgbs,
-                                                         float *__restrict__ xyzs, float *__restrict__ dirs, float *__restrict__ deltas,
-                                                         float *__restrict__ weights_sum, float *__restrict__ depth, float *__restrict__ image,
+                                                         float *__restrict__ xyzs, float *__restrict__ dirs, float *__restrict__ deltas_a,
+                                                         float *__restrict__ deltas_b, float *__restrict__ weights_sum,
+                                                         float *__restrict__ depth, float *__restrict__ image,
                                                          const uint32_t *__restrict__ cull, uint32_t *__restrict__ live_idx,
                                                          uint32_t *__restrict__ live_counts, int32_t *__restrict__ state,
                                                          int32_t *__restrict__ ticket, int32_t *__restrict__ trace, int32_t *__restrict__ snap,
-                                                         FrameSel fs) {
+                                                         uint32_t *__restrict__ blocks, uint32_t S, FrameSel fs) {
     __shared__ uint4 s_cull4[FAST ? 256 : 1];
     __shared__ unsigned long long s_fine[FAST ? kFineCacheCells : 1];
-    __shared__ uint32_t s_cnt[4], s_min4[4];
+    __shared__ uint32_t s_cnt[4], s_hi[4], s_min4[4];
     __shared__ int s_last;
-    const uint32_t n_alive = (uint32_t)state[0], n_step = (uint32_t)state[1], list_len = (uint32_t)state[8];
+    const uint32_t n_alive = (uint32_t)state[0], n_step = (uint32_t)state[1], list_len = (uint32_t)state[8], side = (uint32_t)state[9] & 1u;
     const int32_t it = state[3];
-    int32_t *__restrict__ alive = state[4] ? alive_b : alive_a;
+    const int32_t *__restrict__ list_in = state[4] ? alive_b : alive_a;
+    int32_t *__restrict__ list_out = state[4] ? alive_a : alive_b;
+    const float *__restrict__ deltas_in = side ? deltas_b : deltas_a;
+    float *__restrict__ deltas_out = side ? deltas_a : deltas_b;
     const bool march_next = (uint32_t)state[2] + n_step < (uint32_t)state[6];
     const uint32_t n = threadIdx.x + blockIdx.x * blockDim.x;
+    const uint32_t lane = threadIdx.x & 63u, wid = threadIdx.x >> 6;
     bool survives = false;
-    uint32_t emitted = 0;
-    if (n_alive > 0 && blockIdx.x * 256u < list_len) {
-        const int index = n < list_len ? alive[n] : -1;
+    uint32_t emitted = 0, pos = 0, first = 0;
+    if (n_alive > 0 && blockIdx.x * 256u < list_len && blockIdx.x < S) {
+        const int index = n < list_len ? list_in[n] : -1;
+        first = blocks[S * (1u + side) + blockIdx.x];
+        const unsigned long long entered = __ballot(index >= 0);
+        if (lane == 0) s_cnt[wid] = (uint32_t)__popcll(entered);
         float ro[3] = {0, 0, 0}, rdv[3] = {0, 0, 1}, far_ray = 0, t_new = 0;
         if (index >= 0) {
             if (march_next) {
@@ -1410,9 +1413,14 @@
                 far_ray = fars[index];
             }
             survives = composite_ray(index, n_step, T_thresh, sigmas + (size_t)n * n_step, rgbs + (size_t)n * n_step * 3,
-                                     deltas + (size_t)n * n_step * 2, rays_t, weights_sum, depth, image, &t_new);
-            if (!survives) alive[n] = -1;
-        }
+                                     deltas_in + (size_t)n * n_step * 2, rays_t, weights_sum, depth, image, &t_new);
+        }
+        __syncthreads();
+        pos = first + (uint32_t)__popcll(entered & ((1ull << lane) - 1ull));
+        for (uint32_t w = 0; w < wid; w++) pos += s_cnt[w];
+        const bool placed = index >= 0 && pos < n_alive;
+        if (placed) list_out[pos] = survives ? index : -1;
+        survives = survives && placed;
         const bool marches = survives && march_next;
         const bool grouped = fs.n_frames > 1;
         const uint32_t frame = (grouped && marches) ? (uint32_t)index / fs.rays_per_frame : (grouped ? kNoFrame : 0u);
@@ -1423,41 +1431,69 @@
             OccCache oc;
             occ_cache_load<FAST>(cull_f, grid_f, s_cull4, s_fine, oc);
             if (marches && frame == fcur) {
-                float *px = xyzs + (size_t)n * n_step * 3, *pd = dirs + (size_t)n * n_step * 3, *pl = deltas + (size_t)n * n_step * 2;
+                float *px = xyzs + (size_t)pos * n_step * 3, *pd = dirs + (size_t)pos * n_step * 3, *pl = deltas_out + (size_t)pos * n_step * 2;
                 MarcherT<FAST> m;
                 m.init(ro, rdv, bound, dt_gamma, max_steps, C, H, grid_f);
                 float *tend = state_tend(state);
                 if (tend) tend += index;
                 emitted = march_ray<FAST>(m, oc, t_new, far_ray, n_step, px, pd, pl, tend,
-                                          grouped ? fs.slot_frame + (size_t)n * n_step : nullptr, frame);
+                                          grouped ? fs.slot_frame + (size_t)pos * n_step : nullptr, frame);
             }
             if (!grouped) break;
             fcur = block_min_256((frame != kNoFrame && frame > fcur) ? frame : kNoFrame, s_min4);
         }
-        live_append(emitted, n, n_step, live_idx, live_counts + it + 1);
-    }
-    const unsigned long long mask = __ballot(survives);
-    if ((threadIdx.x & 63u) == 0) s_cnt[threadIdx.x >> 6] = (uint32_t)__popcll(mask);
+        live_append(emitted, pos, n_step, live_idx, live_counts + it + 1);
+    }
+    const uint32_t blk = first >> 8;
+    const unsigned long long mask = __ballot(survives), mask_hi = __ballot(survives && (pos >> 8) != blk);
+    __syncthreads();
+    if (lane == 0) { s_cnt[wid] = (uint32_t)__popcll(mask & ~mask_hi); s_hi[wid] = (uint32_t)__popcll(mask_hi); }
     __syncthreads();
     if (threadIdx.x == 0) {
-        const uint32_t c = s_cnt[0] + s_cnt[1] + s_cnt[2] + s_cnt[3];
-        if (c) atomicAdd(state + 9, (int32_t)c);
+        const uint32_t lo = s_cnt[0] + s_cnt[1] + s_cnt[2] + s_cnt[3], hi = s_hi[0] + s_hi[1] + s_hi[2] + s_hi[3];
+        if (lo && blk < S) atomicAdd(blocks + blk, lo);
+        if (hi && blk + 1u < S) atomicAdd(blocks + blk + 1u, hi);
         __threadfence();
         s_last = (atomicAdd(ticket, 1) == (int)gridDim.x - 1);
     }
     __syncthreads();
-    if (!s_last || threadIdx.x != 0) return;
+    if (!s_last) return;
     __threadfence();
+    uint32_t nb = n_alive > 0 ? (n_alive + 255u) / 256u : 0u;
+    if (nb > S) nb = S;
+    const uint32_t per = (nb + 255u) / 256u, b0 = threadIdx.x * per;
+    uint32_t *__restrict__ prefix_out = blocks + S * (2u - side);
+    uint32_t mine = 0;
+    for (uint32_t b = b0; b < b0 + per && b < nb; b++) mine += __hip_atomic_load(blocks + b, __ATOMIC_RELAXED, __HIP_MEMORY_SCOPE_AGENT);
+    uint32_t incl = mine;
+    #pragma unroll
+    for (int off = 1; off < 64; off <<= 1) {
+        const uint32_t u = __shfl_up(incl, off, 64);
+        if (lane >= (uint32_t)off) incl += u;
+    }
+    if (lane == 63) s_cnt[wid] = incl;
+    __syncthreads();
+    uint32_t run = incl - mine;
+    for (uint32_t w = 0; w < wid; w++) run += s_cnt[w];
+    for (uint32_t b = b0; b < b0 + per && b < nb; b++) {
+        const uint32_t c = __hip_atomic_load(blocks + b, __ATOMIC_RELAXED, __HIP_MEMORY_SCOPE_AGENT);
+        prefix_out[b] = run;
+        blocks[b] = 0;
+        run += c;
+    }
+    if (threadIdx.x != 0) return;
     *ticket = 0;
     const int32_t call = state[7];
     state[7] = call + 1;
-    if (state[0] > 0) {
+    if (n_alive > 0) {
         trace[2 * it] = state[0];
         trace[2 * it + 1] = state[1];
         state[2] += state[1];
         state[3] = it + 1;
-        int32_t n_new = atomicAdd(state + 9, 0);
-        state[9] = 0;
+        state[4] ^= 1;
+        state[8] = (int32_t)n_alive;
+        state[9] = (int32_t)(side ^ 1u);
+        int32_t n_new = (int32_t)(s_cnt[0] + s_cnt[1] + s_cnt[2] + s_cnt[3]);
         if (state[2] >= state[6]) n_new = 0;
         state[0] = n_new;
     }
@@ -1522,7 +1558,7 @@
 
 int loop_composite_compact(uint32_t bound_alive, float T_thresh, int32_t *alive_a, int32_t *alive_b, float *rays_t, const float *sigmas,
                            const float *rgbs, const float *deltas, float *weights_sum, float *depth, float *image, int32_t *state,
-                           uint32_t *block_totals, int32_t *n_out, int32_t *trace, int32_t *snap, hipStream_t st, bool freeze) {
+                           uint32_t *block_totals, int32_t *n_out, int32_t *trace, int32_t *snap, hipStream_t st) {
     const dim3 g(sdn_div_up(bound_alive, 256u)), b(256);
     if (bound_alive > 65536u) {
         static_assert(kScanBlock == 1024, "the compositing kernel's 256-ray survivor counts are summed four to a scatter block");
@@ -1531,12 +1567,12 @@
         const uint32_t nb = sdn_div_up(bound_alive, kScanBlock);
         hipLaunchKernelGGL(k_compact_scatter, dim3(nb), dim3(kScanBlock), 0, st, (const int32_t *)alive_a, 0u, (const uint32_t *)block_totals,
                            alive_b, snap + 8, (const int32_t *)state, (const int32_t *)alive_b, alive_a, 4u);
-        hipLaunchKernelGGL(k_loop_advance, dim3(1), dim3(64), 0, st, state, (const int32_t *)(snap + 8), trace, snap, freeze ? 1 : 0);
+        hipLaunchKernelGGL(k_loop_advance, dim3(1), dim3(64), 0, st, state, (const int32_t *)(snap + 8), trace, snap);
         return sdn_launch_status();
     }
     hipLaunchKernelGGL(k_composite_rays, g, b, 0, st, 0u, 0u, T_thresh, alive_a, rays_t, sigmas, rgbs, deltas, weights_sum, depth, image,
                        (const int32_t *)state, alive_b, block_totals);
-    hipLaunchKernelGGL(k_scatter_advance, g, b, 0, st, alive_a, alive_b, (const uint32_t *)block_totals, state, n_out, trace, snap, freeze ? 1 : 0);
+    hipLaunchKernelGGL(k_scatter_advance, g, b, 0, st, alive_a, alive_b, (const uint32_t *)block_totals, state, n_out, trace, snap);
     return sdn_launch_status();
 }
 
@@ -1544,27 +1580,28 @@
 int loop_steady_begin(uint32_t bound_alive, const int32_t *alive_a, const int32_t *alive_b, const float *rays_t, const float *rays_o,
                       const float *rays_d, float bound, float dt_gamma, uint32_t max_steps, uint32_t C, uint32_t H, const uint8_t *grid,
                       const float *fars, float *xyzs, float *dirs, float *deltas, const uint32_t *cull, uint32_t *live_idx,
-                      uint32_t *live_counts, int32_t *state, const FrameSel &fs, hipStream_t st, bool frozen_already) {
-    if (!frozen_already) hipLaunchKernelGGL(k_steady_begin, dim3(1), dim3(64), 0, st, state);
+                      uint32_t *live_counts, int32_t *state, uint32_t *steady_blocks, uint32_t S, const FrameSel &fs, hipStream_t st) {
+    hipLaunchKernelGGL(k_steady_begin, dim3(sdn_div_up(S, 256u)), dim3(256), 0, st, state, steady_blocks, S);
     return loop_march(bound_alive, alive_a, alive_b, rays_t, rays_o, rays_d, bound, dt_gamma, max_steps, C, H, grid, fars, xyzs, dirs, deltas,
                       cull, live_idx, live_counts, state, fs, st, nullptr);
 }
 
 int loop_composite_march(uint32_t bound_list, float T_thresh, int32_t *alive_a, int32_t *alive_b, float *rays_t, const float *rays_o,
                          const float *rays_d, float bound, float dt_gamma, uint32_t max_steps, uint32_t C, uint32_t H, const uint8_t *grid,
-                         const float *fars, const float *sigmas, const float *rgbs, float *xyzs, float *dirs, float *deltas,
+                         const float *fars, const float *sigmas, const float *rgbs, float *xyzs, float *dirs, float *deltas, float *deltas_b,
                          float *weights_sum, float *depth, float *image, const uint32_t *cull, uint32_t *live_idx, uint32_t *live_counts,
-                         int32_t *state, int32_t *ticket, int32_t *trace, int32_t *snap, const FrameSel &fs, hipStream_t st) {
+                         int32_t *state, int32_t *ticket, int32_t *trace, int32_t *snap, uint32_t *steady_blocks, uint32_t S,
+                         const FrameSel &fs, hipStream_t st) {
     const dim3 g(sdn_div_up(bound_list, 256u)), b(256);
     if (fast_config(bound, C, H)) {
         if (cull && H != 128) cull = nullptr;
         hipLaunchKernelGGL(k_composite_march<true>, g, b, 0, st, T_thresh, alive_a, alive_b, rays_t, rays_o, rays_d, bound, dt_gamma, max_steps, C, H,
-                           grid, fars, sigmas, rgbs, xyzs, dirs, deltas, weights_sum, depth, image, cull, live_idx, live_counts, state, ticket,
-                           trace, snap, fs);
+                           grid, fars, sigmas, rgbs, xyzs, dirs, deltas, deltas_b, weights_sum, depth, image, cull, live_idx, live_counts, state,
+                           ticket, trace, snap, steady_blocks, S, fs);
     } else {
         hipLaunchKernelGGL(k_composite_march<false>, g, b, 0, st, T_thresh, alive_a, alive_b, rays_t, rays_o, rays_d, bound, dt_gamma, max_steps, C,
-                           H, grid, fars, sigmas, rgbs, xyzs, dirs, deltas, weights_sum, depth, image, (const uint32_t *)nullptr, live_idx,
-                           live_counts, state, ticket, trace, snap, fs);
+                           H, grid, fars, sigmas, rgbs, xyzs, dirs, deltas, deltas_b, weights_sum, depth, image, (const uint32_t *)nullptr, live_idx,
+                           live_counts, state, ticket, trace, snap, steady_blocks, S, fs);
     }
     return sdn_launch_status();
 }
diff --git a/seald-nerf_amd/csrc/render.hip b/seald-nerf_amd/csrc/render.hip
--- a/seald-nerf_amd/csrc/render.hip
+++ b/seald-nerf_amd/csrc/render.hip
@@ -141,12 +141,50 @@
                                            c->trace + 2 * (size_t)c->n_counters, st);
 }
 
+static const uint32_t *ctx_cull(const SdnRenderCtx *c) { return (c->H == 128 && c->C == 1) ? (const uint32_t *)c->cull_bits : nullptr; }
+
+int sdn_render_steady_begin(const SdnRenderCtx *c, uint32_t bound_alive, void *stream) {
+    if (!c || bound_alive == 0 || !c->deltas_b || !c->steady_blocks) return SDN_E_BADARG;
+    if (bound_alive > c->N / 8u) bound_alive = c->N / 8u;
+    if (bound_alive == 0) return SDN_E_BADARG;
+    return sdn_int::loop_steady_begin(bound_alive, c->alive_a, c->alive_b, c->rays_t, c->rays_o, c->rays_d, c->bound, c->dt_gamma, c->max_steps, c->C,
+                                      c->H, c->bitfield, c->fars, c->xyzs, c->dirs, c->deltas, ctx_cull(c), c->live_idx, (uint32_t *)c->live_counts,
+                                      c->state, c->steady_blocks, SDN_STEADY_BLOCKS(c->N), sdn_int::frame_sel(c), (hipStream_t)stream);
+}
+
+static int steady_step(const SdnRenderCtx *c, uint32_t bound_list, uint32_t expect_points, void *e0, void *e1, hipStream_t st) {
+    if (!c || bound_list == 0 || !c->deltas_b || !c->steady_blocks) return SDN_E_BADARG;
+    if (bound_list > c->N / 8u) bound_list = c->N / 8u;
+    if (bound_list == 0) return SDN_E_BADARG;
+    const uint32_t m_bound = bound_list * 8u;
+    int rc = seal_map(c, m_bound, st);
+    if (rc) return rc;
+    const bool time_march = g_timed_kernel.load() == 1;
+    void *m0 = time_march ? e0 : nullptr, *m1 = time_march ? e1 : nullptr;
+    if (time_march) e0 = e1 = nullptr;
+    if (e0) (void)hipEventRecord((hipEvent_t)e0, st);
+    rc = launch_field(c, m_bound, expect_points, st);
+    if (e1) (void)hipEventRecord((hipEvent_t)e1, st);
+    if (!rc) rc = seal_color(c, m_bound, st);
+    if (rc) return rc;
+    if (m0) (void)hipEventRecord((hipEvent_t)m0, st);
+    rc = sdn_int::loop_composite_march(bound_list, c->T_thresh, c->alive_a, c->alive_b, c->rays_t, c->rays_o, c->rays_d, c->bound, c->dt_gamma,
+                                       c->max_steps, c->C, c->H, c->bitfield, c->fars, c->sigmas, c->rgbs, c->xyzs, c->dirs, c->deltas, c->deltas_b,
+                                       c->weights_sum, c->depth, c->image, ctx_cull(c), c->live_idx, (uint32_t *)c->live_counts, c->state, c->n_out,
+                                       c->trace, c->trace + 2 * (size_t)c->n_counters, c->steady_blocks, SDN_STEADY_BLOCKS(c->N),
+                                       sdn_int::frame_sel(c), st);
+    if (!rc && m1) (void)hipEventRecord((hipEvent_t)m1, st);
+    return rc;
+}
+
+int sdn_render_steady_step_f16(const SdnRenderCtx *c, uint32_t bound_list, void *stream) {
+    return steady_step(c, bound_list, 0u, nullptr, nullptr, (hipStream_t)stream);
+}
+
 }
 
 namespace {
 
-constexpr uint32_t kRecompactMin = 8192;
-uint32_t recompact_pct(uint32_t list_len) { return list_len > 81920u ? 95u : 50u; }
 constexpr int kDriverTimeoutSeconds = 20;
 
 struct FrameRun {
@@ -157,15 +195,13 @@
     uint32_t max_field_events;
     uint32_t bound, it;
     bool steady, done;
-    bool recompact = false;
-    uint32_t list_bound = 0;
     void *mail_dev = nullptr;
     uint32_t tag = 0;
     uint32_t last_alive = 0;
 
     int begin() {
-        if (!ctx_ok(c)) return SDN_E_BADARG;
-        bound = c->N; it = 0; steady = false; done = false; last_alive = c->N; recompact = false; list_bound = 0;
+        if (!ctx_ok(c) || !c->deltas_b || !c->steady_blocks) return SDN_E_BADARG;
+        bound = c->N; it = 0; steady = false; done = false; last_alive = c->N;
         mail_dev = nullptr;
         unsigned int flags = 0;
         void *dptr = nullptr;
@@ -179,51 +215,21 @@
         }
         return sdn_int::render_begin(c, mail_dev, tag, st);
     }
-    const uint32_t *cull() const { return (c->H == 128 && c->C == 1) ? (const uint32_t *)c->cull_bits : nullptr; }
-
     int enqueue() {
-        int32_t *snap_dev = c->trace + 2 * (size_t)c->n_counters;
         void *e0 = (ev_field && it < max_field_events) ? ev_field[2 * it] : nullptr;
         void *e1 = (ev_field && it < max_field_events) ? ev_field[2 * it + 1] : nullptr;
         int rc;
         if (!steady) {
             rc = sdn_render_step_f16_ev(c, bound, e0, e1, st);
         } else {
-            uint64_t m_bound = (uint64_t)bound * 8u;
-            if (m_bound > c->N) m_bound = c->N;
-            rc = seal_map(c, (uint32_t)m_bound, st);
-            if (rc) return rc;
-            const bool time_march = g_timed_kernel.load() == 1;
-            void *m0 = time_march ? e0 : nullptr, *m1 = time_march ? e1 : nullptr;
-            if (time_march) e0 = e1 = nullptr;
-            if (e0) (void)hipEventRecord((hipEvent_t)e0, st);
-            rc = launch_field(c, (uint32_t)m_bound, last_alive * 8u, st);
-            if (e1) (void)hipEventRecord((hipEvent_t)e1, st);
-            if (!rc) rc = seal_color(c, (uint32_t)m_bound, st);
-            if (!rc && m0) (void)hipEventRecord((hipEvent_t)m0, st);
-            if (!rc && recompact) {
-                rc = sdn_int::loop_composite_compact(bound, c->T_thresh, c->alive_a, c->alive_b, c->rays_t, c->sigmas, c->rgbs, c->deltas, c->weights_sum,
-                                                     c->depth, c->image, c->state, (uint32_t *)c->block_totals, c->n_out, c->trace, snap_dev, st, true);
-                const uint32_t nb = last_alive < bound ? last_alive : bound;
-                if (!rc)
-                    rc = sdn_int::loop_steady_begin(nb, c->alive_a, c->alive_b, c->rays_t, c->rays_o, c->rays_d, c->bound, c->dt_gamma, c->max_steps, c->C,
-                                                    c->H, c->bitfield, c->fars, c->xyzs, c->dirs, c->deltas, cull(), c->live_idx, (uint32_t *)c->live_counts,
-                                                    c->state, sdn_int::frame_sel(c), st, true);
-                bound = list_bound = nb;
-                recompact = false;
-            } else if (!rc)
-                rc = sdn_int::loop_composite_march(bound, c->T_thresh, c->alive_a, c->alive_b, c->rays_t, c->rays_o, c->rays_d, c->bound,
-                                                   c->dt_gamma, c->max_steps, c->C, c->H, c->bitfield, c->fars, c->sigmas, c->rgbs, c->xyzs,
-                                                   c->dirs, c->deltas, c->weights_sum, c->depth, c->image, cull(), c->live_idx,
-                                                   (uint32_t *)c->live_counts, c->state, c->n_out, c->trace, snap_dev, sdn_int::frame_sel(c), st);
-            if (!rc && m1) (void)hipEventRecord((hipEvent_t)m1, st);
+            rc = steady_step(c, bound, last_alive * 8u, e0, e1, st);
         }
         if (rc) return rc;
         if (mail_dev) return 0;
         const uint32_t slot = it & 3u;
         hipError_t e = hipEventRecord((hipEvent_t)ev_main[slot], st);
         if (e == hipSuccess) e = hipStreamWaitEvent(side, (hipEvent_t)ev_main[slot], 0);
-        if (e == hipSuccess) e = hipMemcpyAsync(host_snap + 2 * slot, snap_dev + 2 * slot, 2 * sizeof(int32_t), hipMemcpyDeviceToHost, side);
+        if (e == hipSuccess) e = hipMemcpyAsync(host_snap + 2 * slot, c->trace + 2 * (size_t)c->n_counters + 2 * slot, 2 * sizeof(int32_t), hipMemcpyDeviceToHost, side);
         if (e == hipSuccess) e = hipEventRecord((hipEvent_t)ev_copy[slot], side);
         return (int)e;
     }
@@ -268,18 +274,11 @@
             }
             if (n_prev <= 0) { done = true; return 0; }
             last_alive = (uint32_t)n_prev;
-            if (!steady) {
-                bound = (uint32_t)n_prev;
-                if ((uint64_t)n_prev * 8u <= c->N) {
-                    int rc = sdn_int::loop_steady_begin(bound, c->alive_a, c->alive_b, c->rays_t, c->rays_o, c->rays_d, c->bound, c->dt_gamma,
-                                                        c->max_steps, c->C, c->H, c->bitfield, c->fars, c->xyzs, c->dirs, c->deltas, cull(),
-                                                        c->live_idx, (uint32_t *)c->live_counts, c->state, sdn_int::frame_sel(c), st);
-                    if (rc) return rc;
-                    steady = true;
-                    list_bound = bound;
-                }
-            } else if ((uint64_t)n_prev * 100u <= (uint64_t)list_bound * recompact_pct(list_bound) && (uint32_t)n_prev >= kRecompactMin) {
-                recompact = true;
+            bound = (uint32_t)n_prev;
+            if (!steady && (uint64_t)n_prev * 8u <= c->N) {
+                int rc = sdn_render_steady_begin(c, bound, st);
+                if (rc) return rc;
+                steady = true;
             }
         }
         it++;
diff --git a/seald-nerf_amd/csrc/sdn_internal.h b/seald-nerf_amd/csrc/sdn_internal.h
--- a/seald-nerf_amd/csrc/sdn_internal.h
+++ b/seald-nerf_amd/csrc/sdn_internal.h
@@ -25,16 +25,17 @@
                uint32_t *live_counts, const int32_t *state, const FrameSel &fs, hipStream_t st, const float *jump = nullptr);
 int loop_composite_compact(uint32_t bound_alive, float T_thresh, int32_t *alive_a, int32_t *alive_b, float *rays_t, const float *sigmas,
                            const float *rgbs, const float *deltas, float *weights_sum, float *depth, float *image, int32_t *state,
-                           uint32_t *block_totals, int32_t *n_out, int32_t *trace, int32_t *snap, hipStream_t st, bool freeze = false);
+                           uint32_t *block_totals, int32_t *n_out, int32_t *trace, int32_t *snap, hipStream_t st);
 int loop_steady_begin(uint32_t bound_alive, const int32_t *alive_a, const int32_t *alive_b, const float *rays_t, const float *rays_o,
                       const float *rays_d, float bound, float dt_gamma, uint32_t max_steps, uint32_t C, uint32_t H, const uint8_t *grid,
                       const float *fars, float *xyzs, float *dirs, float *deltas, const uint32_t *cull, uint32_t *live_idx,
-                      uint32_t *live_counts, int32_t *state, const FrameSel &fs, hipStream_t st, bool frozen_already = false);
+                      uint32_t *live_counts, int32_t *state, uint32_t *steady_blocks, uint32_t S, const FrameSel &fs, hipStream_t st);
 int loop_composite_march(uint32_t bound_list, float T_thresh, int32_t *alive_a, int32_t *alive_b, float *rays_t, const float *rays_o,
                          const float *rays_d, float bound, float dt_gamma, uint32_t max_steps, uint32_t C, uint32_t H, const uint8_t *grid,
-                         const float *fars, const float *sigmas, const float *rgbs, float *xyzs, float *dirs, float *deltas,
+                         const float *fars, const float *sigmas, const float *rgbs, float *xyzs, float *dirs, float *deltas, float *deltas_b,
                          float *weights_sum, float *depth, float *image, const uint32_t *cull, uint32_t *live_idx, uint32_t *live_counts,
-                         int32_t *state, int32_t *ticket, int32_t *trace, int32_t *snap, const FrameSel &fs, hipStream_t st);
+                         int32_t *state, int32_t *ticket, int32_t *trace, int32_t *snap, uint32_t *steady_blocks, uint32_t S,
+                         const FrameSel &fs, hipStream_t st);
 int loop_finish(uint32_t N, const float *nears, const float *fars, const float *weights_sum, const float *depth, const float *image, float bg,
                 float *image_out, float *depth_out, hipStream_t st);
 int render_begin(const SdnRenderCtx *c, void *mailbox, uint32_t frame_tag, hipStream_t st);
diff --git a/seald-nerf_amd/dnerf_amd/renderer.py b/seald-nerf_amd/dnerf_amd/renderer.py
--- a/seald-nerf_amd/dnerf_amd/renderer.py
+++ b/seald-nerf_amd/dnerf_amd/renderer.py
@@ -420,7 +420,7 @@
     def __init__(self, model, field, N, device, max_steps=1024, T_thresh=1e-2, dt_gamma=0.0, mailbox=True, mapper=None, frames=1,
                  keep_cull_grids=False):
         import ctypes
-        from sdn_backend import lib, SdnRenderCtx, MAX_GROUP_FRAMES
+        from sdn_backend import lib, SdnRenderCtx, MAX_GROUP_FRAMES, steady_blocks
         f32, i32 = torch.float32, torch.int32
         self.model, self.field, self.N = model, field, N
         self.frames = int(frames)
@@ -431,10 +431,11 @@
         n_counters = max_steps + 8
         z = lambda *shape, dt=f32: torch.empty(*shape, dtype=dt, device=device)
         self.buf = dict(alive_a=z(N, dt=i32), alive_b=z(N, dt=i32), rays_t=z(N), weights_sum=z(N), depth=z(N), image=z(N, 3),
-                        xyzs=z(M, 3), dirs=z(M, 3), deltas=z(M, 2), sigmas=z(M), rgbs=z(M, 3), live_idx=z(M, dt=i32),
+                        xyzs=z(M, 3), dirs=z(M, 3), deltas=z(M, 2), deltas_b=z(M, 2), sigmas=z(M), rgbs=z(M, 3), live_idx=z(M, dt=i32),
                         live_counts=torch.zeros(n_counters, dtype=i32, device=device), state=torch.zeros(16, dtype=i32, device=device),
                         trace=torch.zeros(2 * n_counters + 16, dtype=i32, device=device), n_out=torch.zeros(1, dtype=i32, device=device),
-                        block_totals=z((N + 255) // 256 + 1, dt=i32), nears=z(N), fars=z(N), rays_tend=z(N),
+                        block_totals=z((N + 255) // 256 + 1, dt=i32),
+                        steady_blocks=torch.zeros(3 * steady_blocks(N), dtype=i32, device=device), nears=z(N), fars=z(N), rays_tend=z(N),
                         cull_bits=torch.empty(self.frames * int(lib.sdn_cull_grid_bytes()), dtype=torch.uint8, device=device))
         if self.frames > 1:
             self.buf["slot_frame"] = torch.zeros(M, dtype=torch.uint8, device=device)
diff --git a/seald-nerf_amd/sdn_backend.py b/seald-nerf_amd/sdn_backend.py
--- a/seald-nerf_amd/sdn_backend.py
+++ b/seald-nerf_amd/sdn_backend.py
@@ -39,6 +39,8 @@
     "sdn_render_begin": [_vp, _vp],
     "sdn_render_step_f16": [_vp, _u32, _vp],
     "sdn_render_step_f16_ev": [_vp, _u32, _vp, _vp, _vp],
+    "sdn_render_steady_begin": [_vp, _u32, _vp],
+    "sdn_render_steady_step_f16": [_vp, _u32, _vp],
     "sdn_render_finish": [_vp, _f32, _vp, _vp, _vp],
     "sdn_render_time_kernel": [_i32],
     "sdn_render_frame_f16": [_vp, _f32, _vp, _vp, _vp, _vp, _vp, _vp, _vp, _vp, _u32, _vp],
@@ -65,6 +67,10 @@
 MAX_GROUP_FRAMES = 16
 
 
+def steady_blocks(n_rays):
+    return n_rays // 2048 + 2
+
+
 class SdnFrameTime(ctypes.Structure):
     _fields_ = [("bitfield", _vp * MAX_GROUP_FRAMES), ("field_bias0", _vp), ("zero_deform", _u32), ("reserved_", _u32),
                 ("cull_grid", _vp * MAX_GROUP_FRAMES)]
@@ -80,7 +86,7 @@
                 + [(n, _f32) for n in ("bound", "dt_gamma", "T_thresh", "density_scale")]
                 + [("zero_deform", ctypes.c_int32), ("aabb", _vp), ("min_near", _f32), ("reserved_", ctypes.c_int32), ("rays_tend", _vp), ("seal", _vp), ("seal_mask", _vp),
                    ("n_group_frames", _u32), ("rays_per_frame", _u32), ("frame_bitfield", _vp * MAX_GROUP_FRAMES), ("slot_frame", _vp),
-                   ("frame_cull", _vp * MAX_GROUP_FRAMES), ("field_f32", _i32), ("reserved2_", _i32)])
+                   ("frame_cull", _vp * MAX_GROUP_FRAMES), ("field_f32", _i32), ("reserved2_", _i32), ("deltas_b", _vp), ("steady_blocks", _vp)])
 
 
 class SdnSealBox(ctypes.Structure):
```

Result: slower. 3.239 billion sampled-points/s (-1.5%).
